# AbeelLab/phasm

Measured on AMD Instinct MI355X. Metric: overlaps_per_sec, higher is better.
Workload: dtype u64

## Files before the change

phasm_amd/csrc/c_api.hip:

```cpp
#include "../../include/phasm_overlap.h"

#include <hip/hip_runtime.h>

#include <dlfcn.h>
#include <execinfo.h>
#include <fcntl.h>
#include <signal.h>
#include <sys/mman.h>
#include <sys/stat.h>
#include <unistd.h>

#include <algorithm>
#include <array>
#include <atomic>
#include <chrono>
#include <cmath>
#include <condition_variable>
#include <cstdio>
#include <cstdlib>
#include <cstring>
#include <deque>
#include <functional>
#include <memory>
#include <mutex>
// ... 65 lines not shown
    uint64_t base, bytes;
    uint32_t kind;
};
std::mutex g_pin_mu;
std::vector<PinNote> g_pins;
uint64_t g_pins_ever = 0;
constexpr size_t PIN_LOG_MAX = 1u << 16;
void pin_note(const void* p, size_t bytes, uint32_t kind) {
    if (!p) return;
    std::lock_guard<std::mutex> lock(g_pin_mu);
    ++g_pins_ever;
    for (PinNote& n : g_pins)
        if (n.base == (uint64_t)(uintptr_t)p && n.bytes == bytes && (n.kind & 0xFFu) == kind) {
            n.kind |= 0x100u;
            return;
        }
    if (g_pins.size() < PIN_LOG_MAX) g_pins.push_back(PinNote{(uint64_t)(uintptr_t)p, (uint64_t)bytes, kind | 0x100u});
}
void pin_drop(const void* p) {
    if (!p) return;
    std::lock_guard<std::mutex> lock(g_pin_mu);
    for (PinNote& n : g_pins)
        if (n.base == (uint64_t)(uintptr_t)p && (n.kind & 0x100u)) n.kind &= ~0x100u;
}

struct HostBuf {
    void* p = nullptr;
    size_t cap = 0;
    void release() {
        if (p) {
            pin_drop(p);
            (void)hipHostFree(p);
        }
        p = nullptr;
        cap = 0;
    }
};

inline int phase_events_env() {
    if (const char* e = getenv("PHASM_PHASE_EVENTS")) {
        const int v = atoi(e);
        return v == 1 ? 1 : v == 2 ? 2 : 0;
    }
    return getenv("PHASM_STREAM_TRACE") ? 1 : -1;
}
enum { EV_START = 0, EV_INDEX, EV_COUNT, EV_FILL, EV_VERIFY, EV_SELECT, EV_EMIT, EV_PROBE0, EV_PROBE1, EV_VER0, EV_VER1, EV_DONE, EV_N };

}

constexpr int PO_MAX_PIECES = 16;

struct RegHeader {
    size_t bytes;
    int registered;
};
constexpr size_t REG_PAGE = 4096;
thread_local bool g_reg_defer = false;
template <class T>
struct RegAlloc {
    using value_type = T;
    RegAlloc() = default;
    template <class U> RegAlloc(const RegAlloc<U>&) {}
    T* allocate(size_t n) {
        const size_t bytes = ((n * sizeof(T) + REG_PAGE - 1) / REG_PAGE) * REG_PAGE;
        void* base = nullptr;
        if (posix_memalign(&base, REG_PAGE, bytes + REG_PAGE) != 0 || !base) throw std::bad_alloc();
        RegHeader* hd = static_cast<RegHeader*>(base);
        hd->bytes = bytes;
        hd->registered = 0;
        char* data = static_cast<char*>(base) + REG_PAGE;
        if (getenv("PHASM_POISON_HOST")) std::memset(data, 0xA5, bytes);
        if (!g_reg_defer) reg_now(data);
        return reinterpret_cast<T*>(data);
    }
    static void reg_now(void* data) {
        RegHeader* hd = reinterpret_cast<RegHeader*>(static_cast<char*>(data) - REG_PAGE);
        if (hd->registered || hd->bytes < (1u << 20) || getenv("PHASM_NO_PIN")) return;
        if (hipHostRegister(data, hd->bytes, hipHostRegisterPortable) == hipSuccess) {
            hd->registered = 1;
            pin_note(data, hd->bytes, 2u);
        } else {
            (void)hipGetLastError();
        }
    }
    template <class U> void construct(U*) noexcept {}
    template <class U, class A0, class... Args> void construct(U* q, A0&& a0, Args&&... args) {
        ::new (static_cast<void*>(q)) U(std::forward<A0>(a0), std::forward<Args>(args)...);
    }
    void deallocate(T* p, size_t) {
        char* base = reinterpret_cast<char*>(p) - REG_PAGE;
        RegHeader* hd = reinterpret_cast<RegHeader*>(base);
        if (hd->registered) {
            pin_drop(p);
            (void)hipHostUnregister(p);
        }
        free(base);
    }
    template <class U> bool operator==(const RegAlloc<U>&) const { return true; }
    template <class U> bool operator!=(const RegAlloc<U>&) const { return false; }
};
using WordStore = std::vector<uint64_t, RegAlloc<uint64_t>>;
inline bool store_is_pinned(const WordStore& w) {
    if (w.capacity() == 0) return false;
    const RegHeader* hd = reinterpret_cast<const RegHeader*>(reinterpret_cast<const char*>(w.data()) - REG_PAGE);
    return hd->registered != 0;
}
constexpr size_t STAGE_MAX = 4u << 20;

struct po_handle {
    int device = 0;
    bool dev_ready = false;
    hipStream_t stream = nullptr;
    hipEvent_t ev_sets[2][EV_N] = {};
    hipEvent_t* ev = ev_sets[0];
    hipEvent_t ev_up0 = nullptr, ev_up1 = nullptr;
    uint64_t* pinned = nullptr;
    uint64_t* pinned_dev = nullptr;
    int n_cu = 256;
    size_t lds_max = 64 * 1024;
    std::string err;

    int bits = 2;
    std::vector<std::string> ids;
    std::vector<uint32_t> len;
    std::vector<uint64_t> cum_len;
    std::vector<uint64_t> woff;
    WordStore words[2];
    bool all_pairs_rc = true;
    bool all_pairs_rcx = true;
    uint64_t base1 = 0;
    uint64_t dev_words = 0;
    uint64_t upload_bytes = 0;
    std::vector<uint32_t> exc_off{0};
    std::vector<uint32_t> exc_pos;
    std::vector<uint8_t> exc_byte;
    std::vector<uint8_t> pair_state;
    uint64_t total_bases = 0;
    bool dirty = true;

    DevBuf d_words, d_woff, d_len, d_tiles, d_read_tile0, d_exc_off, d_exc_pos, d_exc_byte, d_pair_state;
    std::vector<uint32_t> h_read_tile0;
    uint32_t n_tiles = 0;
    uint32_t max_len = 0;
    size_t n_exc_uploaded = 0;
    bool paired = false;

    DevBuf d_table, d_slot_cnt, d_slot_cur, d_slot_start, d_read_slot, d_chain, d_chain_tmp, d_long_list;
    DevBuf d_entry_off;
    DevBuf d_bloom, d_selfrep, d_tile_count, d_tile_off, d_truemask, d_ps_blocks, d_scalars, d_left, d_left_cnt, d_tile_extra;
    DevBuf d_cand_a, d_cand_p, d_cand_b, d_type, d_rowcnt, d_row_off, d_flag, d_pair_key, d_pair_min;
    DevBuf d_vlabel, d_vrank, d_vperm;
    DevBuf d_chain_state;
    DevBuf d_tail_state;
    DevBuf spare_rows;
    DevBuf spare_cands;
    DevBuf spare_edges;
    DevBuf spare_nrank;
    HostBuf spare_host;
    HostBuf scratch_host;
    uint64_t pool_bases = 0;
    std::vector<void*> arena_chunks;
    char* arena_cur = nullptr;
    size_t arena_left = 0;
    int poison = -1;
    hipStream_t copy_stream = nullptr;
    DevBuf chunk_rows[PO_MAX_PIECES + 1];
    bool chunk_compact[PO_MAX_PIECES + 1] = {};
    bool home_on = false;
    HostBuf home_stage;
    size_t home_used = 0;
    uint64_t home_seq = 0;
    uint32_t home_gen = 0;
    uint32_t home_sh_b = 0, home_sh_p = 0;
    uint64_t home_pack_n = ~0ull, home_pack_bases = ~0ull;
    uint32_t home_pack_b = 0, home_pack_p = 0;
    uint64_t home_last_bytes = 0;

    hipStream_t up_stream = nullptr;
    hipEvent_t ev_piece[PO_MAX_PIECES] = {};
    hipStream_t rc_stream = nullptr;
    hipEvent_t ev_rc[PO_MAX_PIECES] = {};
    hipEvent_t ev_meta = nullptr;
    hipEvent_t ev_first = nullptr;
    WordStore first_words;
    uint32_t first_n = 0;
    WordStore lead_words;
    uint32_t lead_n = 0;
    uint32_t st_lead = 2;
    HostBuf meta_host;
    HostBuf stage_host;
    size_t stage_used = 0;
    uint32_t meta_n = 0xFFFFFFFFu;
    int meta_bits = 0;
    uint64_t elig_n = ~0ull, elig_val = 0;
    uint32_t elig_m = 0;
    DevBuf d_first, d_defer;
    uint32_t defer_need = 0;
    struct Pending {
        bool valid = false;
        uint32_t k = 0;
        po_stats S = {};
        bool ver_timed = false;
        bool full_events = true;
        bool pair_events = true;
        bool tail = false;
        bool compact = false;
        int zone = 48;
        uint32_t cap_c = 0;
        hipEvent_t* ev = nullptr;
    } st_pend;
    std::function<po_status()> st_harvest;
    uint64_t st_pred_cand[PO_MAX_PIECES] = {};
    std::vector<uint32_t> st_pred_sig;
    bool st_pred_valid = false;
    bool st_selfclean = false;
    bool st_early_index = false;
    bool st_tail_gave_up = false;
    uint32_t st_defer_cap = 0;
    uint64_t last_host_rows = 0;
    uint64_t upload_gen = 0;
    bool idx_valid = false;
    uint64_t idx_gen = 0;
    uint32_t idx_m = 0, idx_tbits = 0, idx_bits = 0, idx_ww = 0;
    bool idx_wide = false;
    bool sl_is_wide = false;
    uint32_t sl_tbits = 0;
    uint64_t sl_entries = 0;
    const uint64_t* asm_pieces = nullptr;
    uint64_t asm_slot_words = 0;
    uint32_t asm_n = 0, asm_parts = 1;
    DevBuf d_end_a, d_end_b, d_dpcnt;
    int live_results = 0;

    po_stats stats = {};

    bool segments_only = false;
    int ids_paired = -1;
    hipEvent_t ev_lay[EV_LAY_N] = {};
    DevBuf d_lay_len, d_lay_cnt, d_rflag, d_removed, d_ekey, d_ecnt, d_ewin, d_eoff;
    DevBuf d_efirst;
    po_layout_stats lstats = {};

    DevBuf d_red[RB_N];
    po_reduce_stats rstats = {};

    DevBuf d_lay_firstc;
    DevBuf d_tip[TB_N];
    po_tips_stats tstats = {};
    po_diamond_stats dstats = {};
    po_node_order_stats nostats = {};

    DevBuf d_mrg[MB_N];
    po_merge_stats mstats = {};

    DevBuf d_cov[VB_N];
    po_coverage_stats cstats = {};

    DevBuf d_rank[RK_N];
    DevBuf d_cc[KB_N];
    po_components_stats ccstats = {};
    DevBuf d_scc[PB_N];
    po_partition_stats pstats = {};
    DevBuf d_sb[UB_N];
    po_superbubble_stats sbstats = {};
    DevBuf d_bc[HB_N];
    po_bubblechain_stats bcstats = {};
    DevBuf d_ct[CB_N];
    po_contig_stats ctstats = {};
    DevBuf d_ph[FB_N];
    po_phase_stats phstats = {};
};

struct po_result {
    po_handle* h = nullptr;
    DevBuf d_rows;
    uint64_t count = 0;
    size_t elem = sizeof(po_row);
    bool kind_edges = false;
    void* host = nullptr;
    size_t host_cap = 0;
    bool host_malloced = false;
    bool unique_twins = false;
    DevBuf d_rank;
    DevBuf d_nrank;
    bool merged = false;
    bool host_graph = false;
    uint64_t n_merged = 0, n_members = 0;
    DevBuf d_moff, d_member, d_prefix, d_mlen;
    void* ext_dst = nullptr;
    uint64_t ext_cap = 0;
    bool wrote_ext = false;
    bool compact = false;
};

namespace {

po_status fail(po_handle* h, po_status st, const std::string& msg) {
    if (h) h->err = msg;
    return st;
}

#define HIP_TRY(h, expr)                                                                        \
    do {                                                                                        \
        hipError_t e_ = (expr);                                                                 \
        if (e_ != hipSuccess) {                                                                 \
            return fail((h), e_ == hipErrorOutOfMemory ? PO_ERR_NOMEM : PO_ERR_HIP,             \
                        std::string(#expr) + ": " + hipGetErrorString(e_));                     \
        }                                                                                       \
    } while (0)

struct AllocTrace {
    const char* what;
    size_t bytes;
    std::chrono::steady_clock::time_point t0;
    bool on;
    AllocTrace(const char* w, size_t b) : what(w), bytes(b), on(getenv("PHASM_ALLOC_TRACE") != nullptr) {
        if (on) t0 = std::chrono::steady_clock::now();
    }
    ~AllocTrace() {
        if (on)
            std::fprintf(stderr, "[alloc] %-16s %10.3f MB  %8.3f ms\n", what, bytes / 1e6,
                         std::chrono::duration<double, std::milli>(std::chrono::steady_clock::now() - t0).count());
    }
};

struct OverlapArgs {
    uint32_t min_length = 0, shard = 0, nshards = 1;
    bool want_cands = false;
    bool streamed = false, idx_only = false;
    uint32_t r_begin = 0, r_end = 0;
    double ws_scale = 1.0;
    uint32_t build_slice = 0, build_n = 0;
    const void* ext_index = nullptr;
    uint32_t ext_slices = 0, ext_tbits = 0, ext_chunk_slots = 0, ext_chain_off = 0;
    bool dp = false;
    uint32_t dp_E = 0, dp_W = 0;
};

po_status ensure(po_handle* h, DevBuf& b, size_t bytes, double scale = 1.0, bool arena_ok = true, bool streamed = false) {
    if (bytes <= b.cap) return PO_OK;
    AllocTrace tr("hipMalloc", bytes);
    const bool first = b.p == nullptr;
    b.release();
    size_t want = bytes + bytes / 8 + 256;
    if (scale > 1.0) want = (size_t)((double)bytes * scale) + 256;
    if (streamed) want += 8192;
    constexpr size_t ARENA_CHUNK = 64u << 20, ARENA_MAX = 8u << 20;
    if (h && first && arena_ok && want <= ARENA_MAX && !getenv("PHASM_NO_ARENA")) {
        want = (want + 255) & ~size_t(255);
        if (h->arena_left < want) {
            void* c = nullptr;
            if (hipMalloc(&c, ARENA_CHUNK) == hipSuccess) {
                h->arena_chunks.push_back(c);
                h->arena_cur = static_cast<char*>(c);
                h->arena_left = ARENA_CHUNK;
            } else {
                (void)hipGetLastError();
            }
        }
        if (h->arena_left >= want) {
            b.p = h->arena_cur;
            b.cap = want;
            b.arena = true;
            h->arena_cur += want;
            h->arena_left -= want;
            if (h->poison >= 0 && h->stream) (void)hipMemsetAsync(b.p, h->poison, want, h->stream);
            return PO_OK;
        }
    }
    hipError_t e = hipMalloc(&b.p, want);
    if (e != hipSuccess) {
// ... 110 lines not shown
        h->ev_up0 = k.ev_up0;
        h->ev_up1 = k.ev_up1;
        h->ev_meta = k.ev_meta;
        h->ev_first = k.ev_first;
        std::memcpy(h->ev_piece, k.ev_piece, sizeof(k.ev_piece));
        std::memcpy(h->ev_rc, k.ev_rc, sizeof(k.ev_rc));
        std::memcpy(h->ev_lay, k.ev_lay, sizeof(k.ev_lay));
        h->pinned = k.pinned;
        h->pinned_dev = k.pinned_dev;
        return true;
    }
    return false;
}

bool kit_give(po_handle* h) {
    if (getenv("PHASM_NO_KIT_POOL") || !h->stream || !h->copy_stream || !h->up_stream || !h->rc_stream || !h->pinned) return false;
    if (hipStreamSynchronize(h->stream) != hipSuccess || hipStreamSynchronize(h->copy_stream) != hipSuccess ||
        hipStreamSynchronize(h->up_stream) != hipSuccess || hipStreamSynchronize(h->rc_stream) != hipSuccess) {
        (void)hipGetLastError();
        return false;
    }
    DevKit k;
    k.device = h->device;
    k.stream = h->stream;
    k.copy_stream = h->copy_stream;
    k.up_stream = h->up_stream;
    k.rc_stream = h->rc_stream;
    std::memcpy(k.ev_sets, h->ev_sets, sizeof(k.ev_sets));
    k.ev_up0 = h->ev_up0;
    k.ev_up1 = h->ev_up1;
    k.ev_meta = h->ev_meta;
    k.ev_first = h->ev_first;
    std::memcpy(k.ev_piece, h->ev_piece, sizeof(k.ev_piece));
    std::memcpy(k.ev_rc, h->ev_rc, sizeof(k.ev_rc));
    std::memcpy(k.ev_lay, h->ev_lay, sizeof(k.ev_lay));
    k.pinned = h->pinned;
    k.pinned_dev = h->pinned_dev;
    std::lock_guard<std::mutex> lock(g_kit_mu);
    if (g_kits.size() >= KIT_POOL_MAX) return false;
    g_kits.push_back(k);
    return true;
}


unsigned cpu_share() {
    static const unsigned share = [] {
        unsigned n = std::thread::hardware_concurrency();
        n = n ? n : 4u;
        long long q = -1, per = 100000;
        if (FILE* f = std::fopen("/sys/fs/cgroup/cpu.max", "r")) {
            char buf[64] = {0};
            if (std::fscanf(f, "%63s %lld", buf, &per) >= 1 && std::strcmp(buf, "max") != 0) q = atoll(buf);
            std::fclose(f);
        } else if (FILE* g = std::fopen("/sys/fs/cgroup/cpu/cpu.cfs_quota_us", "r")) {
            if (std::fscanf(g, "%lld", &q) != 1) q = -1;
            std::fclose(g);
            if (FILE* g2 = std::fopen("/sys/fs/cgroup/cpu/cpu.cfs_period_us", "r")) {
                if (std::fscanf(g2, "%lld", &per) != 1) per = 100000;
                std::fclose(g2);
            }
        }
        if (q > 0 && per > 0) n = std::min<unsigned>(n, (unsigned)std::max<long long>(1, q / per));
        return n;
    }();
    return share;
}

namespace home {

constexpr uint32_t CHUNK = 4096;

struct Job {
    const void* rec = nullptr;
    uint32_t sh_b = 0, sh_p = 0;
    uint64_t n_rec = 0;
    po_row* out = nullptr;
    uint64_t n_rows = 0;
    const volatile uint32_t* flag = nullptr;
    uint32_t want = 0;
    uint32_t paired = 0, bits = 2;
};

struct Pool {
    std::vector<std::thread> thr;
    std::mutex mu;
    std::condition_variable cv_queue;
    std::condition_variable cv_job;
    std::mutex call_mu;
    std::deque<Job> queue;
    std::atomic<uint64_t> submitted{0}, finished{0};
    std::atomic<int> error{0};
    const uint32_t* len = nullptr;
    uint32_t n_reads = 0;
    std::atomic<uint64_t> sum_l{0}, sum_b{0}, sum_e{0};
    Job cur;
    uint64_t job_seq = 0;
    uint32_t n_chunks = 0;
    std::vector<uint64_t> chunk_off;
    std::atomic<uint32_t> next_count{0}, done_count{0}, next_write{0}, done_write{0};
    std::atomic<int> phase{0};
    std::atomic<int> inside{0};
    std::chrono::steady_clock::time_point t0;
    std::vector<std::array<double, 3>> trace;
    bool tracing = false;
};

Pool* g_pool = nullptr;
std::once_flag g_pool_once;

inline void cpu_pause() {
#if defined(__x86_64__) || defined(__i386__)
    __builtin_ia32_pause();
#endif
}

std::atomic<uint32_t> g_spin_limit{4096};
template <class Pred>
inline void spin_until(Pred pred) {
    const uint32_t limit = g_spin_limit.load(std::memory_order_relaxed);
    for (uint32_t n = 0; !pred(); ++n) {
        if (limit == 0 || n < limit) cpu_pause();
        else std::this_thread::yield();
    }
}

inline po::Cand load_rec(const Job& j, uint64_t i) {
    if (!j.sh_b) return static_cast<const po::Cand*>(j.rec)[i];
    return po::unpack_record(static_cast<const uint64_t*>(j.rec)[i], j.sh_b, j.sh_p);
}

inline uint32_t rows_of_rec(const po::Cand& c, uint32_t paired) {
    if (!paired) return (c.type & 1u) + ((c.type >> 1) & 1u);
    return ((c.type & 1u) ? (c.a == (c.b ^ 1u) ? 1u : 2u) : 0u) + ((c.type & 2u) ? 2u : 0u);
}

inline void put_row(uint64_t*& o, uint32_t a, uint32_t b, uint32_t astart, uint32_t aend, uint32_t bend) {
    __builtin_nontemporal_store((uint64_t)a | ((uint64_t)b << 32), o);
    __builtin_nontemporal_store((uint64_t)astart | ((uint64_t)aend << 32), o + 1);
    __builtin_nontemporal_store((uint64_t)bend << 32, o + 2);
    o += 3;
}

bool expand_records(Pool& P, uint64_t lo, uint64_t hi, po_row* out) {
    uint64_t* o = reinterpret_cast<uint64_t*>(out);
    const Job& job = P.cur;
    const uint32_t* len = P.len;
    const uint32_t paired = job.paired, n_reads = P.n_reads, bits = job.bits;
    auto pb = [bits](uint32_t l) -> uint64_t { return bits == 8u ? l : (l >> 2) + ((l & 3u) != 0u); };
    uint64_t sl = 0, sb = 0, se = 0;
    for (uint64_t i = lo; i < hi; ++i) {
        const po::Cand c = load_rec(job, i);
        if (c.a >= n_reads || c.b >= n_reads) return false;
        const uint32_t la = len[c.a], lb = len[c.b];
        se += 2 * pb((c.type & 1u) ? la - c.p : lb);
        if (c.type & 1u) {
            const uint32_t l = la - c.p;
            const bool twin = paired && c.a != (c.b ^ 1u);
            put_row(o, c.a, c.b, c.p, la, l);
            if (twin) put_row(o, c.b ^ 1u, c.a ^ 1u, lb - l, lb, l);
            const uint64_t k = twin ? 2 : 1;
            sl += k * l;
            sb += k * 2 * pb(l);
        }
        if (c.type & 2u) {
            put_row(o, c.a, c.b, c.p, c.p + lb, lb);
            if (paired) put_row(o, c.a ^ 1u, c.b ^ 1u, la - c.p - lb, la - c.p, lb);
            const uint64_t k = paired ? 2 : 1;
            sl += k * lb;
            sb += k * 2 * pb(lb);
        }
    }
    P.sum_l.fetch_add(sl, std::memory_order_relaxed);
    P.sum_b.fetch_add(sb, std::memory_order_relaxed);
    P.sum_e.fetch_add(se, std::memory_order_relaxed);
    return true;
}

void run_phases(Pool& P, bool lead) {
    const uint32_t nc = P.n_chunks;
    for (;;) {
        const uint32_t c = P.next_count.fetch_add(1, std::memory_order_relaxed);
        if (c >= nc) break;
        const uint64_t lo = (uint64_t)c * CHUNK, hi = std::min<uint64_t>(P.cur.n_rec, lo + CHUNK);
        uint64_t n = 0;
        const uint32_t paired = P.cur.paired;
        for (uint64_t i = lo; i < hi; ++i) n += rows_of_rec(load_rec(P.cur, i), paired);
        P.chunk_off[c + 1] = n;
        P.done_count.fetch_add(1, std::memory_order_release);
    }
    if (lead) {
        spin_until([&] { return P.done_count.load(std::memory_order_acquire) >= nc; });
        P.chunk_off[0] = 0;
        for (uint32_t c = 0; c < nc; ++c) P.chunk_off[c + 1] += P.chunk_off[c];
        if (P.chunk_off[nc] != P.cur.n_rows) P.error.store(1);
        P.phase.store(P.error.load() ? 0 : 2, std::memory_order_release);
    } else {
        spin_until([&] { return P.phase.load(std::memory_order_acquire) != 1; });
    }
    if (P.phase.load(std::memory_order_acquire) != 2) return;
    for (;;) {
        const uint32_t c = P.next_write.fetch_add(1, std::memory_order_relaxed);
        if (c >= nc) break;
        const uint64_t lo = (uint64_t)c * CHUNK, hi = std::min<uint64_t>(P.cur.n_rec, lo + CHUNK);
        if (!expand_records(P, lo, hi, P.cur.out + P.chunk_off[c])) P.error.store(2);
#if defined(__x86_64__)
        __builtin_ia32_sfence();
#endif
        P.done_write.fetch_add(1, std::memory_order_release);
    }
}

void helper(Pool* Pp) {
    Pool& P = *Pp;
    uint64_t seen = 0;
    for (;;) {
        {
            std::unique_lock<std::mutex> lock(P.mu);
            P.cv_job.wait(lock, [&] { return P.job_seq != seen; });
            seen = P.job_seq;
        }
        P.inside.fetch_add(1, std::memory_order_acq_rel);
        if (P.phase.load(std::memory_order_acquire) != 0) run_phases(P, false);
        P.inside.fetch_sub(1, std::memory_order_release);
    }
}

void leader(Pool* Pp) {
    Pool& P = *Pp;
    for (;;) {
        Job j;
        {
            std::unique_lock<std::mutex> lock(P.mu);
            P.cv_queue.wait(lock, [&] { return !P.queue.empty(); });
            j = P.queue.front();
            P.queue.pop_front();
        }
        if (j.flag)
            spin_until([&] { return *j.flag == j.want; });
        std::atomic_thread_fence(std::memory_order_acquire);
        const double t_ready = P.tracing ? std::chrono::duration<double, std::micro>(std::chrono::steady_clock::now() - P.t0).count() : 0.0;
        if (P.error.load() == 0 && j.n_rec) {
            spin_until([&] { return P.inside.load(std::memory_order_acquire) == 0; });
            P.cur = j;
            P.n_chunks = (uint32_t)((j.n_rec + CHUNK - 1) / CHUNK);
            if (P.chunk_off.size() < (size_t)P.n_chunks + 1) P.chunk_off.resize((size_t)P.n_chunks + 1);
            P.next_count.store(0);
            P.done_count.store(0);
            P.next_write.store(0);
            P.done_write.store(0);
            P.phase.store(1, std::memory_order_release);
            {
                std::lock_guard<std::mutex> lock(P.mu);
                ++P.job_seq;
            }
            P.cv_job.notify_all();
            run_phases(P, true);
            if (P.phase.load() == 2)
                spin_until([&] { return P.done_write.load(std::memory_order_acquire) >= P.n_chunks; });
            P.phase.store(0, std::memory_order_release);
            std::atomic_thread_fence(std::memory_order_seq_cst);
        }
        if (P.tracing)
            P.trace.push_back({t_ready, std::chrono::duration<double, std::micro>(std::chrono::steady_clock::now() - P.t0).count(), (double)j.n_rows});
        P.finished.fetch_add(1, std::memory_order_release);
    }
}

Pool* pool() {
    std::call_once(g_pool_once, [] {
        Pool* P = new Pool();
        unsigned n = cpu_share();
        n = std::max(1u, std::min(n * 3 / 4, 12u));
        if (const char* e = getenv("PHASM_HOME_THREADS")) n = (unsigned)std::max(1, std::min(64, atoi(e)));
        try {
            P->thr.emplace_back(leader, P);
            P->thr.back().detach();
            for (unsigned i = 1; i < n; ++i) {
                P->thr.emplace_back(helper, P);
                P->thr.back().detach();
            }
        } catch (const std::system_error&) {
        }
        if (P->thr.empty()) {
            delete P;
            P = nullptr;
        }
        g_pool = P;
    });
    return g_pool;
}

void begin(Pool* P, const uint32_t* len, uint32_t n_reads, bool tracing) {
    if (const char* e = getenv("PHASM_HOME_SPIN")) g_spin_limit.store((uint32_t)std::max(0, atoi(e)));
    else g_spin_limit.store(4096);
    P->len = len;
    P->n_reads = n_reads;
    P->error.store(0);
    P->submitted.store(0);
    P->finished.store(0);
    P->sum_l.store(0);
    P->sum_b.store(0);
    P->sum_e.store(0);
    P->tracing = tracing;
    P->trace.clear();
    P->t0 = std::chrono::steady_clock::now();
}

void submit(Pool* P, const Job& j) {
    {
        std::lock_guard<std::mutex> lock(P->mu);
        P->queue.push_back(j);
    }
    P->submitted.fetch_add(1, std::memory_order_release);
    P->cv_queue.notify_one();
}

void wait_all(Pool* P) {
    spin_until([&] { return P->finished.load(std::memory_order_acquire) >= P->submitted.load(std::memory_order_acquire); });
}

}

po_status init_device(po_handle* h) {
    if (h->dev_ready) {
        HIP_TRY(h, hipSetDevice(h->device));
        return PO_OK;
    }
    AllocTrace tr("init_device", 0);
    const auto ti0 = std::chrono::steady_clock::now();
    auto imark = [&](const char* what) {
        if (tr.on) std::fprintf(stderr, "[init] %s at %.1f ms\n", what, std::chrono::duration<double, std::milli>(std::chrono::steady_clock::now() - ti0).count());
    };
    int n = 0;
    hipError_t e = hipGetDeviceCount(&n);
    imark("runtime up (hipGetDeviceCount)");
    if (e != hipSuccess || n == 0)
        return fail(h, PO_ERR_HIP, "no HIP device available (libphasm_overlap has no CPU fallback)");
    if (h->device < 0 || h->device >= n) return fail(h, PO_ERR_INVALID, "device ordinal out of range");
    HIP_TRY(h, hipSetDevice(h->device));
    hipDeviceProp_t prop;
    HIP_TRY(h, hipGetDeviceProperties(&prop, h->device));
    h->n_cu = prop.multiProcessorCount > 0 ? prop.multiProcessorCount : 256;
    h->lds_max = prop.sharedMemPerBlock;
    if (const char* e = getenv("PHASM_POISON")) h->poison = (int)(strtol(e, nullptr, 0) & 0xFF);
    if (!getenv("PHASM_NO_KIT_POOL") && kit_take(h)) {
        h->ev = h->ev_sets[0];
        std::memset(h->pinned, 0, 1024);
        hipLaunchKernelGGL(po::k_fill_u32, dim3(1), dim3(64), 0, h->stream, reinterpret_cast<uint32_t*>(h->pinned_dev + 63), (uint64_t)1, 0u);
        (void)hipGetLastError();
        h->dev_ready = true;
        return PO_OK;
    }
    imark("device selected, properties read");
    HIP_TRY(h, hipStreamCreateWithFlags(&h->stream, hipStreamNonBlocking));
    imark("first stream made");
    for (int i = 0; i < 2 * EV_N; ++i) HIP_TRY(h, hipEventCreate(&h->ev_sets[i / EV_N][i % EV_N]));
    HIP_TRY(h, hipEventCreate(&h->ev_up0));
    HIP_TRY(h, hipEventCreate(&h->ev_up1));
    imark("first events made");
    HIP_TRY(h, hipHostMalloc(reinterpret_cast<void**>(&h->pinned), 1024, hipHostMallocDefault));
    pin_note(h->pinned, 1024, 1u);
    HIP_TRY(h, hipHostGetDevicePointer(reinterpret_cast<void**>(&h->pinned_dev), h->pinned, 0));
    imark("landing zone made");
    if (const char* e = getenv("PHASM_POISON")) h->poison = (int)(strtol(e, nullptr, 0) & 0xFF);
    HIP_TRY(h, hipStreamCreateWithFlags(&h->copy_stream, hipStreamNonBlocking));
    imark("copy stream made");
    HIP_TRY(h, hipStreamCreateWithFlags(&h->up_stream, hipStreamNonBlocking));
    HIP_TRY(h, hipStreamCreateWithFlags(&h->rc_stream, hipStreamNonBlocking));
    imark("other streams made");
    for (int k = 0; k < PO_MAX_PIECES; ++k) {
        HIP_TRY(h, hipEventCreate(&h->ev_piece[k]));
        HIP_TRY(h, hipEventCreateWithFlags(&h->ev_rc[k], hipEventDisableTiming));
    }
    HIP_TRY(h, hipEventCreateWithFlags(&h->ev_first, hipEventDisableTiming));
    HIP_TRY(h, hipEventCreateWithFlags(&h->ev_meta, hipEventDisableTiming));
    imark("streams and events made");
    hipLaunchKernelGGL(po::k_fill_u32, dim3(1), dim3(64), 0, h->stream, reinterpret_cast<uint32_t*>(h->pinned_dev + 63), (uint64_t)1, 0u);
    (void)hipGetLastError();
    imark("first launch queued (code object loaded)");
    if (!getenv("PHASM_NO_WARM")) {
        void* w = nullptr;
        if (hipMalloc(&w, 256) == hipSuccess) {
            uint32_t* wd = static_cast<uint32_t*>(w);
            (void)hipMemcpyAsync(wd, h->pinned + 62, 8, hipMemcpyHostToDevice, h->up_stream);
            hipLaunchKernelGGL(po::k_fill_u32, dim3(1), dim3(64), 0, h->up_stream, wd + 8, (uint64_t)1, 0u);
            (void)hipMemcpyAsync(wd + 16, h->pinned + 62, 8, hipMemcpyHostToDevice, h->stream);
            hipLaunchKernelGGL(po::k_fill_u32, dim3(1), dim3(64), 0, h->rc_stream, wd + 24, (uint64_t)1, 0u);
            hipLaunchKernelGGL(po::k_fill_u32, dim3(1), dim3(64), 0, h->copy_stream, wd + 32, (uint64_t)1, 0u);
            (void)hipMemcpyAsync(h->pinned + 61, wd + 32, 8, hipMemcpyDeviceToHost, h->copy_stream);
            (void)hipMemcpyAsync(h->pinned + 60, wd + 16, 8, hipMemcpyDeviceToHost, h->stream);
            (void)hipStreamSynchronize(h->up_stream);
            (void)hipStreamSynchronize(h->rc_stream);
            (void)hipStreamSynchronize(h->copy_stream);
            (void)hipStreamSynchronize(h->stream);
            (void)hipFree(w);
        }
        (void)hipGetLastError();
        imark("queues and copy paths warmed");
        static const void* const warm_kernels[] = {
            (const void*)po::k_abs_woff, (const void*)po::k_build_tiles, (const void*)po::k_revcomp_store, (const void*)po::k_scatter_first,
            (const void*)po::k_paired_check, (const void*)po::k_call_init, (const void*)po::k_call_reset, (const void*)po::k_table_insert,
            (const void*)po::k_chain_fill, (const void*)po::k_chain_sort_short<uint32_t>, (const void*)po::k_chain_sort_long<uint32_t>,
            (const void*)po::k_table_finalize, (const void*)po::k_ps_reduce<uint32_t>, (const void*)po::k_ps_spine, (const void*)po::k_ps_down<uint32_t>,
            (const void*)po::k_ps_reduce<uint8_t>, (const void*)po::k_ps_down<uint8_t>, (const void*)po::k_ps_chain<uint32_t>,
            (const void*)po::k_ps_chain<uint8_t>, (const void*)po::k_ps_small,
            (const void*)po::k_scan_probe<2, true, true>, (const void*)po::k_scan_probe<2, true, false>, (const void*)po::k_scan_fixup<2, true>,
            (const void*)po::k_scan_fixup<2, false>, (const void*)po::k_scan_fill<2, true>, (const void*)po::k_scan_fill<2, false>,
            (const void*)po::k_read_label, (const void*)po::k_read_sort, (const void*)po::k_read_invert, (const void*)po::k_defer_split,
            (const void*)po::k_verify_a<2, false, true, true>, (const void*)po::k_verify_a<2, false, true, false>,
            (const void*)po::k_verify_a<2, true, true, false>, (const void*)po::k_select_local, (const void*)po::k_tile_rows<true>,
            (const void*)po::k_tile_rows<false>, (const void*)po::k_tail, (const void*)po::k_tail_cands, (const void*)po::k_select,
            (const void*)po::k_emit, (const void*)po::k_verify_flat, (const void*)po::k_deferred_rowcnt, (const void*)po::k_emit_cands,
            (const void*)po::k_wide_insert<2, 1>, (const void*)po::k_wide_insert<2, 16>, (const void*)po::k_wide_chain_fill<2, 1>,
            (const void*)po::k_wide_chain_fill<2, 16>, (const void*)po::k_wide_finalize<2, 1>, (const void*)po::k_wide_finalize<2, 16>,
            (const void*)po::k_chain_sort_short<uint64_t>, (const void*)po::k_chain_sort_long<uint64_t>,
            (const void*)po::k_wide_scan<2, false, true, 1>, (const void*)po::k_wide_scan<2, true, true, 1>,
            (const void*)po::k_wide_scan<2, false, false, 16>, (const void*)po::k_wide_scan<2, true, false, 16>};
        for (const void* k : warm_kernels) {
            hipFuncAttributes fa;
            (void)hipFuncGetAttributes(&fa, k);
        }
        (void)hipGetLastError();
        imark("kernels looked up");
    }
    h->dev_ready = true;
    return PO_OK;
}

struct BaseLut {
    uint8_t v[256];
    BaseLut() {
        std::memset(v, 0x80, sizeof(v));
        v[(unsigned char)'A'] = 0;
        v[(unsigned char)'C'] = 1;
        v[(unsigned char)'G'] = 2;
        v[(unsigned char)'T'] = 3;
    }
};
const BaseLut g_lut;

bool append_packed(po_handle* h, const unsigned char* s, size_t n, int bits) {
    const size_t per = 64 / bits;
    WordStore& store = h->words[h->woff.size() & 1];
    const size_t old_size = store.size();
    const size_t off = (old_size + 1) & ~size_t(1);
    const size_t nw = (n + per - 1) / per;
    store.resize(off + nw + 1, 0);
    uint64_t* w = store.data() + off;
    if (bits == 2) {
        const uint8_t* lut = g_lut.v;
        uint8_t bad = 0;
        const size_t full = n / 32;
        for (size_t k = 0; k < full; ++k) {
            const unsigned char* q = s + k * 32;
            uint64_t acc = 0;
            for (int j = 0; j < 32; ++j) {
                const uint8_t c = lut[q[j]];
                bad |= c;
                acc |= (uint64_t)(c & 3) << (2 * j);
            }
            w[k] = acc;
        }
        if (full * 32 < n) {
            uint64_t acc = 0;
            for (size_t i = full * 32; i < n; ++i) {
                const uint8_t c = lut[s[i]];
                bad |= c;
                acc |= (uint64_t)(c & 3) << (2 * (i & 31));
            }
            w[full] = acc;
        }
        if (bad & 0x80) {
            size_t cnt = 0;
            for (size_t i = 0; i < n; ++i) cnt += lut[s[i]] >> 7;
            if (cnt > n / 64 + 16) {
                store.resize(old_size);
                return false;
            }
            for (size_t i = 0; i < n; ++i) {
                if (lut[s[i]] & 0x80) {
                    h->exc_pos.push_back((uint32_t)i);
                    h->exc_byte.push_back(s[i]);
                }
            }
        }
        h->exc_off.push_back((uint32_t)h->exc_pos.size());
    } else {
        for (size_t i = 0; i < n; ++i) w[i >> 3] |= (uint64_t)s[i] << ((i & 7) * 8);
    }
    h->woff.push_back(off);
    return true;
}

void materialize(const po_handle* h, size_t r, const WordStore* stores, const uint64_t* woff, std::vector<unsigned char>& out) {
    const uint32_t n = h->len[r];
    out.resize(n);
    const uint64_t* w = stores[r & 1].data() + woff[r];
    for (uint32_t i = 0; i < n; ++i) out[i] = "ACGT"[(w[i >> 5] >> ((i & 31) * 2)) & 3];
    for (uint32_t e = h->exc_off[r]; e < h->exc_off[r + 1]; ++e) out[h->exc_pos[e]] = h->exc_byte[e];
}

void widen_to_bytes(po_handle* h) {
    WordStore old_words[2];
    std::vector<uint64_t> old_off;
    old_words[0].swap(h->words[0]);
    old_words[1].swap(h->words[1]);
    old_off.swap(h->woff);
    std::vector<unsigned char> tmp;
    for (size_t r = 0; r < h->len.size(); ++r) {
        materialize(h, r, old_words, old_off.data(), tmp);
        append_packed(h, tmp.data(), h->len[r], 8);
    }
    h->bits = 8;
    h->all_pairs_rc = false;
    h->all_pairs_rcx = false;
    h->first_n = 0;
    h->first_words.clear();
    h->lead_n = 0;
    h->lead_words.clear();
    h->exc_off.assign(1, 0);
    h->exc_pos.clear();
    h->exc_byte.clear();
    h->pair_state.clear();
}

const unsigned char* comp_table() {
    static unsigned char comp[256];
    static bool init = false;
    if (!init) {
        for (int i = 0; i < 256; ++i) comp[i] = (unsigned char)i;
        const char* from = "ACGTURYKMBVDHSWNacgturykmbvdhswn";
        const char* to = "TGCAAYRMKVBHDSWNtgcaayrmkvbhdswn";
        for (int i = 0; from[i]; ++i) comp[(unsigned char)from[i]] = (unsigned char)to[i];
        init = true;
    }
    return comp;
}

void host_pair_check(po_handle* h, size_t r, const unsigned char* s) {
    const size_t pair = r / 2;
    if (h->pair_state.size() <= pair) h->pair_state.resize(pair + 1, 0);
    const bool has_exc = h->exc_off[r - 1] != h->exc_off[r] || h->exc_off[r] != h->exc_off[r + 1];
    if (!has_exc) return;
    const uint32_t n = h->len[r];
    uint8_t state = 1;
    if (h->len[r - 1] != n) {
        state = 2;
    } else {
        std::vector<unsigned char> prev;
        materialize(h, r - 1, h->words, h->woff.data(), prev);
        const unsigned char* c = comp_table();
        for (uint32_t i = 0; i < n; ++i) {
            const unsigned char x = prev[n - 1 - i], y = s[i];
            if (c[x] != y || c[y] != x) {
                state = 2;
                break;
            }
        }
    }
    h->pair_state[pair] = state;
}

bool packed_is_revcomp(const po_handle* h, size_t r) {
    const uint32_t L = h->len[r];
// ... 257 lines not shown
    HIP_TRY(h, hipStreamSynchronize(h->stream));
    if (try_paired) h->paired = (uint32_t)h->pinned[0] == 0;
    float ms = 0;
    (void)hipEventElapsedTime(&ms, h->ev_up0, h->ev_up1);
    h->stats.ms_upload = ms;
    h->stats.upload_bytes = h->upload_bytes;
    ++h->upload_gen;
    h->dirty = false;
    return PO_OK;
}

void shard_range(const po_handle* h, uint32_t shard, uint32_t nshards, uint32_t* r_begin, uint32_t* r_end, uint64_t* bases) {
    const uint32_t n = (uint32_t)h->len.size();
    std::vector<uint64_t>& cum = const_cast<po_handle*>(h)->cum_len;
    if (cum.size() != (size_t)n + 1) {
        size_t have = cum.empty() ? 0 : std::min(cum.size() - 1, (size_t)n);
        cum.resize((size_t)n + 1);
        if (have == 0) cum[0] = 0;
        for (size_t r = have; r < n; ++r) cum[r + 1] = cum[r] + h->len[r];
    }
    auto cut = [&](uint32_t s) -> uint32_t {
        if (s == 0) return 0;
        if (s >= nshards) return n;
        const uint64_t target = (uint64_t)((__uint128_t)cum[n] * s / nshards);
        return (uint32_t)(std::lower_bound(cum.begin(), cum.end(), target) - cum.begin());
    };
    *r_begin = cut(shard);
    *r_end = cut(shard + 1);
    if (*r_end < *r_begin) *r_end = *r_begin;
    if (bases) *bases = cum[*r_end] - cum[*r_begin];
}

po_status chain_state(po_handle* h, uint32_t n_tiles, po::ChainState** out, hipStream_t on, bool streamed = false) {
    const size_t need = po::chain_state_bytes(n_tiles);
    if (need > h->d_chain_state.cap) {
        PO_TRY(ensure(h, h->d_chain_state, std::max<size_t>(need * 2, 1u << 16), 1.0, true, streamed));
        HIP_TRY(h, hipMemsetAsync(h->d_chain_state.p, 0, h->d_chain_state.cap, on));
    }
    *out = h->d_chain_state.as<po::ChainState>();
    return PO_OK;
}

template <typename T>
po_status prefix_sum(po_handle* h, const T* in, uint64_t n, uint32_t* out, volatile uint64_t* total_host,
                     const uint64_t* also_src = nullptr, volatile uint64_t* also_host = nullptr, const uint32_t* extra = nullptr,
                     hipStream_t on = nullptr, uint64_t* total_dev_at = nullptr, const OverlapArgs& a = OverlapArgs()) {
    *total_host = 0;
    if (n == 0) return PO_OK;
    const hipStream_t ps = on ? on : h->stream;
    const uint32_t nblocks = cdiv(n, po::PS_TILE);
    uint64_t* total_dev = total_dev_at ? total_dev_at : h->d_scalars.as<uint64_t>();
    uint64_t* total_mapped = h->pinned_dev + (const_cast<uint64_t*>(total_host) - h->pinned);
    uint64_t* also_mapped = also_host ? h->pinned_dev + (const_cast<uint64_t*>(also_host) - h->pinned) : nullptr;
    if (nblocks <= 64 && !getenv("PHASM_PS_CLASSIC")) {

        po::ChainState* cs = nullptr;
        PO_TRY(chain_state(h, nblocks, &cs, ps, a.streamed));
        hipLaunchKernelGGL(po::k_ps_chain<T>, dim3(nblocks), dim3(po::PS_BLOCK), 0, ps, const_cast<T*>(in), extra, n, out, cs,
                           nblocks, total_dev, total_mapped, also_src, also_mapped);
        HIP_TRY(h, hipGetLastError());
        return PO_OK;
    }
    if (extra) {
        hipLaunchKernelGGL(po::k_add_extra, dim3(cdiv(n, 256)), dim3(256), 0, ps, const_cast<uint32_t*>(reinterpret_cast<const uint32_t*>(in)),
                           extra, 0u, (uint32_t)n);
    }
    PO_TRY(ensure_piece(h, h->d_ps_blocks, (size_t)nblocks * 8, a));
    uint64_t* blocks = h->d_ps_blocks.as<uint64_t>();
    hipLaunchKernelGGL(po::k_ps_reduce<T>, dim3(nblocks), dim3(po::PS_BLOCK), 0, ps, in, n, blocks);
    hipLaunchKernelGGL(po::k_ps_spine, dim3(1), dim3(1024), 0, ps, blocks, nblocks, total_dev, total_mapped, also_src, also_mapped);
    hipLaunchKernelGGL(po::k_ps_down<T>, dim3(nblocks), dim3(po::PS_BLOCK), 0, ps, in, n, blocks, out);
    HIP_TRY(h, hipGetLastError());
    return PO_OK;
}

po_status prefix_sum_small(po_handle* h, uint32_t* in, const uint32_t* extra, uint32_t n, uint32_t* out, volatile uint64_t* total_host,
                           const uint64_t* also_src, volatile uint64_t* also_host, hipStream_t on = nullptr, uint64_t* total_dev_at = nullptr) {
    *total_host = 0;
    if (n == 0) return PO_OK;
    const hipStream_t ps = on ? on : h->stream;
    uint64_t* total_dev = total_dev_at ? total_dev_at : h->d_scalars.as<uint64_t>();
    uint64_t* total_mapped = h->pinned_dev + (const_cast<uint64_t*>(total_host) - h->pinned);
    uint64_t* also_mapped = also_host ? h->pinned_dev + (const_cast<uint64_t*>(also_host) - h->pinned) : nullptr;
    hipLaunchKernelGGL(po::k_ps_small, dim3(1), dim3(1024), 0, ps, in, extra, n, out, total_dev, total_mapped,
                       also_src, also_mapped);
    HIP_TRY(h, hipGetLastError());
    return PO_OK;
}

void stage_times(po_stats& S, hipEvent_t* ev, bool ver_timed, bool full, bool pairs = true) {
    if (!full && !pairs) {
        S.ms_index = S.ms_scan_count = S.ms_scan_fill = S.ms_verify = S.ms_select = S.ms_emit = 0.f;
        S.ms_total = S.ms_scan_probe = S.ms_verify_kernel = 0.f;
        return;
    }
    if (!full) {
        S.ms_index = S.ms_scan_count = S.ms_scan_fill = S.ms_verify = S.ms_select = S.ms_emit = 0.f;
        (void)hipEventElapsedTime(&S.ms_total, ev[EV_START], ev[EV_EMIT]);
        (void)hipEventElapsedTime(&S.ms_scan_probe, ev[EV_PROBE0], ev[EV_PROBE1]);
        S.ms_verify_kernel = 0.f;
        if (ver_timed) (void)hipEventElapsedTime(&S.ms_verify_kernel, ev[EV_VER0], ev[EV_VER1]);
        return;
    }
    (void)hipEventElapsedTime(&S.ms_index, ev[EV_START], ev[EV_INDEX]);
    (void)hipEventElapsedTime(&S.ms_scan_count, ev[EV_INDEX], ev[EV_COUNT]);
    (void)hipEventElapsedTime(&S.ms_scan_fill, ev[EV_COUNT], ev[EV_FILL]);
    (void)hipEventElapsedTime(&S.ms_verify, ev[EV_FILL], ev[EV_VERIFY]);
    (void)hipEventElapsedTime(&S.ms_select, ev[EV_VERIFY], ev[EV_SELECT]);
    (void)hipEventElapsedTime(&S.ms_emit, ev[EV_SELECT], ev[EV_EMIT]);
    (void)hipEventElapsedTime(&S.ms_total, ev[EV_START], ev[EV_EMIT]);
    (void)hipEventElapsedTime(&S.ms_scan_probe, ev[EV_PROBE0], ev[EV_PROBE1]);
    S.ms_verify_kernel = 0.f;
    if (ver_timed) (void)hipEventElapsedTime(&S.ms_verify_kernel, ev[EV_VER0], ev[EV_VER1]);
}

uint64_t close_stats(po_handle* h, po_stats& S, int rows_at, int cnt_at, hipEvent_t* ev, bool ver_timed, bool full, bool pairs) {
    const uint64_t n_rows = rows_at < 0 ? 0 : h->pinned[rows_at];
    S.n_rows = n_rows;
    S.n_verified = h->pinned[cnt_at];
    S.sum_overlap_bases = h->pinned[cnt_at + 1];
    S.verify_bytes_algo = h->pinned[cnt_at + 2];
    S.verify_bytes_exec = h->pinned[cnt_at + 3];
    stage_times(S, ev, ver_timed, full, pairs);
    return n_rows;
}

uint64_t finish_piece(po_handle* h, bool* needs_classic) {
    po_handle::Pending& P = h->st_pend;
    *needs_classic = P.tail && h->pinned[P.zone + 7] != 0;
    if (P.cap_c) {
        P.S.n_candidates = h->pinned[P.zone + 8];
        if (P.S.n_candidates > P.cap_c) *needs_classic = true;
    }
    P.valid = false;
    return close_stats(h, P.S, P.tail ? P.zone : 2, P.tail ? P.zone + 1 : 4, P.ev, P.ver_timed, P.full_events, P.pair_events);
}

struct OverlapSwitches {
    const char* index = getenv("PHASM_INDEX");
    const char* wide_window = getenv("PHASM_WIDE_WINDOW");
    const char* table_mult = getenv("PHASM_TABLE_MULT");
    const char* scan_waves = getenv("PHASM_SCAN_WAVES");
    const char* pred_scale = getenv("PHASM_PRED_SCALE");
    const char* verify_order = getenv("PHASM_VERIFY_ORDER");
    const char* verify_staged = getenv("PHASM_VERIFY_STAGED");
    const char* dp_kernel = getenv("PHASM_DP_KERNEL");
    const char* dp_kernel_soft = getenv("PHASM_DP_KERNEL_SOFT");
    const char* dp_sort = getenv("PHASM_DP_SORT");
    const bool no_index_reuse = getenv("PHASM_NO_INDEX_REUSE") != nullptr;
    const bool debug_left = getenv("PHASM_DEBUG_LEFT") != nullptr;
    const bool piece_reset = getenv("PHASM_PIECE_RESET") != nullptr;
    const bool sync_count = getenv("PHASM_SYNC_COUNT") != nullptr;
    const bool tail_classic = getenv("PHASM_TAIL_CLASSIC") != nullptr;
    const bool select_kernel = getenv("PHASM_SELECT_KERNEL") != nullptr;
    const bool compact_sync = getenv("PHASM_COMPACT_SYNC") != nullptr;
    const int phase_events = phase_events_env();
};

struct IndexFlavour {
    bool wide;
    uint32_t ww;
};
IndexFlavour index_flavour(po_handle* h, uint32_t m, bool streamed, uint32_t lead, const OverlapSwitches& sw, bool inexact = false) {
    const uint32_t W = 64 / h->bits;
    bool wide = count_eligible(h, m) > 160000 && m >= 2 * W - 1;
    if (sw.index) {
        if (!strcmp(sw.index, "wide")) wide = m >= 2 * W - 1;
        if (!strcmp(sw.index, "narrow")) wide = false;
    }
    if (inexact) wide = false;
    uint32_t ww = 1;
    if (wide && h->bits == 2) {
        ww = m >= W * 16 + W - 1 ? 16u : m >= W * 4 + W - 1 ? 4u : 1u;
        if (streamed) ww = (ww >= 4 && lead >= LEAD_WORDS) ? 4u : 1u;
        if (sw.wide_window) {
            const uint32_t v = (uint32_t)atoi(sw.wide_window);
            if ((v == 1 || v == 4 || v == 16) && v <= ww) ww = v;
        }
    }
    return {wide, ww};
}

po_status take_row_buffer(po_handle* h, po_result* res, bool rows_late, uint64_t n_rows, uint64_t worst_rows, bool streamed = false) {
    if (rows_late || (h->spare_rows.cap >= n_rows * sizeof(po_row) && h->spare_rows.p)) {
        res->d_rows = h->spare_rows;
        h->spare_rows = DevBuf();
    } else {
        h->spare_rows.release();
    }
    if (rows_late) return PO_OK;
    const size_t exact = n_rows * sizeof(po_row);
    size_t roomy = worst_rows * sizeof(po_row) <= (2ull << 30) ? (size_t)(worst_rows * sizeof(po_row)) : 0;
    if (roomy && streamed) roomy += 4096 * sizeof(po_row);
    return ensure(h, res->d_rows, std::max<size_t>(std::max(exact, roomy), 256), 1.0, false, streamed);
}

template <int BITS>
struct OverlapCall {
    static constexpr uint32_t W = 64 / BITS;
    po_handle* const h;
    const OverlapArgs& a;
    po_result* const res;
    const OverlapSwitches sw;
    const hipStream_t st;
    po_stats& S;

    uint32_t n = 0, m = 1, K = 1;
    uint64_t kmask = 0;
    uint32_t paired = 0, paired_ver = 0, dpE = 0, dpW = 0;
    uint32_t r_begin = 0, r_end = 0, tile_begin = 0, tile_end = 0, ntiles = 0;
    uint64_t n_elig = 0;
    bool wide = false;
    uint32_t ww = 1;
    bool slice_build = false;
    bool ext_idx = false;
    bool own_lists = false;
    uint32_t tbits = 10, nslots = 0, bloom_log2 = 13;
    size_t bloom_bytes = 0, n_entries = 0, chain_elem = 4;
    bool phase_events = true;
    bool pair_events = true;
    bool reuse_index = false, fold_clear = false;
    uint32_t scan_waves = 0, scan_grid = 0;
    bool self_clean = false;
    bool sel_in_verify = false, staged = false, dp_lanes = false, dp_bitvec = false;
    int zone = 64;

    const uint64_t* words = nullptr;
    const uint64_t* woff = nullptr;
    const uint32_t* len = nullptr;
    po::Slot* table = nullptr;
    uint32_t *slot_cnt = nullptr, *slot_cur = nullptr, *slot_start = nullptr, *read_slot = nullptr, *chain = nullptr;
    uint32_t *bloom = nullptr, *selfrep = nullptr, *tile_off_p = nullptr, *n_long = nullptr;
    unsigned long long* scalars = nullptr;
    uint32_t* n_deferred = nullptr;

    po::ScanArgs A = {};
    po::WideArgs WA = {};
    uint32_t cap_c = 0;
    bool async_count = false, pred_order = true;
    po::CandGuard G = {nullptr, 0u};
    uint64_t n_cand64 = 0, worst_rows = 0;
    uint32_t n_cand = 0, n_selfrep_reads = 0;
    bool use_order = false, defer_needed = false;
    bool ver_timed = false;
    bool compact_tail = false, can_tail = false;
    bool rows_late = false;
    bool cands_late = false, cands_ext = false;
    uint64_t cands_cap = 0;
    bool used_tail = false;
    int tail_zone = 48;

    OverlapCall(po_handle* h_, const OverlapArgs& a_, po_result* res_) : h(h_), a(a_), res(res_), st(h_->stream), S(h_->stats) {}

    po_status ws(DevBuf& b, size_t bytes, bool arena_ok = true) { return ensure(h, b, bytes, 1.0, arena_ok, a.streamed); }
    po_status ws_piece(DevBuf& b, size_t bytes) { return ensure_piece(h, b, bytes, a); }
    template <typename T>
    po_status prefix(const T* in, uint64_t count, uint32_t* out, volatile uint64_t* total_host) {
        return prefix_sum<T>(h, in, count, out, total_host, nullptr, nullptr, nullptr, nullptr, nullptr, a);
    }

    po_status plan(bool* done) {
        *done = true;
        n = (uint32_t)h->len.size();
        m = a.min_length ? a.min_length : 1;
        K = m < W ? m : W;
        kmask = K * BITS >= 64 ? ~0ull : ((1ull << (K * BITS)) - 1ull);
        const float keep_upload = S.ms_upload;
        S = po_stats();
        S.ms_upload = keep_upload;
        S.upload_bytes = h->upload_bytes;
        S.bits_per_base = BITS;
        S.kmer = K;
        S.n_reads = n;
        S.total_bases = h->total_bases;
        dpE = a.dp ? a.dp_E : 0u;
        dpW = a.dp && a.dp_E ? a.dp_W : 0u;
        paired = (BITS == 2 && h->paired && dpE == 0) ? (a.streamed ? po::PAIRED_STREAM_ALL : a.nshards > 1 ? 2u : 1u) : 0u;
        paired_ver = a.streamed ? po::paired_stream(a.r_end) : paired;
        if (a.streamed && (!paired || a.want_cands)) return fail(h, PO_ERR_INVALID, "streamed step without strand pairs");
        S.paired = paired ? 1u : 0u;
        S.max_diff = dpE;
        S.band = dpW;
        if (a.dp && dpE && a.want_cands) return fail(h, PO_ERR_INVALID, "the candidate (multi-GPU) form has no inexact mode");
        if (a.dp && dpE && BITS == 2 && !h->exc_pos.empty())
            return fail(h, PO_ERR_INVALID, "po_overlaps_ex with max_diff > 0 needs pure upper-case ACGT reads (or the 8-bit representation)");

        r_end = n;
        S.shard_bases = h->total_bases;
        if (a.streamed) {
            r_begin = a.r_begin;
            r_end = a.r_end;
            S.shard_bases = 0;
            for (uint32_t r = r_begin; r < r_end; ++r) S.shard_bases += h->len[r];
        } else if (a.nshards > 1) {
            shard_range(h, a.shard, a.nshards, &r_begin, &r_end, &S.shard_bases);
        }
        tile_begin = h->h_read_tile0[r_begin];
        tile_end = h->h_read_tile0[r_end];
        ntiles = tile_end - tile_begin;
        S.n_tiles = ntiles;

        n_elig = count_eligible(h, m);
        S.n_eligible = n_elig;
        res->count = 0;
        if (n == 0 || n_elig == 0 || ntiles == 0) return PO_OK;

// ... 102 lines not shown

    template <typename T>
    void sort_chains() {
        hipLaunchKernelGGL(po::k_chain_sort_short<T>, dim3(cdiv(nslots, 256)), dim3(256), 0, st, slot_cnt, slot_start,
                           nslots, h->d_chain.as<T>(), h->d_long_list.as<uint32_t>(), n_long);
        hipLaunchKernelGGL(po::k_chain_sort_long<T>, dim3(64), dim3(256), 0, st, slot_cnt, slot_start,
                           h->d_long_list.as<uint32_t>(), n_long, h->d_chain.as<T>(), h->d_chain_tmp.as<T>());
    }

    po_status build_index(bool* done) {
        *done = true;
        if (pair_events) HIP_TRY(h, hipEventRecord(h->ev[EV_START], st));
        S.index_reused = reuse_index ? 1u : 0u;
        h->idx_valid = false;
        if (fold_clear) {
        } else if (reuse_index || ext_idx) {
            hipLaunchKernelGGL(po::k_call_reset, dim3(cdiv(std::max(n, 16u), 256)), dim3(256), 0, st, selfrep, n, scalars, 8u,
                               (uint32_t*)nullptr, 0u, (uint32_t*)nullptr, 0u);
        } else {
            const uint32_t bloom_words = (uint32_t)(bloom_bytes / 4);
            const uint32_t init_n = std::max(std::max(nslots, n), std::max(bloom_words, 8u));
            hipLaunchKernelGGL(po::k_call_init, dim3(cdiv(init_n, 256)), dim3(256), 0, st, table, nslots, slot_cnt, slot_cur, selfrep, n,
                               bloom, bloom_words, h->d_scalars.as<unsigned long long>());
        }
        if (reuse_index || ext_idx) {
        } else if (!wide) {
            hipLaunchKernelGGL(po::k_table_insert, dim3(cdiv(n, 256)), dim3(256), 0, st, words, woff, len, n, m, kmask, table,
                               tbits, slot_cnt, read_slot, bloom, bloom_log2, (uint32_t)BITS);
            PO_TRY(prefix<uint32_t>(slot_cnt, nslots, slot_start, &h->pinned[0]));
            hipLaunchKernelGGL(po::k_chain_fill, dim3(cdiv(n, 256)), dim3(256), 0, st, read_slot, n, slot_start, slot_cur, chain);
            sort_chains<uint32_t>();
            hipLaunchKernelGGL(po::k_table_finalize, dim3(cdiv(nslots, 256)), dim3(256), 0, st, table, nslots, slot_cnt,
                               slot_start, chain, len);
        } else {
            uint16_t* entry_off = h->d_entry_off.as<uint16_t>();
            auto k_ins = ww == 16 ? po::k_wide_insert<BITS, 16> : ww == 4 ? po::k_wide_insert<BITS, 4> : po::k_wide_insert<BITS, 1>;
            auto k_cfill = ww == 16 ? po::k_wide_chain_fill<BITS, 16> : ww == 4 ? po::k_wide_chain_fill<BITS, 4> : po::k_wide_chain_fill<BITS, 1>;
            auto k_fin = ww == 16 ? po::k_wide_finalize<BITS, 16> : ww == 4 ? po::k_wide_finalize<BITS, 4> : po::k_wide_finalize<BITS, 1>;
            hipLaunchKernelGGL(k_ins, dim3(cdiv(n_entries, 256)), dim3(256), 0, st, words, woff, len, n, m,
                               table, tbits, slot_cnt, read_slot, entry_off, slice_build ? a.build_n : 1u, a.build_slice);
            PO_TRY(prefix<uint32_t>(slot_cnt, nslots, slot_start, &h->pinned[0]));
            if (slice_build) {
                HIP_TRY(h, hipStreamSynchronize(st));
                PO_TRY(ws(h->d_chain, (size_t)h->pinned[0] * chain_elem));
                PO_TRY(ws(h->d_chain_tmp, (size_t)h->pinned[0] * chain_elem));
            }
            uint64_t* chain64 = h->d_chain.as<uint64_t>();
            hipLaunchKernelGGL(k_cfill, dim3(cdiv(n_entries, 256)), dim3(256), 0, st, read_slot, entry_off,
                               (uint64_t)n_entries, slot_start, slot_cur, chain64, len);
            sort_chains<uint64_t>();
            hipLaunchKernelGGL(k_fin, dim3(cdiv(nslots, 256)), dim3(256), 0, st, table, nslots, slot_cnt,
                               slot_start, chain64, len);
        }
        HIP_TRY(h, hipGetLastError());
        if (phase_events) HIP_TRY(h, hipEventRecord(h->ev[EV_INDEX], st));
        if (slice_build) {
            HIP_TRY(h, hipStreamSynchronize(st));
            h->sl_tbits = tbits;
            h->sl_entries = h->pinned[0];
            if (phase_events) (void)hipEventElapsedTime(&S.ms_index, h->ev[EV_START], h->ev[EV_INDEX]);
            return PO_OK;
        }
        h->idx_valid = a.idx_only || !ext_idx;
        h->idx_gen = h->upload_gen;
        h->idx_m = m;
        h->idx_wide = wide;
        h->idx_tbits = tbits;
        h->idx_bits = (uint32_t)BITS;
        h->idx_ww = ww;
        *done = a.idx_only;
        return PO_OK;
    }

    po_status scan_count() {
        A.words = words;
        A.tiles = h->d_tiles.as<po::TileRec>();
        A.tile_begin = tile_begin;
        A.tile_end = tile_end;
        A.m = m;
        A.kmask = kmask;
        A.bloom = bloom;
        A.bloom_log2 = bloom_log2;
        A.table = table;
        A.tbits = tbits;
        A.chain = chain;
        A.len = len;
        A.paired = paired;
        A.selfrep = selfrep;
        A.n_selfrep = reinterpret_cast<uint32_t*>(scalars + 2);
        A.tile_count = h->d_tile_count.as<uint32_t>();
        A.tile_off = tile_off_p;
        A.truemask = h->d_truemask.as<uint32_t>();
#ifdef PO_STAMPS
        PO_TRY(ws(h->d_flag, (size_t)4096 * 64));
        HIP_TRY(h, hipMemsetAsync(h->d_flag.p, 0, (size_t)4096 * 64, st));
        A.dbg = h->d_flag.as<unsigned long long>();
#endif
        WA.words = words;
        WA.tiles = A.tiles;
        WA.tile_begin = tile_begin;
        WA.tile_end = tile_end;
        WA.m = m;
        WA.table = table;
        WA.tbits = tbits;
        WA.chain = h->d_chain.as<uint64_t>();
        WA.n_slices = 1;
        if (ext_idx) {
            WA.table = static_cast<const po::Slot*>(a.ext_index);
            WA.chain = nullptr;
            WA.n_slices = a.ext_slices;
            WA.chunk_slots = a.ext_chunk_slots;
            WA.chain_off_slots = a.ext_chain_off;
        }
        WA.len = len;
        WA.paired = paired;
        WA.tile_count = A.tile_count;
        WA.lane_slot = A.truemask;
        WA.tile_off = A.tile_off;
        if (wide) {
            if (pair_events) HIP_TRY(h, hipEventRecord(h->ev[EV_PROBE0], st));
            auto wscan = a.streamed ? (ww == 4 ? po::k_wide_scan<BITS, false, BITS == 2, 4> : po::k_wide_scan<BITS, false, BITS == 2, 1>)
                         : ww == 16 ? po::k_wide_scan<BITS, false, false, 16> : ww == 4 ? po::k_wide_scan<BITS, false, false, 4> : po::k_wide_scan<BITS, false, false, 1>;
            hipLaunchKernelGGL(wscan, dim3(cdiv(ntiles, 4)), dim3(256), 0, st, WA, po::CandGuard{nullptr, 0u});
            if (pair_events) HIP_TRY(h, hipEventRecord(h->ev[EV_PROBE1], st));
        } else {
            const size_t scan_lds = (size_t)scan_waves * po::SCAN_LDS_PER_WAVE + bloom_bytes;
            if (scan_lds > h->lds_max) return fail(h, PO_ERR_HIP, "device LDS too small for the scan kernel");
            constexpr bool CAN_STREAM = BITS == 2;
            auto probe_full = a.streamed ? po::k_scan_probe<BITS, true, CAN_STREAM> : po::k_scan_probe<BITS, true, false>;
            auto probe_part = a.streamed ? po::k_scan_probe<BITS, false, CAN_STREAM> : po::k_scan_probe<BITS, false, false>;
            HIP_TRY(h, hipFuncSetAttribute(reinterpret_cast<const void*>(probe_full), hipFuncAttributeMaxDynamicSharedMemorySize, (int)scan_lds));
            HIP_TRY(h, hipFuncSetAttribute(reinterpret_cast<const void*>(probe_part), hipFuncAttributeMaxDynamicSharedMemorySize, (int)scan_lds));
            const uint32_t n_scan_waves = scan_grid * scan_waves;
            PO_TRY(ws(h->d_left, (size_t)n_scan_waves * po::LEFT_CAP * sizeof(uint2)));
            PO_TRY(ws(h->d_left_cnt, (size_t)n_scan_waves * 4));
            PO_TRY(ws(h->d_tile_extra, ((size_t)h->n_tiles + 1) * 4));
            if (fold_clear && self_clean && h->st_selfclean) {
            } else if (fold_clear) {
                const uint32_t te0 = self_clean ? 0u : tile_begin, ten = self_clean ? h->n_tiles : ntiles;
                hipLaunchKernelGGL(po::k_call_reset, dim3(cdiv(std::max(std::max(n, 16u), std::max(n_scan_waves, ten)), 256)), dim3(256), 0, st,
                                   selfrep, n, self_clean ? h->d_scalars.as<unsigned long long>() : scalars, self_clean ? 16u : 8u,
                                   h->d_left_cnt.as<uint32_t>(), n_scan_waves, h->d_tile_extra.as<uint32_t>() + te0, ten);
            } else {
                HIP_TRY(h, hipMemsetAsync(h->d_left_cnt.p, 0, (size_t)n_scan_waves * 4, st));
                HIP_TRY(h, hipMemsetAsync(h->d_tile_extra.as<uint32_t>() + tile_begin, 0, (size_t)ntiles * 4, st));
            }
            A.left = h->d_left.as<uint2>();
            A.left_cnt = h->d_left_cnt.as<uint32_t>();
            A.tile_extra = h->d_tile_extra.as<uint32_t>();
            if (pair_events) HIP_TRY(h, hipEventRecord(h->ev[EV_PROBE0], st));
            hipLaunchKernelGGL(K == W ? probe_full : probe_part, dim3(scan_grid), dim3(scan_waves * 64), scan_lds, st, A);
            if (pair_events) HIP_TRY(h, hipEventRecord(h->ev[EV_PROBE1], st));
            auto fixup = a.streamed ? po::k_scan_fixup<BITS, CAN_STREAM> : po::k_scan_fixup<BITS, false>;
            hipLaunchKernelGGL(fixup, dim3(n_scan_waves), dim3(256), 0, st, A, n_scan_waves, self_clean ? 1u : 0u);
            if (sw.debug_left) {
                PO_TRY(ensure_host(h, h->scratch_host, (size_t)n_scan_waves * 4));
                HIP_TRY(h, hipMemcpyAsync(h->scratch_host.p, h->d_left_cnt.p, (size_t)n_scan_waves * 4, hipMemcpyDeviceToHost, st));
                HIP_TRY(h, hipStreamSynchronize(st));
                const uint32_t* lc = static_cast<const uint32_t*>(h->scratch_host.p);
                uint64_t sum = 0;
                uint32_t mx = 0;
                for (uint32_t k = 0; k < n_scan_waves; ++k) sum += lc[k], mx = std::max(mx, lc[k]);
                std::fprintf(stderr, "[left] %u scan waves deferred %llu positions (max %u per wave, cap %d)\n", n_scan_waves,
                             (unsigned long long)sum, mx, (int)po::LEFT_CAP);
            }
        }
        HIP_TRY(h, hipGetLastError());
#ifdef PO_STAMPS
        if (!wide) {
            std::vector<unsigned long long> dbg(4096 * 8);
            HIP_TRY(h, hipMemcpyAsync(dbg.data(), h->d_flag.p, dbg.size() * 8, hipMemcpyDeviceToHost, st));
            HIP_TRY(h, hipStreamSynchronize(st));
            double sum[6] = {0, 0, 0, 0, 0, 0};
            for (size_t w = 0; w < 4096; ++w) for (int k = 0; k < 6; ++k) sum[k] += (double)dbg[w * 8 + k];
            if (sum[5] > 0)
                std::fprintf(stderr, "[stamps] per pass (cycles): wait_rw %.0f  filter %.0f  wait_probe %.0f  consume %.0f  issue %.0f  (passes %.0f)\n",
                             sum[0] / sum[5], sum[1] / sum[5], sum[2] / sum[5], sum[3] / sum[5], sum[4] / sum[5], sum[5]);
        }
#endif
        return PO_OK;
    }

    po_status candidate_count() {
        if (a.streamed && h->st_harvest && h->st_pred_valid && !a.dp && !a.want_cands && !sw.sync_count && !sw.tail_classic) {
            uint64_t pred = h->st_pred_cand[a.shard];
            uint64_t cap = pred + pred / 50 + 256;
            if (sw.pred_scale) cap = pred = (uint64_t)((double)pred * atof(sw.pred_scale));
            const uint64_t worst = cap * 4u;
            bool order = pred >= 400000 && (r_end - r_begin) >= 4096;
            if (sw.verify_order) order = atoi(sw.verify_order) != 0;
            pred_order = order;
            auto fits = [](const DevBuf& b, uint64_t bytes) { return b.p && b.cap >= bytes; };
            async_count = pred > 0 && cap < (16u << 20) && cdiv(cap, po::TAIL_TILE) <= po::TAIL_MAX_TILES &&
                          fits(h->d_cand_a, cap * 4) && fits(h->d_cand_p, cap * 4) && fits(h->d_cand_b, cap * 4) && fits(h->d_type, cap) &&
                          fits(h->d_rowcnt, cap) && fits(h->d_row_off, (cap + 1) * 4) &&
                          fits(h->spare_rows, h->home_on ? cap * sizeof(po::Cand) : worst * sizeof(po_row)) &&
                          (!order || (fits(h->d_vlabel, (uint64_t)(r_end - r_begin) * 4) && fits(h->d_vperm, (uint64_t)(r_end - r_begin) * 4) &&
                                      fits(h->d_vrank, (uint64_t)(r_end - r_begin) * 4))) && h->dev_words < 0xFFFFFFF0ull;
            cap_c = (uint32_t)cap;
        }
        volatile uint64_t* count_slot = async_count ? &h->pinned[zone + 8] : &h->pinned[1];
        volatile uint64_t* also_slot = async_count ? &h->pinned[zone + 9] : &h->pinned[8];
        if (ntiles <= po::PS_SMALL_MAX) {
            PO_TRY(prefix_sum_small(h, A.tile_count + tile_begin, wide ? nullptr : A.tile_extra + tile_begin, ntiles,
                                    tile_off_p + tile_begin, count_slot,
                                    reinterpret_cast<const uint64_t*>(scalars + 2), also_slot, st, reinterpret_cast<uint64_t*>(scalars)));
        } else {
            PO_TRY(prefix_sum<uint32_t>(h, A.tile_count + tile_begin, ntiles, tile_off_p + tile_begin, count_slot,
                                        reinterpret_cast<const uint64_t*>(scalars + 2), also_slot,
                                        wide ? nullptr : A.tile_extra + tile_begin, st, reinterpret_cast<uint64_t*>(scalars), a));
        }
        if (phase_events) HIP_TRY(h, hipEventRecord(h->ev[EV_COUNT], st));
        if (async_count) {
            n_cand64 = cap_c;
            n_selfrep_reads = 0;
            S.n_predicted = 1;
            G.n_dev = scalars;
            G.cap = cap_c;
        } else {
            if (h->st_pend.valid && h->st_harvest) {
                HIP_TRY(h, hipEventSynchronize(h->st_pend.ev[EV_DONE]));
                PO_TRY(h->st_harvest());
            }
            HIP_TRY(h, hipStreamSynchronize(st));
            n_cand64 = h->pinned[1];
            n_selfrep_reads = (uint32_t)h->pinned[8];
        }
        if (own_lists || dpE) n_selfrep_reads |= 1u;
        S.n_candidates = n_cand64;
        if (n_cand64 >= 0xFFFFFF00ull)
            return fail(h, PO_ERR_CAPACITY, "candidate count " + std::to_string(n_cand64) + " exceeds one call's capacity (2^32)");
        n_cand = (uint32_t)n_cand64;
        worst_rows = (uint64_t)n_cand * (paired ? 4u : 2u);
        return PO_OK;
    }

    po_status scan_fill() {
        PO_TRY(ws_piece(h->d_cand_a, (size_t)n_cand * 4));
        PO_TRY(ws_piece(h->d_cand_p, (size_t)n_cand * 4));
        PO_TRY(ws_piece(h->d_cand_b, (size_t)n_cand * 4));
        PO_TRY(ws_piece(h->d_type, (size_t)n_cand));
        PO_TRY(ws_piece(h->d_rowcnt, (size_t)n_cand));
        PO_TRY(ws_piece(h->d_row_off, ((size_t)n_cand + 1) * 4));
        A.cand_a = h->d_cand_a.as<uint32_t>();
        A.cand_p = h->d_cand_p.as<uint32_t>();
        A.cand_b = h->d_cand_b.as<uint32_t>();
        if (wide) {
            WA.cand_a = A.cand_a;
            WA.cand_p = A.cand_p;
            WA.cand_b = A.cand_b;
            auto wfill = a.streamed ? (ww == 4 ? po::k_wide_scan<BITS, true, BITS == 2, 4> : po::k_wide_scan<BITS, true, BITS == 2, 1>)
                         : ww == 16 ? po::k_wide_scan<BITS, true, false, 16> : ww == 4 ? po::k_wide_scan<BITS, true, false, 4> : po::k_wide_scan<BITS, true, false, 1>;
            hipLaunchKernelGGL(wfill, dim3(cdiv(ntiles, 4)), dim3(256), 0, st, WA, G);
        } else {
            auto fill = a.streamed ? po::k_scan_fill<BITS, BITS == 2> : po::k_scan_fill<BITS, false>;
            hipLaunchKernelGGL(fill, dim3(cdiv(ntiles, 4 * po::FILL_TILES)), dim3(256), 0, st, A, G);
        }
        use_order = n_cand >= 400000 && (r_end - r_begin) >= 4096;
        if (sw.verify_order) use_order = atoi(sw.verify_order) != 0;
        if (async_count) use_order = pred_order;
        use_order = use_order && !a.dp;
        defer_needed = a.streamed && r_end < n;
        if (defer_needed && !use_order) {
            hipLaunchKernelGGL(po::k_defer_split, dim3(cdiv(n_cand, 256)), dim3(256), 0, st, A.cand_a, A.cand_p, A.cand_b, n_cand,
                               r_end, h->d_defer.as<po::Cand>(), h->st_defer_cap, h->d_defer.as<uint32_t>() + (size_t)h->st_defer_cap * 4, G);
        }
        HIP_TRY(h, hipGetLastError());
        if (phase_events) HIP_TRY(h, hipEventRecord(h->ev[EV_FILL], st));
        return PO_OK;
    }

    po_status verify_dp() {
        if (2ull * h->max_len + 64ull >= (1ull << 30))
            return fail(h, PO_ERR_CAPACITY, "po_overlaps_ex: reads of 2^29 bases or more are beyond the DP kernel");
        PO_TRY(ws(h->d_end_a, (size_t)n_cand * 4));
        PO_TRY(ws(h->d_end_b, (size_t)n_cand * 4));
        PO_TRY(ws(h->d_dpcnt, 64));
        HIP_TRY(h, hipMemsetAsync(h->d_dpcnt.p, 0, 64, st));
        po::ExtArgs X = {};
        X.words = words;
        X.woff = woff;
        X.len = len;
        X.cand_a = A.cand_a;
        X.cand_p = A.cand_p;
        X.cand_b = A.cand_b;
        X.n_cand = n_cand;
        X.max_diff = dpE;
        X.band = dpW;
        X.paired = paired;
        X.exc_off = h->n_exc_uploaded ? h->d_exc_off.as<uint32_t>() : nullptr;
        X.exc_pos = h->d_exc_pos.as<uint32_t>();
        X.exc_byte = h->d_exc_byte.as<uint8_t>();
        X.type = h->d_type.as<uint8_t>();
        X.end_a = h->d_end_a.as<uint32_t>();
        X.end_b = h->d_end_b.as<uint32_t>();
        X.counters = h->d_dpcnt.as<unsigned long long>();
        S.dp_lanes = dp_bitvec ? 2u : dp_lanes ? 1u : 0u;
        if (pair_events) HIP_TRY(h, hipEventRecord(h->ev[EV_VER0], st));
        if (dp_lanes) {
            const uint32_t* perm = nullptr;
            bool sorted = n_cand >= 4096;
            if (sw.dp_sort) sorted = atoi(sw.dp_sort) != 0;
            if (sorted) {
                const uint32_t max_bins = (uint32_t)((std::min<size_t>(h->lds_max, 160 * 1024) - 1024) / 4);
                const uint32_t max_rows = h->max_len + dpW;
                uint32_t shift = 0;
                while ((max_rows >> shift) + 1 > max_bins) ++shift;
                const uint32_t n_bins = (max_rows >> shift) + 1;
                const size_t sort_lds = ((size_t)n_bins + po::SORT_BLOCK / 64) * 4;
                PO_TRY(ws(h->d_vlabel, (size_t)n_cand * 4));
                PO_TRY(ws(h->d_vrank, (size_t)n_cand * 4));
                PO_TRY(ws(h->d_vperm, (size_t)n_cand * 4));
                hipLaunchKernelGGL(po::k_dp_rows, dim3(cdiv(n_cand, 256)), dim3(256), 0, st, A.cand_a, A.cand_p, A.cand_b, len, n_cand,
                                   dpW, h->d_vlabel.as<uint32_t>());
                if (sort_lds > 48 * 1024)
                    HIP_TRY(h, hipFuncSetAttribute(reinterpret_cast<const void*>(po::k_read_sort),
                                                   hipFuncAttributeMaxDynamicSharedMemorySize, (int)sort_lds));
                hipLaunchKernelGGL(po::k_read_sort, dim3(1), dim3(po::SORT_BLOCK), sort_lds, st, h->d_vlabel.as<uint32_t>(), n_cand,
                                   shift, n_bins, h->d_vrank.as<uint32_t>());
                hipLaunchKernelGGL(po::k_read_invert, dim3(cdiv(n_cand, 256)), dim3(256), 0, st, h->d_vrank.as<uint32_t>(), n_cand, 0u,
                                   h->d_vperm.as<uint32_t>());
                perm = h->d_vperm.as<uint32_t>();
            }
            auto kern = dp_bitvec ? po::k_extend_bits : dpW <= 4 ? po::k_extend_lanes<4> : dpW <= 8 ? po::k_extend_lanes<8> : po::k_extend_lanes<15>;
            hipLaunchKernelGGL(kern, dim3(cdiv(n_cand, 256)), dim3(256), 0, st, X, perm);
        } else {
            hipLaunchKernelGGL((po::k_extend_dp<BITS>), dim3(cdiv(n_cand, 256 / po::WAVE)), dim3(256), 0, st, X);
        }
        if (pair_events) HIP_TRY(h, hipEventRecord(h->ev[EV_VER1], st));
        HIP_TRY(h, hipMemcpyAsync(h->pinned + 32, h->d_dpcnt.p, 16, hipMemcpyDeviceToHost, st));
        return PO_OK;
    }

    po_status verify_exact() {
        const uint64_t need_words = ((uint64_t)h->max_len + W - 1) / W + 3;
        const uint32_t lds_words_raw = (uint32_t)std::min<uint64_t>(need_words, 8192 - 1100);
        const uint32_t n_a = r_end - r_begin;
        const uint32_t* perm = nullptr;
        if (use_order) {
            const uint32_t max_bins = (uint32_t)((std::min<size_t>(h->lds_max, 160 * 1024) - 1024) / 4);
            uint32_t shift = 0, n_bins;
            while ((n >> shift) + 1 > max_bins) ++shift;
            n_bins = (n >> shift) + 1;
            const size_t sort_lds = ((size_t)n_bins + po::SORT_BLOCK / 64) * 4;
            PO_TRY(ws(h->d_vlabel, (size_t)n_a * 4));
            PO_TRY(ws(h->d_vperm, (size_t)n_a * 4));
            po::DeferOut dfo = {};
            if (defer_needed) {
                dfo.cand_p = A.cand_p;
                dfo.b_limit = r_end;
                dfo.list = h->d_defer.as<uint4>();
                dfo.cap = h->st_defer_cap;
                dfo.counter = h->d_defer.as<uint32_t>() + (size_t)h->st_defer_cap * 4;
            }
            hipLaunchKernelGGL(po::k_read_label, dim3(cdiv((uint64_t)n_a * 16, 256)), dim3(256), 0, st,
                               h->d_read_tile0.as<uint32_t>(), tile_off_p, A.cand_b, r_begin, n_a, paired,
                               h->d_vlabel.as<uint32_t>(), dfo, G);
            if (sort_lds > 48 * 1024)
                HIP_TRY(h, hipFuncSetAttribute(reinterpret_cast<const void*>(po::k_read_sort),
                                               hipFuncAttributeMaxDynamicSharedMemorySize, (int)sort_lds));
            PO_TRY(ws(h->d_vrank, (size_t)n_a * 4));
            hipLaunchKernelGGL(po::k_read_sort, dim3(1), dim3(po::SORT_BLOCK), sort_lds, st, h->d_vlabel.as<uint32_t>(), n_a,
                               shift, n_bins, h->d_vrank.as<uint32_t>());
            hipLaunchKernelGGL(po::k_read_invert, dim3(cdiv(n_a, 256)), dim3(256), 0, st, h->d_vrank.as<uint32_t>(), n_a, r_begin,
                               h->d_vperm.as<uint32_t>());
            perm = h->d_vperm.as<uint32_t>();
        }
        const uint32_t ver_grid = perm ? 8 * ((n_a + 7) / 8) : n_a;
        auto verify = paired == 2u ? (staged ? po::k_verify_a<BITS, true, true> : po::k_verify_a<BITS, true, false>)
                                   : (staged ? po::k_verify_a<BITS, false, true> : po::k_verify_a<BITS, false, false>);
        if (a.streamed) verify = staged ? po::k_verify_a<BITS, false, true, BITS == 2> : po::k_verify_a<BITS, false, false, BITS == 2>;
        const uint32_t lds_words = (lds_words_raw + 1u) & ~1u;
        const size_t ver_lds = (size_t)lds_words * 8 + (size_t)po::VREC_CAP * sizeof(po::VRec) + 16;
        if (ver_lds > 48 * 1024)
            HIP_TRY(h, hipFuncSetAttribute(reinterpret_cast<const void*>(verify), hipFuncAttributeMaxDynamicSharedMemorySize, (int)ver_lds));
        if (pair_events) HIP_TRY(h, hipEventRecord(h->ev[EV_VER0], st));
        hipLaunchKernelGGL(verify, dim3(ver_grid), dim3(po::VER_BLOCK), ver_lds, st,
                           words, woff, len, h->d_read_tile0.as<uint32_t>(), tile_off_p, A.cand_p,
                           A.cand_b, r_begin, lds_words, paired_ver,
                           h->n_exc_uploaded ? h->d_exc_off.as<uint32_t>() : nullptr, h->d_exc_pos.as<uint32_t>(),
                           h->d_exc_byte.as<uint8_t>(), h->d_type.as<uint8_t>(), perm, n_a, G,
                           sel_in_verify ? selfrep : nullptr, sel_in_verify ? n_deferred : nullptr);
        if (pair_events) HIP_TRY(h, hipEventRecord(h->ev[EV_VER1], st));
        return PO_OK;
    }

    po_status select_local() {
        ver_timed = true;
        HIP_TRY(h, hipGetLastError());
#ifdef PO_VSTAMPS
        {
            unsigned long long v[64 * 8], z[64 * 8] = {};
            HIP_TRY(h, hipStreamSynchronize(st));
            HIP_TRY(h, hipMemcpyFromSymbol(v, HIP_SYMBOL(po::g_vstamps), sizeof(v)));
            HIP_TRY(h, hipMemcpyToSymbol(HIP_SYMBOL(po::g_vstamps), z, sizeof(z)));
            double sum[8] = {};
            for (int i = 0; i < 64; ++i) for (int k = 0; k < 8; ++k) sum[k] += (double)v[i * 8 + k];
            if (sum[6] > 0)
                std::fprintf(stderr, "[vstamps] per wave (shader clocks): setup %.0f  wait_b %.0f  lds+cmp %.0f  book+init %.0f  life %.0f | iterations %.1f  group-steps/iteration %.2f  waves %.0f\n",
                             sum[0] / sum[6], sum[1] / sum[6], sum[2] / sum[6], sum[3] / sum[6], sum[4] / sum[6], sum[5] / sum[6], sum[7] / sum[5], sum[6]);
        }
#endif
        if (phase_events) HIP_TRY(h, hipEventRecord(h->ev[EV_VERIFY], st));
        if ((own_lists || dpE) && !sel_in_verify) {
            static_assert(po::SEL_CAP == 512, "k_select_local hashes to 9 bits");
            hipLaunchKernelGGL(po::k_select_local, dim3(cdiv(r_end - r_begin, 256 / po::WAVE)), dim3(256), 0, st,
                               h->d_read_tile0.as<uint32_t>(), tile_off_p, A.cand_p, A.cand_b, h->d_type.as<uint8_t>(),
                               r_begin, r_end - r_begin, selfrep, n_deferred, G);
        }
        const bool gated_ok = !n_selfrep_reads || (own_lists && n_cand < (16u << 20));
        const bool home_tail_ok = h->home_on && !a.want_cands && !dpE && !sw.tail_classic && gated_ok &&
                                  cdiv(n_cand, po::TAIL_TILE) <= po::TAIL_MAX_TILES;
        if (home_tail_ok && !async_count && h->spare_rows.cap < (size_t)n_cand * sizeof(po::Cand))
            PO_TRY(ws(h->spare_rows, (size_t)n_cand * sizeof(po::Cand) + (a.streamed ? 65536 : 0), false));
        compact_tail = home_tail_ok && h->spare_rows.p && h->spare_rows.cap >= (size_t)n_cand * sizeof(po::Cand);
        can_tail = compact_tail ||
                   (!a.want_cands && !dpE && h->spare_rows.p && h->spare_rows.cap >= worst_rows * sizeof(po_row) && gated_ok &&
                    cdiv(n_cand, po::TAIL_TILE) <= (a.streamed || h->home_on ? po::TAIL_MAX_TILES : 4096u) && !sw.tail_classic);
        if (async_count && !can_tail) return fail(h, PO_ERR_HIP, "internal: a piece with a predicted candidate count needs the fused tail");
        return PO_OK;
    }

    po_status fused_tail() {
        const uint32_t n_tt = cdiv(n_cand, po::TAIL_TILE);
        if (((size_t)po::TAIL_MAX_TILES + 4) * 4 > h->d_tail_state.cap) {
            PO_TRY(ws(h->d_tail_state, ((size_t)po::TAIL_MAX_TILES + 4) * 4));
            HIP_TRY(h, hipMemsetAsync(h->d_tail_state.p, 0, h->d_tail_state.cap, st));
        }
        uint32_t* tile_rows = h->d_tail_state.as<uint32_t>();
        uint32_t* tail_done = tile_rows + po::TAIL_MAX_TILES;
        const uint32_t* tgate = n_selfrep_reads ? n_deferred : nullptr;
        hipLaunchKernelGGL(compact_tail ? po::k_tile_rows<true> : po::k_tile_rows<false>, dim3(n_tt), dim3(po::TAIL_BLOCK), 0, st, A.cand_a,
                           A.cand_b, h->d_type.as<uint8_t>(), n_cand, paired, tgate, tile_rows, G);
        if (phase_events) HIP_TRY(h, hipEventRecord(h->ev[EV_SELECT], st));
        rows_late = true;
        used_tail = true;
        S.fused_tail = 1;
        res->d_rows = h->spare_rows;
        h->spare_rows = DevBuf();
        tail_zone = async_count ? zone : 48;
        h->pinned[tail_zone] = 0;
        h->pinned[tail_zone + 7] = 0;
        if (compact_tail) {
            res->compact = true;
            hipLaunchKernelGGL(po::k_tail_cands, dim3(n_tt), dim3(po::TAIL_BLOCK), 0, st, A.cand_a, A.cand_p, A.cand_b, h->d_type.as<uint8_t>(),
                               n_cand, res->d_rows.as<po::Cand>(), paired, tgate, tile_rows, n_tt, tail_done,
                               scalars + 3, h->pinned_dev + tail_zone, G, h->home_sh_b, h->home_sh_p);
        } else
        hipLaunchKernelGGL(po::k_tail, dim3(n_tt), dim3(po::TAIL_BLOCK), 0, st, A.cand_a, A.cand_p, A.cand_b, h->d_type.as<uint8_t>(),
                           n_cand, len, res->d_rows.as<po::Row>(), (uint32_t)BITS, paired, tgate, tile_rows, n_tt, tail_done,
                           scalars + 4, h->pinned_dev + tail_zone, G);
        HIP_TRY(h, hipGetLastError());
        return PO_OK;
    }

    po_status classic_tail() {
        po::PairSlot* ptab = nullptr;
        uint32_t pbits = 0;
        const uint32_t* gate = nullptr;
        uint64_t n_rows64 = 0;
        if (n_selfrep_reads) {
            uint32_t n_sus;
            if (own_lists && n_cand < (4u << 20)) {
                n_sus = n_cand;
                gate = n_deferred;
            } else {
                uint32_t* n_suspect = reinterpret_cast<uint32_t*>(scalars + 2) + 1;
                hipLaunchKernelGGL(po::k_count_suspects, dim3(std::min<uint32_t>(cdiv(n_cand, 256), (uint32_t)h->n_cu * 8)), dim3(256), 0,
                                   st, A.cand_b, h->d_type.as<uint8_t>(), n_cand, selfrep, n_suspect);
                HIP_TRY(h, hipMemcpyAsync(h->pinned + 8, scalars + 2, 8, hipMemcpyDeviceToHost, st));
                HIP_TRY(h, hipStreamSynchronize(st));
                n_sus = (uint32_t)(h->pinned[8] >> 32);
            }
            if (n_sus) {
                pbits = 4;
                while ((1ull << pbits) < 2ull * n_sus) ++pbits;
                PO_TRY(ws_piece(h->d_pair_key, ((size_t)1 << pbits) * sizeof(po::PairSlot)));
                hipLaunchKernelGGL(po::k_fill_gated, dim3((uint32_t)h->n_cu * 8), dim3(256), 0, st, h->d_pair_key.as<uint4>(),
                                   (uint64_t)((size_t)1 << pbits) * sizeof(po::PairSlot) / 16, 0xFFFFFFFFu, gate);
                ptab = h->d_pair_key.as<po::PairSlot>();
                hipLaunchKernelGGL(po::k_select_mark, dim3(cdiv(n_cand, 256)), dim3(256), 0, st, A.cand_a, A.cand_p, A.cand_b,
                                   h->d_type.as<uint8_t>(), n_cand, selfrep, ptab, pbits, gate);
            }
        }
        if (a.want_cands) PO_TRY(ws(h->d_flag, (size_t)n_cand));
        hipLaunchKernelGGL(po::k_select, dim3(cdiv(n_cand, 256)), dim3(256), 0, st, A.cand_a, A.cand_p, A.cand_b,
                           h->d_type.as<uint8_t>(), n_cand, selfrep, ptab, pbits, paired, h->d_rowcnt.as<uint8_t>(),
                           a.want_cands ? h->d_flag.as<uint8_t>() : nullptr, gate);
        HIP_TRY(h, hipGetLastError());
        if (!a.want_cands) {
            PO_TRY(prefix<uint8_t>(h->d_rowcnt.as<uint8_t>(), n_cand, h->d_row_off.as<uint32_t>(), &h->pinned[2]));
            if (phase_events) HIP_TRY(h, hipEventRecord(h->ev[EV_SELECT], st));
            rows_late = h->spare_rows.p && h->spare_rows.cap >= worst_rows * sizeof(po_row);
            if (!rows_late) {
                HIP_TRY(h, hipStreamSynchronize(st));
                n_rows64 = h->pinned[2];
                if (n_rows64 >= 0xFFFFFF00ull) return fail(h, PO_ERR_CAPACITY, "row count exceeds one call's capacity (2^32)");
            }
            PO_TRY(take_row_buffer(h, res, rows_late, n_rows64, worst_rows, a.streamed));
            if (dpE)
                hipLaunchKernelGGL(po::k_emit_ex, dim3(std::min<uint32_t>(cdiv(n_cand, 256), (uint32_t)h->n_cu * 16)), dim3(256), 0,
                                   st, A.cand_a, A.cand_p, A.cand_b, h->d_type.as<uint8_t>(), h->d_end_a.as<uint32_t>(),
                                   h->d_end_b.as<uint32_t>(), h->d_row_off.as<uint32_t>(), n_cand, len,
                                   res->d_rows.as<po::Row>(), (uint32_t)BITS, scalars + 4);
            else
            hipLaunchKernelGGL(po::k_emit, dim3(std::min<uint32_t>(cdiv(n_cand, 256), (uint32_t)h->n_cu * 16)), dim3(256), 0,
                               st, A.cand_a, A.cand_p, A.cand_b, h->d_type.as<uint8_t>(), h->d_row_off.as<uint32_t>(),
                               n_cand, len, res->d_rows.as<po::Row>(), (uint32_t)BITS, paired, scalars + 4);
            HIP_TRY(h, hipGetLastError());
            return PO_OK;
        }
        PO_TRY(prefix<uint8_t>(h->d_flag.as<uint8_t>(), n_cand, h->d_row_off.as<uint32_t>(), &h->pinned[3]));
        if (phase_events) HIP_TRY(h, hipEventRecord(h->ev[EV_SELECT], st));
        po::Cand* dst;
        uint64_t dst_cap;
        if (res->ext_dst && res->ext_cap && !sw.compact_sync) {
            dst = static_cast<po::Cand*>(res->ext_dst);
            dst_cap = res->ext_cap;
            cands_late = true;
            cands_ext = true;
        } else if (h->spare_cands.p && h->spare_cands.cap >= (size_t)n_cand * sizeof(po::Cand) && !sw.compact_sync) {
            res->d_rows = h->spare_cands;
            h->spare_cands = DevBuf();
            dst = res->d_rows.as<po::Cand>();
            dst_cap = n_cand;
            cands_late = true;
        } else {
            HIP_TRY(h, hipStreamSynchronize(st));
            const uint64_t n_ver = h->pinned[3];
            if (res->ext_dst && n_ver <= res->ext_cap) {
                dst = static_cast<po::Cand*>(res->ext_dst);
                res->wrote_ext = true;
            } else {
                if (h->spare_cands.p && h->spare_cands.cap >= n_ver * sizeof(po::Cand)) {
                    res->d_rows = h->spare_cands;
                    h->spare_cands = DevBuf();
                }
                PO_TRY(ws(res->d_rows, std::max<size_t>(n_ver * sizeof(po::Cand), 256), false));
                dst = res->d_rows.as<po::Cand>();
            }
            dst_cap = n_ver;
        }
        cands_cap = dst_cap;
        hipLaunchKernelGGL(po::k_compact, dim3(cdiv(n_cand, 256)), dim3(256), 0, st, A.cand_a, A.cand_p, A.cand_b,
                           h->d_type.as<uint8_t>(), h->d_flag.as<uint8_t>(), h->d_row_off.as<uint32_t>(), n_cand, dst,
                           (uint32_t)std::min<uint64_t>(dst_cap, 0xFFFFFFFFull));
        HIP_TRY(h, hipGetLastError());
        res->elem = sizeof(po::Cand);
        return PO_OK;
    }

    po_status tail_fallback() {
        h->spare_rows = res->d_rows;
        res->d_rows = DevBuf();
        res->compact = false;
        rows_late = false;
        used_tail = false;
        S.fused_tail = 0;
        S.tail_fallback = 1;
        return classic_tail();
    }

    po_status no_candidates() {
        if (phase_events) HIP_TRY(h, hipEventRecord(h->ev[EV_FILL], st));
        if (phase_events) HIP_TRY(h, hipEventRecord(h->ev[EV_VERIFY], st));
        if (phase_events) HIP_TRY(h, hipEventRecord(h->ev[EV_SELECT], st));
        return PO_OK;
    }

    po_status finish() {
        if (pair_events) HIP_TRY(h, hipEventRecord(h->ev[EV_EMIT], st));
        if (!used_tail) HIP_TRY(h, hipMemcpyAsync(h->pinned + 4, scalars + 4, 4 * sizeof(uint64_t), hipMemcpyDeviceToHost, st));
        res->unique_twins = !a.want_cands && paired != 0 && !dpE;
        HIP_TRY(h, hipEventRecord(h->ev[EV_DONE], st));
        h->st_selfclean = self_clean && used_tail;
        if (async_count && h->st_pend.valid) {
            HIP_TRY(h, hipEventSynchronize(h->st_pend.ev[EV_DONE]));
            PO_TRY(h->st_harvest());
        }
        if (a.streamed && rows_late && h->st_harvest && !h->st_pend.valid) {
            po_handle::Pending& P = h->st_pend;
            P.tail = used_tail;
            P.compact = res->compact;
            P.zone = tail_zone;
            P.cap_c = async_count ? cap_c : 0u;
            P.valid = true;
            P.k = a.shard;
            P.S = S;
            P.ver_timed = ver_timed;
            P.full_events = phase_events;
            P.pair_events = pair_events;
            P.ev = h->ev;
            res->count = 0;
            return PO_OK;
        }
        HIP_TRY(h, hipStreamSynchronize(st));
        if (async_count) return fail(h, PO_ERR_HIP, "internal: a piece with a predicted count must stay pending");
        if (used_tail && h->pinned[tail_zone + 7]) {
            PO_TRY(tail_fallback());
            HIP_TRY(h, hipEventRecord(h->ev[EV_EMIT], st));
// ... 2129 lines not shown
        reg_thread = std::thread([blocks, &fmark] {
            for (int k = 0; k < 2; ++k)
                if (blocks[k]) RegAlloc<uint64_t>::reg_now(blocks[k]);
            fmark("stores registered");
        });
    } catch (const std::system_error&) {
    }
    struct RegJoin {
        std::thread& t;
        po_handle* h;
        ~RegJoin() {
            if (t.joinable()) t.join();
            else
                for (int k = 0; k < 2; ++k)
                    if (h->words[k].capacity()) RegAlloc<uint64_t>::reg_now(h->words[k].data());
        }
    } reg_join{reg_thread, h};
    const uint8_t* lut = g_lut.v;
    const unsigned char* comp = comp_table();
    std::atomic<size_t> next{0};
    std::atomic<int> bad{0};
    auto pack = [&](const unsigned char* sq, size_t n, uint64_t* w) -> uint8_t {
        uint8_t b = 0;
        const size_t full = n / 32;
        for (size_t k = 0; k < full; ++k) {
            const unsigned char* q = sq + k * 32;
            uint64_t acc = 0;
            for (int j = 0; j < 32; ++j) {
                const uint8_t c = lut[q[j]];
                b |= c;
                acc |= (uint64_t)(c & 3) << (2 * j);
            }
            w[k] = acc;
        }
        if (full * 32 < n) {
            uint64_t acc = 0;
            for (size_t i = full * 32; i < n; ++i) {
                const uint8_t c = lut[sq[i]];
                b |= c;
                acc |= (uint64_t)(c & 3) << (2 * (i & 31));
            }
            w[full] = acc;
        }
        return b;
    };
    auto worker = [&]() {
      try {
        std::string seq, rc;
        for (;;) {
            const size_t lo = next.fetch_add(64);
            if (lo >= recs.size() || bad.load(std::memory_order_relaxed)) return;
            const size_t hi = std::min(recs.size(), lo + 64);
            for (size_t i = lo; i < hi; ++i) {
                const FastaRec& r = recs[i];
                seq.clear();
                seq.reserve(r.seq_len);
                for (const char* p = r.seq_begin; p < r.seq_end;) {
                    const char* nl = static_cast<const char*>(std::memchr(p, '\n', (size_t)(r.seq_end - p)));
                    size_t n = nl ? (size_t)(nl - p) + 1 : (size_t)(r.seq_end - p);
                    const char* q = p;
                    size_t m = n;
                    trim_seq_line(q, m);
                    seq.append(q, m);
                    p += n;
                }
                const size_t n = seq.size();
                if (n != r.seq_len) {
                    bad.store(1);
                    return;
                }
                rc.resize(n);
                for (size_t k = 0; k < n; ++k) rc[k] = (char)comp[(unsigned char)seq[n - 1 - k]];
                const size_t nw = (n + 31) / 32;
                for (int k = 0; k < 2; ++k) {
                    const size_t prev_end = i ? off[2 * (i - 1) + k] + (recs[i - 1].seq_len + 31) / 32 + 1 : old_words[k];
                    if (off[2 * i + k] > prev_end) words[k][off[2 * i + k] - 1] = 0;
                    words[k][off[2 * i + k] + nw] = 0;
                }
                uint8_t b = pack(reinterpret_cast<const unsigned char*>(seq.data()), n, words[0] + off[2 * i]);
                b |= pack(reinterpret_cast<const unsigned char*>(rc.data()), n, words[1] + off[2 * i + 1]);
                if (n != r.seq_len || (b & 0x80)) {
                    bad.store(1);
                    return;
                }
            }
        }
      } catch (...) {
        bad.store(1);
      }
    };
    {
        const unsigned hw = std::max(1u, cpu_share() > 3 ? cpu_share() - 2 : cpu_share());
        const unsigned n_thr = std::max(1u, std::min(hw, 16u));
        std::vector<std::thread> thr;
        try {
            for (unsigned t = 1; t < n_thr; ++t) thr.emplace_back(worker);
        } catch (const std::system_error&) {
        }
        worker();
        for (auto& th : thr) th.join();
    }
    fmark("packed");
    if (bad.load()) {
        h->words[0].resize(old_words[0]);
        h->words[1].resize(old_words[1]);
        return false;
    }
    h->ids.reserve(h->ids.size() + 2 * recs.size());
    for (size_t i = 0; i < recs.size(); ++i) {
        std::string id(recs[i].name, recs[i].name_len);
        id.push_back('+');
        h->ids.push_back(id);
        id.back() = '-';
        h->ids.push_back(std::move(id));
        for (int k = 0; k < 2; ++k) {
            h->len.push_back((uint32_t)recs[i].seq_len);
            h->woff.push_back(off[2 * i + k]);
            h->exc_off.push_back((uint32_t)h->exc_pos.size());
        }
        h->total_bases += 2 * recs[i].seq_len;
    }
    h->dirty = true;
    h->ids_paired = -1;
    if (n_records) *n_records = recs.size();
    fmark("ids and tables appended");
    return true;
}

}

extern "C" {

int po_abi_version(void) { return PO_ABI_VERSION; }

po_status po_create(po_handle** out) {
    if (!out) return PO_ERR_INVALID;
    po_handle* h = new (std::nothrow) po_handle();
    if (!h) return PO_ERR_NOMEM;
    *out = h;
    return PO_OK;
}

void po_destroy(po_handle* h) {
    if (!h) return;
    if (h->dev_ready) {
        (void)hipSetDevice(h->device);
        (void)hipStreamSynchronize(h->stream);
        DevBuf* bufs[] = {&h->d_words, &h->d_woff, &h->d_len, &h->d_tiles, &h->d_read_tile0, &h->d_left, &h->d_left_cnt, &h->d_tile_extra, &h->d_exc_off, &h->d_exc_pos, &h->d_exc_byte, &h->d_pair_state, &h->d_truemask,
                          &h->d_table, &h->d_slot_cnt, &h->d_slot_cur, &h->d_slot_start, &h->d_read_slot, &h->d_chain,
                          &h->d_chain_tmp, &h->d_long_list, &h->d_entry_off, &h->d_bloom, &h->d_selfrep, &h->d_tile_count, &h->d_tile_off,
                          &h->d_ps_blocks, &h->d_scalars, &h->d_cand_a, &h->d_cand_p, &h->d_cand_b, &h->d_type,
                          &h->d_rowcnt, &h->d_row_off, &h->d_flag, &h->d_pair_key, &h->d_pair_min, &h->spare_rows, &h->spare_cands, &h->spare_edges, &h->spare_nrank,
                          &h->d_vlabel, &h->d_vrank, &h->d_vperm, &h->d_end_a, &h->d_end_b, &h->d_dpcnt, &h->d_lay_len, &h->d_lay_cnt, &h->d_rflag, &h->d_removed, &h->d_ekey, &h->d_ecnt,
                          &h->d_ewin, &h->d_eoff, &h->d_chain_state, &h->d_tail_state, &h->d_efirst, &h->d_lay_firstc};
        if (h->copy_stream) (void)hipStreamSynchronize(h->copy_stream);
        if (h->up_stream) (void)hipStreamSynchronize(h->up_stream);
        if (h->rc_stream) (void)hipStreamSynchronize(h->rc_stream);
        for (DevBuf* b : bufs) b->release();
        for (DevBuf& b : h->d_red) b.release();
        for (DevBuf& b : h->d_tip) b.release();
        for (DevBuf& b : h->d_mrg) b.release();
        for (DevBuf& b : h->d_cov) b.release();
        for (DevBuf& b : h->d_rank) b.release();
        for (DevBuf& b : h->d_cc) b.release();
        for (DevBuf& b : h->d_scc) b.release();
        for (DevBuf& b : h->d_sb) b.release();
        for (DevBuf& b : h->d_bc) b.release();
        for (DevBuf& b : h->d_ct) b.release();
        for (DevBuf& b : h->d_ph) b.release();
        const bool pooled = kit_give(h);
        if (!pooled) {
        for (int i = 0; i < 2 * EV_N; ++i) (void)hipEventDestroy(h->ev_sets[i / EV_N][i % EV_N]);
        for (hipEvent_t e : h->ev_lay)
            if (e) (void)hipEventDestroy(e);
        (void)hipEventDestroy(h->ev_up0);
        (void)hipEventDestroy(h->ev_up1);
        if (h->pinned) {
            pin_drop(h->pinned);
            (void)hipHostFree(h->pinned);
        }
        }
        h->spare_host.release();
        h->scratch_host.release();
        h->home_stage.release();
        for (DevBuf& b : h->chunk_rows) b.release();
        h->d_first.release();
        h->d_defer.release();
        h->meta_host.release();
        h->stage_host.release();
        for (void* c : h->arena_chunks) (void)hipFree(c);
        h->arena_chunks.clear();
        if (!pooled) {
        if (h->up_stream) {
            (void)hipStreamSynchronize(h->up_stream);
            (void)hipStreamDestroy(h->up_stream);
        }
        for (hipEvent_t e : h->ev_piece)
            if (e) (void)hipEventDestroy(e);
        for (hipEvent_t e : h->ev_rc)
            if (e) (void)hipEventDestroy(e);
        if (h->ev_meta) (void)hipEventDestroy(h->ev_meta);
        if (h->rc_stream) {
            (void)hipStreamSynchronize(h->rc_stream);
            (void)hipStreamDestroy(h->rc_stream);
        }
        if (h->ev_first) (void)hipEventDestroy(h->ev_first);
        if (h->copy_stream) {
            (void)hipStreamSynchronize(h->copy_stream);
            (void)hipStreamDestroy(h->copy_stream);
        }
        (void)hipStreamDestroy(h->stream);
        }
    }
    h->spare_host.release();
    h->home_stage.release();
    delete h;
}

po_status po_set_device(po_handle* h, int device) {
    if (!h) return PO_ERR_INVALID;
    if (h->dev_ready && device != h->device) return fail(h, PO_ERR_INVALID, "device already initialised");
    h->device = device;
    return PO_OK;
}

po_status po_add_sequence(po_handle* h, const char* id, size_t id_len, const char* seq, size_t seq_len) {
    if (!h || (!id && id_len) || (!seq && seq_len)) return PO_ERR_INVALID;
    if (h->segments_only) return fail(h, PO_ERR_INVALID, "this handle holds GFA segments (no sequences); use a new handle");
    if (seq_len > 0x7FFFFFF0ull) return fail(h, PO_ERR_CAPACITY, "read longer than 2^31 bases");
    if (h->len.size() >= 0xFFFFFFF0ull) return fail(h, PO_ERR_CAPACITY, "too many reads");
    quiesce_store(h);
    try {
        const unsigned char* s = reinterpret_cast<const unsigned char*>(seq);
        if (h->bits != 2 || !append_packed(h, s, seq_len, 2)) {
            if (h->bits == 2) widen_to_bytes(h);
            append_packed(h, s, seq_len, 8);
        }
        h->ids.emplace_back(id ? id : "", id_len);
        h->len.push_back((uint32_t)seq_len);
        h->total_bases += seq_len;
        h->dirty = true;
        h->ids_paired = -1;
        if (h->total_bases >= h->pool_bases && h->total_bases >= (64ull << 20)) result_pool_grow(h);
        if (h->bits == 2 && h->first_n + 1 == h->len.size()) note_first_words(h);
        if (h->bits == 2 && (h->len.size() & 1) == 0) {
            const size_t r = h->len.size() - 1;
            if (!h->exc_pos.empty()) host_pair_check(h, r, s);
            const bool has_exc = h->exc_off[r - 1] != h->exc_off[r] || h->exc_off[r] != h->exc_off[r + 1];
            if (h->all_pairs_rcx) {
                const bool ok = has_exc ? (h->pair_state.size() > r / 2 && h->pair_state[r / 2] == 1) : packed_is_revcomp(h, r);
                h->all_pairs_rcx = ok;
                if (has_exc || !ok) h->all_pairs_rc = false;
            } else {
                h->all_pairs_rc = false;
            }
        }
    } catch (const std::bad_alloc&) {
        return fail(h, PO_ERR_NOMEM, "out of host memory in po_add_sequence");
    }
    return PO_OK;
}

po_status po_add_fasta(po_handle* h, const char* path, int both_strands, uint64_t* n_records) {
    if (!h || !path) return PO_ERR_INVALID;
    if (n_records) *n_records = 0;
    quiesce_store(h);
    if (both_strands && !h->segments_only && !getenv("PHASM_FASTA_SEQUENTIAL")) {
        const int fd = ::open(path, O_RDONLY);
        if (fd < 0) return fail(h, PO_ERR_INVALID, std::string("cannot open ") + path);
        struct stat sb;
        bool done = false;
        if (::fstat(fd, &sb) == 0 && sb.st_size > 0) {
            void* m = ::mmap(nullptr, (size_t)sb.st_size, PROT_READ, MAP_PRIVATE, fd, 0);
            if (m != MAP_FAILED) {
                std::thread warm;
                if ((uint64_t)sb.st_size >= (32ull << 20) && !h->dev_ready && !getenv("PHASM_NO_POOL") && !getenv("PHASM_NO_WARM")) {
                    const uint64_t est_bases = 2ull * (uint64_t)sb.st_size;
                    try {
                        warm = std::thread([h, est_bases] {
                            if (h->total_bases + est_bases >= h->pool_bases) result_pool_grow(h, h->total_bases + est_bases);
                        });
                    } catch (const std::system_error&) {
                    }
                }
                struct Joiner {
                    std::thread& t;
                    ~Joiner() {
                        if (t.joinable()) t.join();
                    }
                } joiner{warm};
                try {
                    const auto tf0 = std::chrono::steady_clock::now();
                    done = add_fasta_parallel(h, static_cast<const char*>(m), (size_t)sb.st_size, n_records);
                    if (getenv("PHASM_FASTA_TRACE")) {
                        const double t_parse = std::chrono::duration<double, std::milli>(std::chrono::steady_clock::now() - tf0).count();
                        if (warm.joinable()) warm.join();
                        std::fprintf(stderr, "[fasta] parsed and packed in %.1f ms; the device and the result pool were ready %.1f ms after the start\n", t_parse,
                                     std::chrono::duration<double, std::milli>(std::chrono::steady_clock::now() - tf0).count());
                    }
                } catch (const std::bad_alloc&) {
                    ::munmap(m, (size_t)sb.st_size);
                    ::close(fd);
                    return fail(h, PO_ERR_NOMEM, "out of host memory in po_add_fasta");
                } catch (const std::system_error&) {
                    done = false;
                }
                ::munmap(m, (size_t)sb.st_size);
// ... 383 lines not shown
    sum.tail_fallback += S.tail_fallback;
    sum.n_predicted += S.n_predicted;
    sum.ms_index += S.ms_index;
    sum.ms_scan_count += S.ms_scan_count;
    sum.ms_scan_fill += S.ms_scan_fill;
    sum.ms_verify += S.ms_verify;
    sum.ms_select += S.ms_select;
    sum.ms_emit += S.ms_emit;
    sum.ms_total += S.ms_total;
    sum.ms_scan_probe += S.ms_scan_probe;
    sum.ms_verify_kernel += S.ms_verify_kernel;
}

po_status run_chunk(po_handle* h, const OverlapArgs& a, uint64_t* nk) {
    const uint32_t k = a.shard;
    po_result part;
    part.h = h;
    if (h->chunk_rows[k].p) {
        h->spare_rows.release();
        h->spare_rows = h->chunk_rows[k];
        h->chunk_rows[k] = DevBuf();
    }
    const po_status st = h->bits == 2 ? run_overlaps<2>(h, a, &part) : run_overlaps<8>(h, a, &part);
    h->chunk_rows[k] = part.d_rows;
    h->chunk_compact[k] = part.compact;
    part.d_rows = DevBuf();
    *nk = part.count;
    return st;
}

bool stream_eligible(const po_handle* h, uint32_t min_length) {
    const uint32_t n = (uint32_t)h->len.size();
    if (!h->dirty || h->bits != 2 || n < 4 || (n % 2) != 0 || !h->all_pairs_rcx) return false;
    if (h->asm_pieces) return false;
    if (getenv("PHASM_FULL_UPLOAD") || getenv("PHASM_NO_MIRROR")) return false;
    bool want = n >= 4096 && h->words[0].size() * 8 >= (16ull << 20);
    if (const char* e = getenv("PHASM_STREAM")) want = atoi(e) != 0;
    if (!want) return false;
    const uint32_t m = min_length ? min_length : 1;
    const uint64_t n_elig = count_eligible(const_cast<po_handle*>(h), m);
    if (n_elig == 0) return false;
    return true;
}

std::vector<uint32_t> stream_bounds(const po_handle* h) {
    const uint32_t n = (uint32_t)h->len.size();
    const uint64_t bytes0 = (uint64_t)h->words[0].size() * 8;
    uint64_t max_pieces = h->chunk_rows[0].p ? 12 : 8;
    const bool big = bytes0 >= (512ull << 20) && h->chunk_rows[0].p;
    if (big) max_pieces = 15;
    if (const char* e = getenv("PHASM_STREAM_MAX_PIECES")) max_pieces = (uint64_t)std::max(2, std::min(PO_MAX_PIECES - 1, atoi(e)));
    const uint32_t n_pieces = (uint32_t)std::min<uint64_t>(max_pieces, std::max<uint64_t>(2, (bytes0 + (8ull << 20)) / (16ull << 20)));
    const double skew = big ? 1.6 : 1.25;
    std::vector<uint32_t> cuts;
    for (uint32_t i = 1; i < n_pieces; ++i) cuts.push_back((uint32_t)(1000.0 * (1.0 - std::pow(1.0 - (double)i / n_pieces, skew))));
    if (const char* e = getenv("PHASM_STREAM_CUTS")) {
        cuts.clear();
        for (const char* q = e; *q;) {
            char* endp = nullptr;
            const long v = strtol(q, &endp, 10);
            if (endp == q) break;
            if (v > 0 && v < 1000 && (cuts.empty() || (uint32_t)v > cuts.back()) && cuts.size() + 1 < (size_t)PO_MAX_PIECES) cuts.push_back((uint32_t)v);
            q = *endp ? endp + 1 : endp;
        }
    }
    std::vector<uint32_t> b{0};
    const uint64_t total = h->words[0].size();
    for (uint32_t c : cuts) {
        const uint64_t target = total * c / 1000;
        uint32_t lo = 0, hi = n / 2;
        while (lo < hi) {
            const uint32_t mid = (lo + hi) / 2;
            if (h->woff[2 * (size_t)mid] >= target) hi = mid; else lo = mid + 1;
        }
        if (2 * lo > b.back() && 2 * lo < n) b.push_back(2 * lo);
    }
    b.push_back(n);
    return b;
}

po_status stream_begin(po_handle* h, const std::vector<uint32_t>& bounds) {
    const uint32_t n = (uint32_t)h->len.size();
    const uint32_t P = (uint32_t)bounds.size() - 1;
    bool generate = false;
    if (!h->up_stream) HIP_TRY(h, hipStreamCreateWithFlags(&h->up_stream, hipStreamNonBlocking));
    for (uint32_t k = 0; k < P; ++k)
        if (!h->ev_piece[k]) HIP_TRY(h, hipEventCreate(&h->ev_piece[k]));
    auto queue_piece = [&](uint32_t k) -> po_status {
        uint64_t* dw = h->d_words.as<uint64_t>();
        const uint64_t wb = bounds[k] < n ? h->woff[bounds[k]] : h->words[0].size();
        const uint64_t we = bounds[k + 1] < n ? h->woff[bounds[k + 1]] : h->words[0].size();
        if (we > wb) {
            HIP_TRY(h, hipMemcpyAsync(dw + wb, h->words[0].data() + wb, (we - wb) * 8, hipMemcpyHostToDevice, h->up_stream));
            h->upload_bytes += (we - wb) * 8;
        }
        HIP_TRY(h, hipEventRecord(h->ev_piece[k], h->up_stream));
        return PO_OK;
    };
    PO_TRY(upload_meta(h, &generate));
    if (!generate) return fail(h, PO_ERR_INVALID, "streamed step on reads that are not (x, reverse complement of x) pairs");
    uint64_t* dw = h->d_words.as<uint64_t>();
    if (h->poison >= 0) {
        HIP_TRY(h, hipEventRecord(h->ev_up1, h->stream));
        HIP_TRY(h, hipStreamWaitEvent(h->up_stream, h->ev_up1, 0));
    }
    HIP_TRY(h, hipEventRecord(h->ev_up0, h->up_stream));
    PO_TRY(queue_piece(0));
    if (P > 1) {
        const uint32_t r0 = h->st_early_index ? 0u : bounds[1];
        if (h->st_lead > 2) {
            note_lead_words(h);
            PO_TRY(ensure(h, h->d_first, (size_t)n * LEAD_WORDS * 8));
            HIP_TRY(h, hipMemcpyAsync(h->d_first.as<uint64_t>() + (size_t)LEAD_WORDS * r0, h->lead_words.data() + (size_t)LEAD_WORDS * r0,
                                      (size_t)(n - r0) * LEAD_WORDS * 8, hipMemcpyHostToDevice, h->stream));
            h->upload_bytes += (size_t)(n - r0) * LEAD_WORDS * 8;
            hipLaunchKernelGGL(po::k_scatter_lead, dim3(cdiv((uint64_t)(n - r0) * LEAD_WORDS, 256)), dim3(256), 0, h->stream, dw,
                               h->d_woff.as<uint64_t>(), h->d_len.as<uint32_t>(), h->d_first.as<uint64_t>(), LEAD_WORDS, r0, n);
        } else {
            note_first_words(h);
            PO_TRY(ensure(h, h->d_first, (size_t)n * 16));
            HIP_TRY(h, hipMemcpyAsync(h->d_first.as<uint64_t>() + 2 * (size_t)r0, h->first_words.data() + 2 * (size_t)r0,
                                      (size_t)(n - r0) * 16, hipMemcpyHostToDevice, h->stream));
            h->upload_bytes += (size_t)(n - r0) * 16;
            hipLaunchKernelGGL(po::k_scatter_first, dim3(cdiv(n - r0, 256)), dim3(256), 0, h->stream, dw, h->d_woff.as<uint64_t>(),
                               h->d_first.as<ulonglong2>(), r0, n);
        }
        HIP_TRY(h, hipGetLastError());
        if (!h->ev_first) HIP_TRY(h, hipEventCreateWithFlags(&h->ev_first, hipEventDisableTiming));
        HIP_TRY(h, hipEventRecord(h->ev_first, h->stream));
        HIP_TRY(h, hipStreamWaitEvent(h->up_stream, h->ev_first, 0));
    }
    for (uint32_t k = 1; k < P; ++k) PO_TRY(queue_piece(k));
    HIP_TRY(h, hipEventRecord(h->ev_up1, h->up_stream));
    if (!h->rc_stream) HIP_TRY(h, hipStreamCreateWithFlags(&h->rc_stream, hipStreamNonBlocking));
    if (!h->ev_meta) HIP_TRY(h, hipEventCreateWithFlags(&h->ev_meta, hipEventDisableTiming));
    HIP_TRY(h, hipEventRecord(h->ev_meta, h->stream));
    HIP_TRY(h, hipStreamWaitEvent(h->rc_stream, h->ev_meta, 0));
    for (uint32_t k = 0; k < P; ++k) {
        if (!h->ev_rc[k]) HIP_TRY(h, hipEventCreateWithFlags(&h->ev_rc[k], hipEventDisableTiming));
        HIP_TRY(h, hipStreamWaitEvent(h->rc_stream, h->ev_piece[k], 0));
        const uint32_t p0 = bounds[k] / 2, p1 = bounds[k + 1] / 2;
        if (p1 > p0)
            hipLaunchKernelGGL(po::k_revcomp_store, dim3(cdiv((uint64_t)(p1 - p0) * 64, 256)), dim3(256), 0, h->rc_stream, dw,
                               h->d_woff.as<uint64_t>(), h->d_len.as<uint32_t>(), p0, p1,
                               h->n_exc_uploaded ? h->d_exc_off.as<uint32_t>() : nullptr, h->d_exc_pos.as<uint32_t>());
        HIP_TRY(h, hipGetLastError());
        HIP_TRY(h, hipEventRecord(h->ev_rc[k], h->rc_stream));
    }
    h->st_defer_cap = std::max<uint32_t>(1u << 16, h->defer_need + h->defer_need / 2);
    if (const char* e = getenv("PHASM_DEFER_CAP")) h->st_defer_cap = (uint32_t)std::max(1, atoi(e));
    PO_TRY(ensure(h, h->d_defer, (size_t)h->st_defer_cap * sizeof(po::Cand) + 16));
    if (!getenv("PHASM_DEFER_CAP")) h->st_defer_cap = (uint32_t)std::min<size_t>((h->d_defer.cap - 16) / sizeof(po::Cand), 0xFFFFFF00u);
    HIP_TRY(h, hipMemsetAsync(h->d_defer.as<char>() + (size_t)h->st_defer_cap * sizeof(po::Cand), 0, 16, h->stream));
    h->paired = true;
    ++h->upload_gen;
    h->dirty = false;
    return PO_OK;
}

po_status overlaps_streamed(po_handle* h, uint32_t min_length, HostRows& R, po_stats& sum, bool* overflow) {
    *overflow = false;
    const uint32_t n = (uint32_t)h->len.size();
    const std::vector<uint32_t> bounds = stream_bounds(h);
    const uint32_t P = (uint32_t)bounds.size() - 1;
    const bool trace = getenv("PHASM_STREAM_TRACE") != nullptr;
    const auto t_start = std::chrono::steady_clock::now();
    auto since = [&]() { return std::chrono::duration<double, std::milli>(std::chrono::steady_clock::now() - t_start).count(); };
    std::vector<uint32_t> sig(bounds);
    sig.push_back(min_length);
    sig.push_back((uint32_t)(h->total_bases & 0xFFFFFFFFu));
    h->st_pred_valid = h->st_pred_valid && sig == h->st_pred_sig;
    uint64_t new_pred[PO_MAX_PIECES] = {};
    h->st_selfclean = false;
    h->st_early_index = P > 1 && h->poison < 0 && !getenv("PHASM_NO_INDEX_REUSE") && !getenv("PHASM_LATE_INDEX");
    h->st_lead = index_flavour(h, min_length ? min_length : 1, true, LEAD_WORDS, OverlapSwitches()).ww >= 4 && !getenv("PHASM_STREAM_LEAD2") ? LEAD_WORDS : 2u;
    PO_TRY(stream_begin(h, bounds));
    auto piece_args = [&](uint32_t k) {
        OverlapArgs a{min_length, k, P};
        a.streamed = true;
        a.r_begin = bounds[k];
        a.r_end = bounds[k + 1];
        return a;
    };
    if (trace) std::fprintf(stderr, "[stream] %u pieces queued at %.3f ms\n", P, since());
    if (h->st_early_index) {
        po_result part;
        part.h = h;
        OverlapArgs a = piece_args(0);
        a.idx_only = true;
        const po_status ist = run_overlaps<2>(h, a, &part);
        part.d_rows.release();
        if (ist != PO_OK) {
            (void)hipStreamSynchronize(h->stream);
            (void)hipStreamSynchronize(h->up_stream);
            (void)hipStreamSynchronize(h->rc_stream);
            h->dirty = true;
            return ist;
        }
    }
    uint64_t* dw = h->d_words.as<uint64_t>();
    po_status st = PO_OK;
    auto completed = [&](uint32_t k, const po_stats& S, uint64_t nk) -> po_status {
        add_stats(sum, S);
        new_pred[k] = S.n_candidates;
        const double seen = (double)bounds[k + 1] / (double)n;
        if (h->chunk_compact[k]) PO_TRY(append_home(h, R, h->chunk_rows[k], S.n_verified, nk, k, P, seen * seen));
        else PO_TRY(append_rows(h, R, h->chunk_rows[k], nk, k, P, seen * seen));
        if (trace) {
            float up = 0;
            (void)hipEventElapsedTime(&up, h->ev_up0, h->ev_piece[k]);
            std::fprintf(stderr, "[stream] piece %u reads [%u, %u): landed %.3f ms after the first copy started, rows counted at %.3f ms (device %.3f ms: scan %.3f verify %.3f), %llu rows (%.1f MB) queued for home\n",
                         k, bounds[k], bounds[k + 1], up, since(), S.ms_total, S.ms_scan_count + S.ms_scan_fill, S.ms_verify,
                         (unsigned long long)nk, nk * 24e-6);
        }
        return PO_OK;
    };
    h->st_pend.valid = false;
    bool tail_gave_up = false;
    h->st_harvest = [&]() -> po_status {
        const uint32_t k = h->st_pend.k;
        bool needs_classic = false;
        const uint64_t nk = finish_piece(h, &needs_classic);
        if (needs_classic) {
            tail_gave_up = true;
            return PO_OK;
        }
        return completed(k, h->st_pend.S, nk);
    };
    if (getenv("PHASM_STREAM_SYNC")) h->st_harvest = nullptr;
    for (uint32_t k = 0; k < P && st == PO_OK; ++k) {
        if (hipStreamWaitEvent(h->stream, h->ev_rc[k], 0) != hipSuccess) { st = fail(h, PO_ERR_HIP, "hipStreamWaitEvent"); break; }
        OverlapArgs a = piece_args(k);
        {
            const double mine = (double)bounds[k + 1] * bounds[k + 1] - (double)bounds[k] * bounds[k];
            for (uint32_t j = k + 1; j < P; ++j)
                a.ws_scale = std::max(a.ws_scale, ((double)bounds[j + 1] * bounds[j + 1] - (double)bounds[j] * bounds[j]) / mine * 1.1);
        }
        h->ev = h->ev_sets[k & 1];
        uint64_t nk = 0;
        st = run_chunk(h, a, &nk);
        if (st != PO_OK || tail_gave_up) break;
        if (h->st_pend.valid && h->st_pend.k == k) continue;
        if (h->st_pend.valid) {
            if (hipStreamSynchronize(h->stream) != hipSuccess) { st = fail(h, PO_ERR_HIP, "stream"); break; }
            st = h->st_harvest();
            if (st != PO_OK) break;
        }
        st = completed(k, h->stats, nk);
    }
    if (st == PO_OK && h->st_pend.valid && !tail_gave_up) {
        if (hipStreamSynchronize(h->stream) != hipSuccess) st = fail(h, PO_ERR_HIP, "stream");
        else st = h->st_harvest();
    }
    h->st_harvest = nullptr;
    h->st_pend.valid = false;
    h->ev = h->ev_sets[0];
    if (st == PO_OK && tail_gave_up) {
        (void)hipStreamSynchronize(h->stream);
        (void)hipStreamSynchronize(h->up_stream);
        (void)hipStreamSynchronize(h->rc_stream);
        h->dirty = true;
        h->st_tail_gave_up = true;
        h->st_pred_valid = false;
        *overflow = true;
        return PO_OK;
    }
    if (st != PO_OK) {
        (void)hipStreamSynchronize(h->up_stream);
        (void)hipStreamSynchronize(h->rc_stream);
        h->dirty = true;
        h->st_pred_valid = false;
        return st;
    }
    h->st_pred_sig = sig;
    std::memcpy(h->st_pred_cand, new_pred, sizeof(new_pred));
    h->st_pred_valid = true;
    float ms = 0;
    (void)hipEventSynchronize(h->ev_up1);
    (void)hipEventElapsedTime(&ms, h->ev_up0, h->ev_up1);
    h->stats.ms_upload = ms;
    HIP_TRY(h, hipMemcpyAsync(h->pinned + 40, h->d_defer.as<char>() + (size_t)h->st_defer_cap * sizeof(po::Cand), 8,
                              hipMemcpyDeviceToHost, h->stream));
    HIP_TRY(h, hipStreamSynchronize(h->stream));
    const uint32_t n_def = (uint32_t)h->pinned[40];
    h->defer_need = n_def;
    if (n_def > h->st_defer_cap) {
        *overflow = true;
        return PO_OK;
    }
    if (n_def) {
        hipStream_t s = h->stream;
        po::Cand* list = h->d_defer.as<po::Cand>();
        PO_TRY(ensure(h, h->d_rowcnt, (size_t)n_def));
        PO_TRY(ensure(h, h->d_row_off, ((size_t)n_def + 1) * 4));
        HIP_TRY(h, hipEventRecord(h->ev[EV_START], s));
        hipLaunchKernelGGL(po::k_verify_flat, dim3(cdiv((uint64_t)n_def * 64, 256)), dim3(256), 0, s, dw, h->d_woff.as<uint64_t>(),
                           h->d_len.as<uint32_t>(), list, n_def, h->n_exc_uploaded ? h->d_exc_off.as<uint32_t>() : nullptr,
                           h->d_exc_pos.as<uint32_t>(), h->d_exc_byte.as<uint8_t>());
        hipLaunchKernelGGL(po::k_deferred_rowcnt, dim3(cdiv(n_def, 256)), dim3(256), 0, s, list, n_def, 1u, h->d_rowcnt.as<uint8_t>());
        HIP_TRY(h, hipGetLastError());
        PO_TRY(prefix_sum<uint8_t>(h, h->d_rowcnt.as<uint8_t>(), n_def, h->d_row_off.as<uint32_t>(), &h->pinned[2]));
        HIP_TRY(h, hipStreamSynchronize(s));
        const uint64_t n_rows = h->pinned[2];
        if (n_rows) {
            PO_TRY(ensure(h, h->chunk_rows[P], n_rows * sizeof(po_row)));
            unsigned long long* scalars = h->d_scalars.as<unsigned long long>();
            HIP_TRY(h, hipMemsetAsync(scalars + 4, 0, 32, s));
            hipLaunchKernelGGL(po::k_emit_cands, dim3(std::min<uint32_t>(cdiv(n_def, 256), (uint32_t)h->n_cu * 16)), dim3(256), 0, s,
                               list, h->d_rowcnt.as<uint8_t>(), h->d_row_off.as<uint32_t>(), n_def, h->d_len.as<uint32_t>(),
                               h->chunk_rows[P].as<po::Row>(), 2u, 1u, scalars + 4);
            HIP_TRY(h, hipGetLastError());
            HIP_TRY(h, hipMemcpyAsync(h->pinned + 4, scalars + 4, 4 * sizeof(uint64_t), hipMemcpyDeviceToHost, s));
            HIP_TRY(h, hipEventRecord(h->ev[EV_EMIT], s));
            HIP_TRY(h, hipStreamSynchronize(s));
            float ms_def = 0;
            (void)hipEventElapsedTime(&ms_def, h->ev[EV_START], h->ev[EV_EMIT]);
            sum.n_verified += h->pinned[4];
            sum.sum_overlap_bases += h->pinned[5];
            sum.verify_bytes_algo += h->pinned[6];
            sum.verify_bytes_exec += h->pinned[7];
            sum.n_rows += n_rows;
            sum.ms_verify += ms_def;
            sum.ms_total += ms_def;
            PO_TRY(append_rows(h, R, h->chunk_rows[P], n_rows, P, P + 1));
        }
    }
    (void)n;
    if (trace) {
        std::fprintf(stderr, "[stream] deferred list settled at %.3f ms (%u candidates)\n", since(), n_def);
        (void)hipStreamSynchronize(h->copy_stream);
        std::fprintf(stderr, "[stream] last row home at %.3f ms\n", since());
    }
    return PO_OK;
}

}
}

po_status po_overlaps_to_host(po_handle* h, uint32_t min_length, po_result** out) {
    if (!h || !out) return PO_ERR_INVALID;
    *out = nullptr;
    if (h->segments_only) return fail(h, PO_ERR_INVALID, "this handle holds GFA segments without sequences: nothing to overlap");
    uint32_t n_chunks = (h->len.size() >= 8192 && h->total_bases >= (64ull << 20)) ? 4u : 1u;
    if (const char* e = getenv("PHASM_HOST_CHUNKS")) n_chunks = (uint32_t)std::max(1, std::min(4, atoi(e)));
    po_result* r = new (std::nothrow) po_result();
    if (!r) return fail(h, PO_ERR_NOMEM, "out of host memory");
    r->h = h;
    po_status st = PO_OK;
    HostRows R;
    po_stats sum = {};
    bool streamed = false, overflowed = false;
    float ms_upload = 0;
    try {
        st = init_device(h);
        if (st == PO_OK && !h->copy_stream && hipStreamCreateWithFlags(&h->copy_stream, hipStreamNonBlocking) != hipSuccess)
            st = fail(h, PO_ERR_HIP, "cannot create the copy stream");
        if (st == PO_OK && h->spare_host.p) {
            R.hb = h->spare_host;
            h->spare_host = HostBuf();
        }
        if (st == PO_OK) {
            (void)home_begin(h);
            h->home_last_bytes = 0;
        }
        if (st == PO_OK && stream_eligible(h, min_length)) {
            bool overflow = false;
            st = overlaps_streamed(h, min_length, R, sum, &overflow);
            ms_upload = h->stats.ms_upload;
            if (st == PO_OK && !overflow) {
                streamed = true;
            } else if (st == PO_OK) {
                overflowed = true;
                home_wait(h);
                if (h->home_on) {
                    home::g_pool->sum_l.store(0);
                    home::g_pool->sum_b.store(0);
                    home::g_pool->sum_e.store(0);
                }
                if (hipStreamSynchronize(h->copy_stream) != hipSuccess) st = fail(h, PO_ERR_HIP, "copy stream");
                R.total = 0;
                sum = po_stats();
            }
        }
        if (st == PO_OK && !streamed) st = upload(h);
        for (uint32_t k = 0; k < n_chunks && st == PO_OK && !streamed; ++k) {
            uint64_t nk = 0;
            st = run_chunk(h, OverlapArgs{min_length, k, n_chunks}, &nk);
            if (st != PO_OK) break;
            add_stats(sum, h->stats);
            st = h->chunk_compact[k] ? append_home(h, R, h->chunk_rows[k], h->stats.n_verified, nk, k, n_chunks)
                                     : append_rows(h, R, h->chunk_rows[k], nk, k, n_chunks);
        }
    } catch (const std::bad_alloc&) {
        st = fail(h, PO_ERR_NOMEM, "out of host memory in po_overlaps_to_host");
    }
    h->st_harvest = nullptr;
    h->st_pend.valid = false;
    h->ev = h->ev_sets[0];
    if (h->dev_ready) (void)hipStreamSynchronize(h->stream);
    if (h->up_stream) (void)hipStreamSynchronize(h->up_stream);
    if (h->rc_stream) (void)hipStreamSynchronize(h->rc_stream);
    if (h->copy_stream && hipStreamSynchronize(h->copy_stream) != hipSuccess && st == PO_OK) st = fail(h, PO_ERR_HIP, "row copy device->host");
    {
        const int herr = home_end(h, &sum);
        if (herr && st == PO_OK)
            st = fail(h, PO_ERR_HIP, herr == 1 ? "internal: the host's row count of a piece differs from the device's"
                                     : herr == 2 ? "internal: a verified-candidate record names a read the handle does not hold"
                                                 : "the event behind a device->host copy of records failed");
    }
    if (st != PO_OK) {
        R.hb.release();
        delete r;
        return st;
    }
    po_stats& S = h->stats;
    S.n_candidates = sum.n_candidates;
    S.n_verified = sum.n_verified;
    S.n_rows = sum.n_rows;
    S.sum_overlap_bases = sum.sum_overlap_bases;
    S.verify_bytes_algo = sum.verify_bytes_algo;
    S.verify_bytes_exec = sum.verify_bytes_exec;
    S.n_tiles = sum.n_tiles;
    S.shard_bases = sum.shard_bases;
    S.ms_index = sum.ms_index;
    S.ms_scan_count = sum.ms_scan_count;
    S.ms_scan_fill = sum.ms_scan_fill;
    S.ms_verify = sum.ms_verify;
    S.ms_select = sum.ms_select;
    S.ms_emit = sum.ms_emit;
    S.ms_total = sum.ms_total;
    S.ms_scan_probe = sum.ms_scan_probe;
    S.ms_verify_kernel = sum.ms_verify_kernel;
    S.fused_tail = sum.fused_tail;
// ... 997 lines not shown
```

phasm_amd/csrc/kernels.hip.h:

```cpp
#pragma once
#include <hip/hip_runtime.h>
#include <stdint.h>

namespace po {

using u32x4 = __attribute__((ext_vector_type(4))) uint32_t;

constexpr uint32_t NO_SELFREP = 0xFFFFFFFFu;
constexpr uint64_t KEY_EMPTY = ~0ull;
constexpr int WAVE = 64;

#ifndef PO_VER_PAD
#define PO_VER_PAD 0
#endif
#ifndef PO_SCAN_PAD
#define PO_SCAN_PAD 0
#endif
template <int N>
__device__ __forceinline__ void valu_pad(uint32_t& r, uint32_t c) {
#pragma unroll
    for (int i = 0; i < N; ++i) asm volatile("v_xor_b32 %0, %0, %1" : "+v"(r) : "v"(c));
}

struct CandGuard {
// ... 895 lines not shown
        const uint32_t p0 = (rec.word0 + lane) * W;
        if (have_tile && rec.la >= m && p0 <= rec.la - m) {
            hitmask = filter_tile<BITS, FULLK>(s_bloom, A.bloom_log2, w0, w1, kmask);
            const uint32_t nvalid = rec.la - m - p0 + 1;
            if (nvalid < (uint32_t)W) hitmask &= (1u << nvalid) - 1u;
        }
        PO_STAMP(st2);
        asm volatile("s_waitcnt vmcnt(3)" : "+v"(ps0), "+v"(ps1), "+v"(ps2), "+v"(ps3), "+v"(pt0), "+v"(pt1), "+v"(pt2), "+v"(pt3)
                     : : "memory");
        PO_STAMP(st3);
        if (prev_t != 0xFFFFFFFFu) {
            auto settle = [&](uint64_t key, uint32_t home, uint32_t src, bool on, const u32x4& q0, const u32x4& q1,
                              const u32x4& q2, const u32x4& q3) __attribute__((always_inline)) -> uint32_t {
                const uint32_t klo = (uint32_t)key, khi = (uint32_t)(key >> 32);
                auto stops = [&](const u32x4& q) __attribute__((always_inline)) -> bool {
                    return q.w == 0 || (q.x == klo && q.y == khi);
                };
                const bool h0 = stops(q0), h1 = stops(q1), h2 = stops(q2), h3 = stops(q3);
                u32x4 s = q3;
                if (h2) s = q2;
                if (h1) s = q1;
                if (h0) s = q0;
                const bool settled = h0 | h1 | h2 | h3;
                const bool hard = on && (!settled || (s.w != 0 && !(s.w & SLOT_SINGLE)));
                const bool deferred = defer(hard, prev_t, src);
                uint32_t n = 0;
                if (on && !deferred) {
                    if (!settled) {
                        uint32_t j = (home + PROBE_GROUP - 1u) & tmask;
                        while (s.w != 0 && (((uint64_t)s.y << 32) | s.x) != key) {
                            j = (j + 1u) & tmask;
                            s = *reinterpret_cast<const u32x4*>(&table[j]);
                        }
                    }
                    if (s.w != 0) n = count_slot(s, prev_a, prev_la, (prev_word0 + (src >> 8)) * W + (src & 255u));
                    if (n) atomicOr(&tm[src >> 8], 1u << (src & 255u));
                }
                return n;
            };
            uint32_t n = settle(pk, pidx, psrc, pon, ps0, ps1, ps2, ps3);
            if (extra) n += settle(pk2, pidx2, psrc2, pon2, pt0, pt1, pt2, pt3);
            wave_lds_fence();
            truemask[(size_t)prev_t * WAVE + lane] = tm[lane];
            tm[lane] = 0;
            n = __any(n > 1u) ? wave_sum(n) : (uint32_t)__popcll(__ballot(n != 0u));
            if (lane == 0) tile_count[prev_t] = n;
        }
        PO_STAMP(st4);
        if (!have_tile) return false;
        const uint32_t nh = __popc(hitmask);
        const uint32_t incl = wave_incl_scan(nh);
        const uint32_t total = read_last_lane(incl);
        uint32_t rank = incl - nh;
        while (hitmask && rank < 2u * WAVE) {
            const uint32_t sft = __ffs(hitmask) - 1;
            hitmask &= hitmask - 1;
            qs[rank] = (lane << 8) | sft;
            ++rank;
        }
        while (__any(hitmask != 0)) {
            const bool want = hitmask != 0;
            const uint32_t sft = want ? __ffs(hitmask) - 1 : 0;
            const bool ok = defer(want, t, (lane << 8) | sft);
            if (!__any(ok)) break;
            if (ok) hitmask &= hitmask - 1;
        }
        uint32_t ovf_n = 0;
        while (hitmask) {
            const uint32_t sft = __ffs(hitmask) - 1;
            hitmask &= hitmask - 1;
            const uint64_t kmer = funnel(w0, w1, sft * BITS) & kmask;
            uint32_t z = 0, w = 0;
            table_probe(table, tbits, kmer, z, w);
            if (w) {
                const uint32_t nn = count_slot(u32x4{0, 0, z, w}, rec.read, rec.la, p0 + sft);
                if (nn) {
                    atomicOr(&tm[lane], 1u << sft);
                    ovf_n += nn;
                }
            }
        }
        wave_lds_fence();
        auto request = [&](uint32_t src, bool on, uint64_t& key, uint32_t& home, u32x4& q0, u32x4& q1, u32x4& q2,
                           u32x4& q3) __attribute__((always_inline)) {
            const uint32_t sl = src >> 8;
            const uint32_t x0 = __shfl((uint32_t)w0, sl, WAVE), x1 = __shfl((uint32_t)(w0 >> 32), sl, WAVE);
            const uint32_t x2 = __shfl((uint32_t)w1, sl, WAVE), x3 = __shfl((uint32_t)(w1 >> 32), sl, WAVE);
            const uint32_t sh = (src & 255u) * BITS;
            const bool up = sh >= 32u;
            uint32_t lo = __builtin_amdgcn_alignbit(up ? x2 : x1, up ? x1 : x0, sh);
            uint32_t hi = __builtin_amdgcn_alignbit(up ? x3 : x2, up ? x2 : x1, sh);
            if constexpr (!FULLK) {
                lo &= (uint32_t)kmask;
                hi &= (uint32_t)(kmask >> 32);
            }
            const uint64_t kmer = ((uint64_t)hi << 32) | lo;
            uint32_t idx = narrow_home((lo ^ ((hi << 13) | (hi >> 19))) * 0x9E3779B1u, tbits);
            if (kmer == KEY_EMPTY) idx = tmask + 1u;
            if (!on) idx = 0;
            key = kmer;
            home = idx;
            const Slot* g = &table[idx];
            q0 = ld16(g);
            asm volatile("global_load_dwordx4 %0, %1, off offset:16" : "=v"(q1) : "v"(g) : "memory");
            asm volatile("global_load_dwordx4 %0, %1, off offset:32" : "=v"(q2) : "v"(g) : "memory");
            asm volatile("global_load_dwordx4 %0, %1, off offset:48" : "=v"(q3) : "v"(g) : "memory");
        };
        pon = lane < total;
        psrc = pon ? qs[lane] : 0u;
        request(psrc, pon, pk, pidx, ps0, ps1, ps2, ps3);
        extra = total > (uint32_t)WAVE;
        if (extra) {
            pon2 = lane + (uint32_t)WAVE < total;
            psrc2 = pon2 ? qs[WAVE + lane] : 0u;
            request(psrc2, pon2, pk2, pidx2, pt0, pt1, pt2, pt3);
        }
        wave_lds_fence();
        if (__any(ovf_n != 0)) {
            const uint32_t e = wave_sum(ovf_n);
            if (lane == 0) atomicAdd(&A.tile_extra[t], e);
        }
        prev_t = t;
        prev_a = rec.read;
        prev_la = rec.la;
        prev_word0 = rec.word0;
        t = tn;
        rec = rec1;
#ifdef PO_STAMPS
        PO_STAMP(st5);
        acc_s[0] += st1 - st0;
        acc_s[1] += st2 - st1;
        acc_s[2] += st3 - st2;
        acc_s[3] += st4 - st3;
        acc_s[4] += st5 - st4;
        acc_s[5] += 1;
#endif
        return true;
    };
    while (pass(wa, wb) && pass(wb, wa)) {
    }
    asm volatile("s_waitcnt vmcnt(0)" ::: "memory");
    if (lane == 0) A.left_cnt[blockIdx.x * nwaves + wave] = left_n;
#ifdef PO_STAMPS
    if (A.dbg && lane == 0) {
        unsigned long long* o = A.dbg + (size_t)(blockIdx.x * nwaves + wave) * 8;
        for (int k = 0; k < 6; ++k) o[k] = acc_s[k];
    }
#endif
}

template <int BITS, bool STREAM = false>
__global__ void k_scan_fixup(const ScanArgs A, uint32_t n_waves, uint32_t clean) {
    constexpr int W = 64 / BITS;
    const uint32_t wv = blockIdx.x;
    if (wv >= n_waves) return;
    const uint32_t cnt = min(A.left_cnt[wv], LEFT_CAP);
    const uint2* __restrict__ list = A.left + (size_t)wv * LEFT_CAP;
    for (uint32_t k = threadIdx.x; k < cnt; k += blockDim.x) {
        const uint2 e = list[k];
        const uint32_t t = e.x, ln = e.y >> 8, sft = e.y & 255u;
        if (t < A.tile_begin || t >= A.tile_end || ln >= (uint32_t)WAVE || sft >= (uint32_t)W) continue;
        const TileRec rec = A.tiles[t];
        const uint64_t w0 = A.words[rec.wabs + ln], w1 = A.words[rec.wabs + ln + 1];
        const uint64_t kmer = funnel(w0, w1, sft * BITS) & A.kmask;
        uint32_t z = 0, w = 0;
        table_probe(A.table, A.tbits, kmer, z, w);
        if (!w) continue;
        const uint32_t a = rec.read, p = (rec.word0 + ln) * W + sft;
        if (p > 0) {
            if (w & SLOT_SINGLE) {
                if (z == a) note_selfrep(A.selfrep, a, p, A.n_selfrep);
            } else {
                for (uint32_t j = 0; j < w; ++j)
                    if (A.chain[z + j] == a) note_selfrep(A.selfrep, a, p, A.n_selfrep);
            }
        }
        uint32_t n = 0;
        for_each_candidate<STREAM>(A.chain, A.len, A.paired, z, w, a, rec.la - p, [&](uint32_t, uint32_t, uint32_t) { ++n; });
        if (n) {
            atomicOr(&A.truemask[(size_t)t * WAVE + ln], 1u << sft);
            atomicAdd(&A.tile_count[t], n);
        }
    }
    if (clean) {
        __syncthreads();
        if (threadIdx.x == 0) A.left_cnt[wv] = 0;
    }
}

__global__ void k_add_extra(uint32_t* __restrict__ tile_count, const uint32_t* __restrict__ tile_extra, uint32_t t0, uint32_t t1) {
    const uint32_t t = t0 + blockIdx.x * blockDim.x + threadIdx.x;
    if (t < t1 && tile_extra[t]) tile_count[t] += tile_extra[t];
}

#ifndef PO_FILL_TILES
#define PO_FILL_TILES 8
#endif
constexpr int FILL_TILES = PO_FILL_TILES;

template <int BITS, bool STREAM = false>
__global__ __launch_bounds__(256) void k_scan_fill(const ScanArgs A, const CandGuard G) {
    constexpr int W = 64 / BITS;
    __shared__ uint32_t q_src[4 * WAVE];
    __shared__ TileRec q_rec[4 * FILL_TILES];
    if (G.overflow()) return;
    const uint32_t lane = lane_id(), wave = threadIdx.x >> 6;
    uint32_t* qs = q_src + wave * WAVE;
    TileRec* qr = q_rec + wave * FILL_TILES;
    const uint32_t t0 = __builtin_amdgcn_readfirstlane(A.tile_begin + (blockIdx.x * 4 + wave) * FILL_TILES);
    if (t0 >= A.tile_end) return;
    uint32_t hm[FILL_TILES], rk[FILL_TILES];
#pragma unroll
    for (int i = 0; i < FILL_TILES; ++i) hm[i] = t0 + i < A.tile_end ? A.truemask[(size_t)(t0 + i) * WAVE + lane] : 0u;
    if (lane < (uint32_t)FILL_TILES) qr[lane] = A.tiles[min(t0 + lane, A.tile_end - 1)];
    uint32_t out = A.tile_off[t0];
    uint32_t total = 0;
#pragma unroll
    for (int i = 0; i < FILL_TILES; ++i) {
        const uint32_t nh = __popc(hm[i]);
        const uint32_t incl = wave_incl_scan(nh);
        rk[i] = total + incl - nh;
        total += read_last_lane(incl);
    }
    if (total == 0) return;
    for (uint32_t r0 = 0; r0 < total; r0 += WAVE) {
#pragma unroll
        for (int i = 0; i < FILL_TILES; ++i) {
            while (hm[i] && rk[i] < r0 + WAVE) {
                const uint32_t sft = __ffs(hm[i]) - 1;
                hm[i] &= hm[i] - 1;
                qs[rk[i] - r0] = ((uint32_t)i << 16) | (lane << 8) | sft;
                ++rk[i];
            }
        }
        wave_lds_fence();
        const bool has = r0 + lane < total;
        const uint32_t src = has ? qs[lane] : 0u;
        const TileRec rec = qr[src >> 16];
        wave_lds_fence();
        const uint32_t ln = (src >> 8) & 255u, sft = src & 255u;
        uint32_t z = 0, w = 0;
        if (has) {
            const uint64_t w0 = A.words[rec.wabs + ln], w1 = A.words[rec.wabs + ln + 1];
            table_probe(A.table, A.tbits, funnel(w0, w1, sft * BITS) & A.kmask, z, w);
        }
        const uint32_t a = rec.read, la = rec.la;
        const uint32_t p = (rec.word0 + ln) * W + sft;
        uint32_t n = 0;
        if (w) for_each_candidate<STREAM>(A.chain, A.len, A.paired, z, w, a, la - p, [&](uint32_t, uint32_t, uint32_t) { ++n; });
        const uint32_t inc = wave_incl_scan(n);
        uint32_t off = out + inc - n;
        if (n) {
            for_each_candidate<STREAM>(A.chain, A.len, A.paired, z, w, a, la - p, [&](uint32_t b, uint32_t, uint32_t) {
                A.cand_a[off] = a;
                A.cand_p[off] = p;
                A.cand_b[off] = b;
                ++off;
            });
        }
        out += read_last_lane(inc);
    }
}

struct DeferOut {
    const uint32_t* cand_p;
    uint32_t b_limit;
    uint4* list;
    uint32_t cap;
    uint32_t* counter;
};
__global__ __launch_bounds__(256) void k_read_label(const uint32_t* __restrict__ read_tile0, const uint32_t* __restrict__ tile_off,
                                                    const uint32_t* __restrict__ cand_b, uint32_t r_begin, uint32_t n_reads,
                                                    uint32_t paired, uint32_t* __restrict__ label, const DeferOut defer,
                                                    const CandGuard G) {
    const uint32_t t = blockIdx.x * blockDim.x + threadIdx.x;
    const uint32_t i = t >> 4, sub = t & 15u;
    if (i >= n_reads) return;
    if (G.overflow()) {
        if (sub == 0) label[i] = r_begin + i;
        return;
    }
    const uint32_t a = r_begin + i;
    const uint32_t seg0 = tile_off[read_tile0[a]], seg1 = tile_off[read_tile0[a + 1]];
    const bool reversed = (paired & 3u) == 3u;
    auto rank = [&](uint32_t x) { return reversed ? ~x : mirror_rank(x, paired); };
    uint32_t best = rank(a);
    for (uint32_t c = seg0 + sub; c < seg1; c += 16) {
        const uint32_t b = cand_b[c];
        best = max(best, rank(b ^ 1u));
        if (defer.list && b >= defer.b_limit) {
            const uint32_t k = atomicAdd(defer.counter, 1u);
            if (k < defer.cap) defer.list[k] = uint4{a, defer.cand_p[c], b, 0u};
        }
    }
#pragma unroll
    for (int o = 8; o >= 1; o >>= 1) best = max(best, (uint32_t)__shfl_xor((int)best, o, 16));
    if (paired == 2u) best = (__brev(best & 0xFFFFFF00u) << 8) | (best & 0xFFu);
    if (reversed) best = ~best;
    if (sub == 0) label[i] = best;
}

constexpr int SORT_BLOCK = 1024;
__global__ __launch_bounds__(SORT_BLOCK) void k_read_sort(const uint32_t* __restrict__ label, uint32_t n_reads, uint32_t shift,
                                                          uint32_t n_bins, uint32_t* __restrict__ rank) {
    extern __shared__ uint32_t s_bin[];
    uint32_t* s_wave = s_bin + n_bins;
    const uint32_t tid = threadIdx.x;
    for (uint32_t b = tid; b < n_bins; b += SORT_BLOCK) s_bin[b] = 0;
    __syncthreads();
    constexpr uint32_t UN = 16;
    for (uint32_t base = tid; base < n_reads; base += UN * SORT_BLOCK) {
        uint32_t v[UN];
#pragma unroll
        for (uint32_t k = 0; k < UN; ++k) {
            const uint32_t i = base + k * SORT_BLOCK;
            v[k] = i < n_reads ? label[i] : ~0u;
        }
#pragma unroll
        for (uint32_t k = 0; k < UN; ++k)
            if (v[k] != ~0u) atomicAdd(&s_bin[v[k] >> shift], 1u);
    }
    __syncthreads();
    const uint32_t per = (n_bins + SORT_BLOCK - 1) / SORT_BLOCK;
    const uint32_t lo = min(tid * per, n_bins), hi = min(lo + per, n_bins);
    uint32_t sum = 0;
    for (uint32_t b = lo; b < hi; ++b) sum += s_bin[b];
    const uint32_t incl = wave_incl_scan(sum);
    if (lane_id() == WAVE - 1) s_wave[tid >> 6] = incl;
    __syncthreads();
    uint32_t run = incl - sum;
    for (uint32_t w = 0; w < (tid >> 6); ++w) run += s_wave[w];
    for (uint32_t b = lo; b < hi; ++b) {
        const uint32_t v = s_bin[b];
        s_bin[b] = run;
        run += v;
    }
    __syncthreads();
    for (uint32_t base = tid; base < n_reads; base += UN * SORT_BLOCK) {
        uint32_t v[UN];
#pragma unroll
        for (uint32_t k = 0; k < UN; ++k) {
            const uint32_t i = base + k * SORT_BLOCK;
            v[k] = i < n_reads ? label[i] : ~0u;
        }
#pragma unroll
        for (uint32_t k = 0; k < UN; ++k)
            if (v[k] != ~0u) rank[base + k * SORT_BLOCK] = atomicAdd(&s_bin[v[k] >> shift], 1u);
    }
}

__global__ void k_read_invert(const uint32_t* __restrict__ rank, uint32_t n_reads, uint32_t r_begin, uint32_t* __restrict__ perm) {
    const uint32_t i = blockIdx.x * blockDim.x + threadIdx.x;
    if (i < n_reads && rank[i] < n_reads) perm[rank[i]] = r_begin + i;
}

__device__ inline bool exceptions_equal(const uint32_t* __restrict__ exc_off, const uint32_t* __restrict__ exc_pos,
                                        const uint8_t* __restrict__ exc_byte, uint32_t a, uint32_t p, uint32_t b,
                                        uint32_t n) {
    uint32_t ia = exc_off[a];
    const uint32_t ea = exc_off[a + 1];
    uint32_t ib = exc_off[b];
    const uint32_t eb = exc_off[b + 1];
    if (ia == ea && ib == eb) return true;
    {
        uint32_t lo = ia, hi = ea;
        while (lo < hi) {
            const uint32_t mid = (lo + hi) >> 1;
            if (exc_pos[mid] < p) lo = mid + 1; else hi = mid;
        }
        ia = lo;
    }
    for (;;) {
        const bool ha = ia < ea && exc_pos[ia] - p < n;
        const bool hb = ib < eb && exc_pos[ib] < n;
        if (!ha && !hb) return true;
        if (ha != hb) return false;
        if (exc_pos[ia] - p != exc_pos[ib] || exc_byte[ia] != exc_byte[ib]) return false;
        ++ia;
        ++ib;
    }
}

#ifndef PO_VER_GROUP
#define PO_VER_GROUP 16
#endif
constexpr int VER_GROUP = PO_VER_GROUP;
#ifndef PO_VER_BLOCK
#define PO_VER_BLOCK 256
#endif
constexpr int VER_BLOCK = PO_VER_BLOCK;
#ifndef PO_VER_BLOCKS
#define PO_VER_BLOCKS 3
#endif
#ifndef PO_VER_FIRST
#define PO_VER_FIRST PO_VER_BLOCKS
#endif
constexpr int VER_BLOCKS = PO_VER_BLOCKS;

#ifdef PO_VSTAMPS
__device__ unsigned long long g_vstamps[64 * 8];
#define VST(...) __VA_ARGS__
#else
#define VST(...)
#endif

constexpr int VREC_CAP = 512;
constexpr uint32_t SEL_CAP = 512;
__device__ __forceinline__ void select_read_list(uint32_t seg0, uint32_t seg1, const uint32_t* __restrict__ cand_p,
                                                 const uint32_t* __restrict__ cand_b, uint8_t* __restrict__ type,
                                                 uint32_t* __restrict__ selfrep, uint32_t* __restrict__ n_deferred,
                                                 uint32_t* key, uint32_t* mn, uint32_t lane);
struct __attribute__((aligned(16))) VRec {
    uint32_t pk;
    uint32_t b;
    uint32_t nk;
    uint32_t wo;
};

__device__ __forceinline__ uint32_t lds_draw(uint32_t* counter) {
    typedef __attribute__((address_space(3))) uint32_t lds_u32;
    const uint32_t addr = (uint32_t)(uintptr_t)(lds_u32*)counter;
    uint32_t old, one = 1u;
    asm volatile("ds_add_rtn_u32 %0, %1, %2\n\ts_waitcnt lgkmcnt(0)" : "=v"(old) : "v"(addr), "v"(one) : "memory");
    return old;
}

__device__ __forceinline__ uint32_t group_bcast0(uint32_t v, uint32_t gshift) {
    if constexpr (VER_GROUP == 16) {
        (void)gshift;
        return (uint32_t)__builtin_amdgcn_update_dpp(0, (int)v, 0x150, 0xf, 0xf, false);
    } else {
        return (uint32_t)__shfl((int)v, (int)gshift);
    }
}

template <int BITS, bool SCRAMBLED, bool IN_LDS, bool STAGED, bool STREAM = false>
__device__ __forceinline__ void verify_run(const uint64_t* __restrict__ words, const uint64_t* __restrict__ woff,
                                           const uint32_t* __restrict__ len, const uint32_t* __restrict__ cand_p,
                                           const uint32_t* __restrict__ cand_b, uint32_t paired,
                                           const uint32_t* __restrict__ exc_off, const uint32_t* __restrict__ exc_pos,
                                           const uint8_t* __restrict__ exc_byte, uint8_t* __restrict__ type,
                                           const uint32_t* __restrict__ s_a, const uint32_t* __restrict__ ga32,
                                           const VRec* __restrict__ s_rec, uint32_t* s_next, uint32_t a, uint32_t la,
                                           uint32_t seg0, uint32_t seg1
                                           VST(, unsigned long long vt_start, unsigned long long (&vt)[8])) {
    constexpr int W = 64 / BITS;
    (void)W;
    const uint32_t sub = threadIdx.x & (VER_GROUP - 1);
    const uint32_t gshift = (lane_id() / VER_GROUP) * VER_GROUP;
    constexpr uint32_t NGROUPS = VER_BLOCK / VER_GROUP;

    uint32_t c = seg0;
    uint32_t cA = seg0 + threadIdx.x / VER_GROUP, cB = cA + NGROUPS;
    bool have = cA < seg1;
    uint32_t nbits = 0, sh = 0, q = 0, d = 0, keep = 0, nblk_var = 1, cur_p = 0, cur_b = 0;
    uint32_t nd = 0;
    constexpr bool UNIFORM_STEPS = PO_VER_FIRST == PO_VER_BLOCKS;
    const uint32_t* B = reinterpret_cast<const uint32_t*>(words);
    const uint32_t c_last = seg1 - 1;
    uint32_t m0p = 0, m0b = 0, m0l = 0, m1p = 0, m1b = 0;
    uint64_t m0w = 0;
    if constexpr (!STAGED) {
        const uint32_t c0 = min(cA, c_last), c1 = min(cB, c_last);
        m0p = cand_p[c0];
        m0b = cand_b[c0];
        m1p = cand_p[c1];
        m1b = cand_b[c1];
        m0l = len[m0b];
        m0w = woff[m0b];
    }
    auto init = [&]() __attribute__((always_inline)) {
        uint32_t p, b, lb;
        uint64_t wo;
        if constexpr (STAGED) {
            c = cA;
            const VRec r = s_rec[c - seg0];
            p = r.pk;
            b = r.b;
            lb = r.nk;
            wo = r.wo;
            uint32_t drawn = 0;
            if (sub == 0) drawn = lds_draw(s_next);
            cA = group_bcast0(drawn, gshift);
        } else {
            p = m0p;
            b = m0b;
            lb = m0l;
            wo = m0w;
            c = cA;
            cA = cB;
            m0p = m1p;
            m0b = m1b;
            m0l = len[m1b];
            m0w = woff[m1b];
            uint32_t drawn = 0;
            if (sub == 0) drawn = lds_draw(s_next);
            cB = group_bcast0(drawn, gshift);
            const uint32_t c2 = min(cB, c_last);
            m1p = cand_p[c2];
            m1b = cand_b[c2];
// ... 780 lines not shown
}
__device__ __forceinline__ void chain_store(unsigned long long* p, unsigned long long v) {
    __hip_atomic_store(p, v, __ATOMIC_RELAXED, __HIP_MEMORY_SCOPE_AGENT);
}

__device__ __forceinline__ uint32_t chain_take_tile(ChainState* st, uint32_t* s_tile) {
    if (threadIdx.x == 0) *s_tile = atomicAdd(&st->ticket, 1u);
    __syncthreads();
    return *s_tile;
}

__device__ __forceinline__ unsigned long long chain_lookback(ChainState* st, uint32_t tile, unsigned long long aggregate) {
    const uint32_t lane = lane_id();
    if (lane == 0) chain_store(&st->status[tile], (tile == 0 ? CHAIN_PFX : CHAIN_AGG) | aggregate);
    unsigned long long prefix = 0;
    if (tile == 0) return 0;
    int64_t j = (int64_t)tile - 1;
    for (;;) {
        const int64_t idx = j - (int64_t)lane;
        unsigned long long v;
        for (;;) {
            v = idx >= 0 ? chain_load(&st->status[idx]) : CHAIN_PFX;
            if (!__any((v >> 62) == 0)) break;
            __builtin_amdgcn_s_sleep(1);
        }
        const uint64_t pm = __ballot((v >> 62) == 2);
        const uint32_t first = pm ? (uint32_t)__builtin_ctzll(pm) : 64u;
        unsigned long long part = lane <= first ? (v & CHAIN_VAL) : 0ull;
        part = wave_sum64(part);
        prefix += part;
        if (pm) break;
        j -= 64;
    }
    if (lane == 0) chain_store(&st->status[tile], CHAIN_PFX | (prefix + aggregate));
    return prefix;
}

__device__ __forceinline__ bool chain_finish(ChainState* st, uint32_t n_tiles, uint32_t* s_last) {
    __syncthreads();
    if (threadIdx.x == 0) *s_last = atomicAdd(&st->done, 1u) == n_tiles - 1u ? 1u : 0u;
    __syncthreads();
    const bool last = *s_last != 0u;
    if (last) {
        for (uint32_t i = threadIdx.x; i < n_tiles; i += blockDim.x) st->status[i] = 0;
        if (threadIdx.x == 0) {
            st->ticket = 0;
            st->done = 0;
        }
    }
    return last;
}

template <typename T>
__global__ __launch_bounds__(PS_BLOCK) void k_ps_chain(T* __restrict__ in, const uint32_t* __restrict__ extra, uint64_t n,
                                                       uint32_t* __restrict__ out, ChainState* __restrict__ st, uint32_t n_tiles,
                                                       uint64_t* __restrict__ total, uint64_t* __restrict__ total_host,
                                                       const uint64_t* __restrict__ also_src, uint64_t* __restrict__ also_host) {
    static_assert(PS_ITEMS == 16, "vector paths assume 16 items per thread");
    __shared__ uint32_t s_wave[PS_BLOCK / WAVE];
    __shared__ uint32_t s_tile, s_last;
    __shared__ unsigned long long s_prefix;
    const uint32_t tile = chain_take_tile(st, &s_tile);
    const uint64_t base = (uint64_t)tile * PS_TILE + (uint64_t)threadIdx.x * PS_ITEMS;
    const bool full = base + PS_ITEMS <= n;
    uint32_t v[PS_ITEMS];
    if (full && (reinterpret_cast<uintptr_t>(in + base) & 15u) == 0) {
        if constexpr (sizeof(T) == 1) {
            const u32x4 q = *reinterpret_cast<const u32x4*>(in + base);
            const uint32_t w[4] = {q.x, q.y, q.z, q.w};
#pragma unroll
            for (int k = 0; k < PS_ITEMS; ++k) v[k] = (w[k >> 2] >> (8 * (k & 3))) & 0xFFu;
        } else {
#pragma unroll
            for (int g = 0; g < 4; ++g) {
                const u32x4 q = *reinterpret_cast<const u32x4*>(in + base + 4 * g);
                v[4 * g] = q.x;
                v[4 * g + 1] = q.y;
                v[4 * g + 2] = q.z;
                v[4 * g + 3] = q.w;
            }
        }
    } else {
#pragma unroll
        for (int k = 0; k < PS_ITEMS; ++k) {
            const uint64_t i = base + k;
            v[k] = i < n ? (uint32_t)in[i] : 0u;
        }
    }
    if constexpr (sizeof(T) == 4) {
        if (extra) {
#pragma unroll
            for (int k = 0; k < PS_ITEMS; ++k) {
                const uint64_t i = base + k;
                const uint32_t e = i < n ? extra[i] : 0u;
                if (e) {
                    v[k] += e;
                    in[i] = v[k];
                }
            }
        }
    }
    uint32_t acc = 0;
#pragma unroll
    for (int k = 0; k < PS_ITEMS; ++k) acc += v[k];
    const uint32_t incl = wave_incl_scan(acc);
    if (lane_id() == WAVE - 1) s_wave[threadIdx.x >> 6] = incl;
    __syncthreads();
    uint32_t wave_base = 0, block_total = 0;
    for (uint32_t w = 0; w < PS_BLOCK / WAVE; ++w) {
        if (w < (threadIdx.x >> 6)) wave_base += s_wave[w];
        block_total += s_wave[w];
    }
    if (threadIdx.x < WAVE) {
        const unsigned long long pfx = chain_lookback(st, tile, block_total);
        if (threadIdx.x == 0) s_prefix = pfx;
    }
    __syncthreads();
    uint32_t run = (uint32_t)s_prefix + wave_base + incl - acc;
    uint32_t o[PS_ITEMS];
#pragma unroll
    for (int k = 0; k < PS_ITEMS; ++k) {
        o[k] = run;
        run += v[k];
    }
    if (full && (reinterpret_cast<uintptr_t>(out + base) & 15u) == 0) {
#pragma unroll
        for (int g = 0; g < 4; ++g) {
            u32x4 q;
            q.x = o[4 * g];
            q.y = o[4 * g + 1];
            q.z = o[4 * g + 2];
            q.w = o[4 * g + 3];
            *reinterpret_cast<u32x4*>(out + base + 4 * g) = q;
        }
    } else {
#pragma unroll
        for (int k = 0; k < PS_ITEMS; ++k)
            if (base + k < n) out[base + k] = o[k];
    }
    if (base < n && n <= base + PS_ITEMS) {
        const unsigned long long tot = s_prefix + wave_base + incl;
        out[n] = (uint32_t)tot;
        *total = tot;
        *total_host = tot;
        if (also_src) *also_host = *also_src;
    }
    chain_finish(st, n_tiles, &s_last);
}

constexpr int TAIL_BLOCK = 256;
constexpr int TAIL_ITEMS = 2;
constexpr int TAIL_TILE = TAIL_BLOCK * TAIL_ITEMS;
constexpr uint32_t TAIL_MAX_TILES = 1u << 15;

template <bool COMPACT = false>
__global__ __launch_bounds__(TAIL_BLOCK) void k_tile_rows(const uint32_t* __restrict__ cand_a, const uint32_t* __restrict__ cand_b,
                                                          const uint8_t* __restrict__ type, uint32_t n_cand, uint32_t paired,
                                                          const uint32_t* __restrict__ gate, uint32_t* __restrict__ tile_rows,
                                                          const CandGuard G) {
    __shared__ uint32_t s_part[TAIL_BLOCK / WAVE];
    if (gate && *gate != 0u) return;
    if (G.n_dev) {
        if (G.overflow()) return;
        n_cand = (uint32_t)*G.n_dev;
    }
    const uint32_t base = blockIdx.x * TAIL_TILE;
    if (base >= n_cand) return;
    uint32_t n = 0;
#pragma unroll
    for (int r = 0; r < TAIL_ITEMS; ++r) {
        const uint32_t i = base + r * TAIL_BLOCK + threadIdx.x;
        const uint32_t t = i < n_cand ? type[i] : 0u;
        if (COMPACT) n += t != 0u;
        else if (t) n += rows_of(t, cand_a[i], cand_b[i], paired);
    }
    n = wave_sum(n);
    if (lane_id() == 0) s_part[threadIdx.x >> 6] = n;
    __syncthreads();
    if (threadIdx.x == 0) {
        uint32_t s = 0;
        for (int w = 0; w < TAIL_BLOCK / WAVE; ++w) s += s_part[w];
        tile_rows[blockIdx.x] = s;
    }
}

__global__ __launch_bounds__(TAIL_BLOCK) void k_tail(const uint32_t* __restrict__ cand_a, const uint32_t* __restrict__ cand_p,
                                                     const uint32_t* __restrict__ cand_b, const uint8_t* __restrict__ type,
                                                     uint32_t n_cand, const uint32_t* __restrict__ len, Row* __restrict__ rows,
                                                     uint32_t bits, uint32_t paired, const uint32_t* __restrict__ gate,
                                                     const uint32_t* __restrict__ tile_rows, uint32_t n_tiles, uint32_t* __restrict__ done,
                                                     unsigned long long* __restrict__ counters, uint64_t* __restrict__ host_out,
                                                     const CandGuard G) {
    __shared__ uint32_t s_cnt[TAIL_ITEMS][TAIL_BLOCK / WAVE];
    __shared__ uint32_t s_pre[TAIL_BLOCK / WAVE];
    __shared__ uint32_t s_last;
    if ((gate && *gate != 0u) || G.overflow()) {
        if (blockIdx.x == 0 && threadIdx.x == 0) host_out[7] = G.overflow() ? 2 : 1;
        return;
    }
    if (G.n_dev) {
        n_cand = (uint32_t)*G.n_dev;
        n_tiles = (n_cand + TAIL_TILE - 1) / TAIL_TILE;
        if (n_tiles == 0) {
            if (blockIdx.x == 0 && threadIdx.x == 0) {
                for (int k = 0; k < 5; ++k) host_out[k] = 0;
                host_out[7] = 0;
            }
            return;
        }
        if (blockIdx.x >= n_tiles) return;
    }
    const uint32_t tile = blockIdx.x;
    const uint32_t base = tile * TAIL_TILE;
    const uint32_t wave = threadIdx.x >> 6, lane = lane_id();
    uint32_t pre = 0;
    {
        uint32_t k = threadIdx.x;
        for (; k + 3 * TAIL_BLOCK < tile; k += 4 * TAIL_BLOCK)
            pre += tile_rows[k] + tile_rows[k + TAIL_BLOCK] + tile_rows[k + 2 * TAIL_BLOCK] + tile_rows[k + 3 * TAIL_BLOCK];
        for (; k < tile; k += TAIL_BLOCK) pre += tile_rows[k];
    }
    uint32_t t[TAIL_ITEMS], a[TAIL_ITEMS], b[TAIL_ITEMS], cnt[TAIL_ITEMS], excl[TAIL_ITEMS];
    uint32_t pp[TAIL_ITEMS], la[TAIL_ITEMS], lb[TAIL_ITEMS];
#pragma unroll
    for (int r = 0; r < TAIL_ITEMS; ++r) {
        const uint32_t i = base + r * TAIL_BLOCK + threadIdx.x;
        t[r] = i < n_cand ? type[i] : 0u;
    }
#pragma unroll
    for (int r = 0; r < TAIL_ITEMS; ++r) {
        const uint32_t i = base + r * TAIL_BLOCK + threadIdx.x;
        a[r] = b[r] = pp[r] = la[r] = lb[r] = 0;
        if (t[r]) {
            a[r] = cand_a[i];
            b[r] = cand_b[i];
            pp[r] = cand_p[i];
        }
    }
#pragma unroll
    for (int r = 0; r < TAIL_ITEMS; ++r) {
        if (t[r]) {
            la[r] = len[a[r]];
            lb[r] = len[b[r]];
        }
        cnt[r] = t[r] ? rows_of(t[r], a[r], b[r], paired) : 0u;
        const uint32_t inc = wave_incl_scan(cnt[r]);
        excl[r] = inc - cnt[r];
        if (lane == WAVE - 1) s_cnt[r][wave] = inc;
    }
    pre = wave_sum(pre);
    if (lane == 0) s_pre[wave] = pre;
    __syncthreads();
    uint32_t pfx = 0, block_total = 0;
#pragma unroll
    for (int w = 0; w < TAIL_BLOCK / WAVE; ++w) pfx += s_pre[w];
#pragma unroll
    for (int r = 0; r < TAIL_ITEMS; ++r) {
        uint32_t before = block_total;
#pragma unroll
        for (int w = 0; w < TAIL_BLOCK / WAVE; ++w) {
            if ((uint32_t)w < wave) before += s_cnt[r][w];
            block_total += s_cnt[r][w];
        }
        excl[r] += before;
    }
    uint64_t nver = 0, suml = 0, sumb = 0, sume = 0;
#pragma unroll
    for (int r = 0; r < TAIL_ITEMS; ++r) {
        if (!t[r]) continue;
        nver += 1;
        write_rows(rows, pfx + excl[r], t[r], a[r], pp[r], b[r], la[r], lb[r], bits, paired, suml, sumb, sume);
    }
    {
        __shared__ uint64_t s_red[4][TAIL_BLOCK / WAVE];
        nver = wave_sum64(nver);
        suml = wave_sum64(suml);
        sumb = wave_sum64(sumb);
        sume = wave_sum64(sume);
        if (lane == 0) {
            s_red[0][wave] = nver;
            s_red[1][wave] = suml;
            s_red[2][wave] = sumb;
            s_red[3][wave] = sume;
        }
        __syncthreads();
        if (threadIdx.x < 4) {
            uint64_t v = 0;
            for (int w = 0; w < TAIL_BLOCK / WAVE; ++w) v += s_red[threadIdx.x][w];
            unsigned long long old = 0;
            if (v) old = atomicAdd(&counters[threadIdx.x], (unsigned long long)v);
            asm volatile("" :: "v"((uint32_t)old));
        }
    }
    if (tile == n_tiles - 1u && threadIdx.x == 0) host_out[0] = (uint64_t)pfx + block_total;
    __syncthreads();
    if (threadIdx.x == 0) {
        s_last = atomicAdd(done, 1u) == n_tiles - 1u ? 1u : 0u;
        if (s_last) {
            *done = 0;
            for (int k = 0; k < 4; ++k) {
                host_out[1 + k] = __hip_atomic_load(&counters[k], __ATOMIC_RELAXED, __HIP_MEMORY_SCOPE_AGENT);
                counters[k] = 0;
            }
            host_out[7] = 0;
        }
    }
}

__device__ inline uint32_t row_sums(uint32_t t, uint32_t a, uint32_t p, uint32_t b, uint32_t la, uint32_t lb, uint32_t bits,
                                    uint32_t paired, uint64_t& suml, uint64_t& sumb, uint64_t& sume) {
    uint32_t n = 0;
    sume += 2ull * packed_bytes((t & 1u) ? la - p : lb, bits);
    if (t & 1u) {
        const uint32_t l = la - p;
        const uint32_t k = (paired && a != (b ^ 1u)) ? 2u : 1u;
        suml += (uint64_t)k * l;
        sumb += (uint64_t)k * 2ull * packed_bytes(l, bits);
        n += k;
    }
    if (t & 2u) {
        const uint32_t k = paired ? 2u : 1u;
        suml += (uint64_t)k * lb;
        sumb += (uint64_t)k * 2ull * packed_bytes(lb, bits);
        n += k;
    }
    return n;
}

__global__ __launch_bounds__(TAIL_BLOCK) void k_tail_cands(const uint32_t* __restrict__ cand_a, const uint32_t* __restrict__ cand_p,
                                                           const uint32_t* __restrict__ cand_b, const uint8_t* __restrict__ type,
                                                           uint32_t n_cand, Cand* __restrict__ out, uint32_t paired,
                                                           const uint32_t* __restrict__ gate, const uint32_t* __restrict__ tile_recs,
                                                           uint32_t n_tiles, uint32_t* __restrict__ done, unsigned long long* __restrict__ rows_ctr,
                                                           uint64_t* __restrict__ host_out, const CandGuard G, uint32_t sh_b, uint32_t sh_p) {
    __shared__ uint32_t s_cnt[TAIL_ITEMS][TAIL_BLOCK / WAVE];
    __shared__ uint32_t s_pre[TAIL_BLOCK / WAVE];
    __shared__ uint32_t s_rows[TAIL_BLOCK / WAVE];
    __shared__ uint32_t s_last;
    if ((gate && *gate != 0u) || G.overflow()) {
        if (blockIdx.x == 0 && threadIdx.x == 0) host_out[7] = G.overflow() ? 2 : 1;
        return;
    }
    if (G.n_dev) {
        n_cand = (uint32_t)*G.n_dev;
        n_tiles = (n_cand + TAIL_TILE - 1) / TAIL_TILE;
        if (n_tiles == 0) {
            if (blockIdx.x == 0 && threadIdx.x == 0) {
                for (int k = 0; k < 5; ++k) host_out[k] = 0;
                host_out[7] = 0;
            }
            return;
        }
        if (blockIdx.x >= n_tiles) return;
    }
    const uint32_t tile = blockIdx.x;
    const uint32_t base = tile * TAIL_TILE;
    const uint32_t wave = threadIdx.x >> 6, lane = lane_id();
    uint32_t pre = 0;
    {
        uint32_t k = threadIdx.x;
        for (; k + 3 * TAIL_BLOCK < tile; k += 4 * TAIL_BLOCK)
            pre += tile_recs[k] + tile_recs[k + TAIL_BLOCK] + tile_recs[k + 2 * TAIL_BLOCK] + tile_recs[k + 3 * TAIL_BLOCK];
        for (; k < tile; k += TAIL_BLOCK) pre += tile_recs[k];
    }
    uint32_t t[TAIL_ITEMS], a[TAIL_ITEMS], b[TAIL_ITEMS], pp[TAIL_ITEMS], excl[TAIL_ITEMS];
#pragma unroll
    for (int r = 0; r < TAIL_ITEMS; ++r) {
        const uint32_t i = base + r * TAIL_BLOCK + threadIdx.x;
        t[r] = i < n_cand ? type[i] : 0u;
    }
#pragma unroll
    for (int r = 0; r < TAIL_ITEMS; ++r) {
        const uint32_t i = base + r * TAIL_BLOCK + threadIdx.x;
        a[r] = b[r] = pp[r] = 0;
        if (t[r]) {
            a[r] = cand_a[i];
            b[r] = cand_b[i];
            pp[r] = cand_p[i];
        }
    }
    uint32_t nrows = 0;
#pragma unroll
    for (int r = 0; r < TAIL_ITEMS; ++r) {
        const uint32_t cnt = t[r] ? 1u : 0u;
        const uint32_t inc = wave_incl_scan(cnt);
        excl[r] = inc - cnt;
        if (lane == WAVE - 1) s_cnt[r][wave] = inc;
        if (t[r]) nrows += rows_of(t[r], a[r], b[r], paired);
    }
    pre = wave_sum(pre);
    nrows = wave_sum(nrows);
    if (lane == 0) {
        s_pre[wave] = pre;
        s_rows[wave] = nrows;
    }
    __syncthreads();
    uint32_t pfx = 0, block_total = 0;
#pragma unroll
    for (int w = 0; w < TAIL_BLOCK / WAVE; ++w) pfx += s_pre[w];
#pragma unroll
    for (int r = 0; r < TAIL_ITEMS; ++r) {
        uint32_t before = block_total;
#pragma unroll
        for (int w = 0; w < TAIL_BLOCK / WAVE; ++w) {
            if ((uint32_t)w < wave) before += s_cnt[r][w];
            block_total += s_cnt[r][w];
        }
        excl[r] += before;
    }
    if (sh_b) {
        uint64_t* out8 = reinterpret_cast<uint64_t*>(out);
#pragma unroll
        for (int r = 0; r < TAIL_ITEMS; ++r)
            if (t[r]) out8[pfx + excl[r]] = pack_record(a[r], pp[r], b[r], t[r], sh_b, sh_p);
    } else {
#pragma unroll
        for (int r = 0; r < TAIL_ITEMS; ++r)
            if (t[r]) out[pfx + excl[r]] = Cand{a[r], pp[r], b[r], t[r]};
    }
    if (tile == n_tiles - 1u && threadIdx.x == 0) host_out[1] = (uint64_t)pfx + block_total;
    if (threadIdx.x == 0) {
        uint32_t rows = 0;
        for (int w = 0; w < TAIL_BLOCK / WAVE; ++w) rows += s_rows[w];
        unsigned long long old = 0;
        if (rows) old = atomicAdd(rows_ctr, (unsigned long long)rows);
        asm volatile("" :: "v"((uint32_t)old));
        s_last = atomicAdd(done, 1u) == n_tiles - 1u ? 1u : 0u;
        if (s_last) {
            *done = 0;
            host_out[0] = __hip_atomic_load(rows_ctr, __ATOMIC_RELAXED, __HIP_MEMORY_SCOPE_AGENT);
            *rows_ctr = 0;
            host_out[2] = host_out[3] = host_out[4] = 0;
            host_out[7] = 0;
        }
    }
}

}
```

Baseline: 1.515 billion.

## Queue deferred-list settle behind last piece and streamline compact tail kernels

Several changes land together. Per-tile row counts are now computed in k_tile_rows, so the last block of k_tail_cands writes the totals directly and the atomic done/rows counters are gone. The tail tile size becomes a template parameter, the fixup grid shrinks, k_read_sort can write the permutation directly for small inputs, and expand_records gets a fast path for paired type-1 twins. The deferred list is verified and emitted on the stream behind the last piece, using a deferred count read from the previous harvest, which removes a host round trip at the end. The cost is extra buffers, more code paths, and dependence on that count still being valid when the settle runs.

```diff
diff --git a/phasm_amd/csrc/c_api.hip b/phasm_amd/csrc/c_api.hip
--- a/phasm_amd/csrc/c_api.hip
+++ b/phasm_amd/csrc/c_api.hip
@@ -241,6 +241,7 @@
     DevBuf d_vlabel, d_vrank, d_vperm;
     DevBuf d_chain_state;
     DevBuf d_tail_state;
+    static constexpr size_t TAIL_STATE_BYTES = (2 * (size_t)po::TAIL_MAX_TILES + 4) * 4;
     DevBuf spare_rows;
     DevBuf spare_cands;
     DevBuf spare_edges;
@@ -306,6 +307,8 @@
     bool st_early_index = false;
     bool st_tail_gave_up = false;
     uint32_t st_defer_cap = 0;
+    DevBuf d_settle, d_settle_rows;
+    uint32_t st_settle_cap = 0;
     uint64_t last_host_rows = 0;
     uint64_t upload_gen = 0;
     bool idx_valid = false;
@@ -722,6 +725,21 @@
         const po::Cand c = load_rec(job, i);
         if (c.a >= n_reads || c.b >= n_reads) return false;
         const uint32_t la = len[c.a], lb = len[c.b];
+        if (paired && c.type == 1u && c.a != (c.b ^ 1u)) {
+            const uint32_t l = la - c.p;
+            const uint64_t q = pb(l);
+            __builtin_nontemporal_store((uint64_t)c.a | ((uint64_t)c.b << 32), o);
+            __builtin_nontemporal_store((uint64_t)c.p | ((uint64_t)la << 32), o + 1);
+            __builtin_nontemporal_store((uint64_t)l << 32, o + 2);
+            __builtin_nontemporal_store((uint64_t)(c.b ^ 1u) | ((uint64_t)(c.a ^ 1u) << 32), o + 3);
+            __builtin_nontemporal_store((uint64_t)(lb - l) | ((uint64_t)lb << 32), o + 4);
+            __builtin_nontemporal_store((uint64_t)l << 32, o + 5);
+            o += 6;
+            sl += 2ull * l;
+            sb += 4 * q;
+            se += 2 * q;
+            continue;
+        }
         se += 2 * pb((c.type & 1u) ? la - c.p : lb);
         if (c.type & 1u) {
             const uint32_t l = la - c.p;
@@ -978,8 +996,9 @@
             (const void*)po::k_scan_fixup<2, false>, (const void*)po::k_scan_fill<2, true>, (const void*)po::k_scan_fill<2, false>,
             (const void*)po::k_read_label, (const void*)po::k_read_sort, (const void*)po::k_read_invert, (const void*)po::k_defer_split,
             (const void*)po::k_verify_a<2, false, true, true>, (const void*)po::k_verify_a<2, false, true, false>,
-            (const void*)po::k_verify_a<2, true, true, false>, (const void*)po::k_select_local, (const void*)po::k_tile_rows<true>,
-            (const void*)po::k_tile_rows<false>, (const void*)po::k_tail, (const void*)po::k_tail_cands, (const void*)po::k_select,
+            (const void*)po::k_verify_a<2, true, true, false>, (const void*)po::k_select_local,
+            (const void*)po::k_tile_rows<true, po::TAIL_CANDS_ITEMS>, (const void*)po::k_tile_rows<false>, (const void*)po::k_tail,
+            (const void*)po::k_tail_cands<po::TAIL_CANDS_ITEMS>, (const void*)po::k_select,
             (const void*)po::k_emit, (const void*)po::k_verify_flat, (const void*)po::k_deferred_rowcnt, (const void*)po::k_emit_cands,
             (const void*)po::k_wide_insert<2, 1>, (const void*)po::k_wide_insert<2, 16>, (const void*)po::k_wide_chain_fill<2, 1>,
             (const void*)po::k_wide_chain_fill<2, 16>, (const void*)po::k_wide_finalize<2, 1>, (const void*)po::k_wide_finalize<2, 16>,
@@ -1543,6 +1562,8 @@
     const bool piece_reset = getenv("PHASM_PIECE_RESET") != nullptr;
     const bool sync_count = getenv("PHASM_SYNC_COUNT") != nullptr;
     const bool tail_classic = getenv("PHASM_TAIL_CLASSIC") != nullptr;
+    const char* tail_tile = getenv("PHASM_TAIL_TILE");
+    const char* sort_direct = getenv("PHASM_SORT_DIRECT");
     const bool select_kernel = getenv("PHASM_SELECT_KERNEL") != nullptr;
     const bool compact_sync = getenv("PHASM_COMPACT_SYNC") != nullptr;
     const int phase_events = phase_events_env();
@@ -1951,7 +1972,7 @@
             hipLaunchKernelGGL(K == W ? probe_full : probe_part, dim3(scan_grid), dim3(scan_waves * 64), scan_lds, st, A);
             if (pair_events) HIP_TRY(h, hipEventRecord(h->ev[EV_PROBE1], st));
             auto fixup = a.streamed ? po::k_scan_fixup<BITS, CAN_STREAM> : po::k_scan_fixup<BITS, false>;
-            hipLaunchKernelGGL(fixup, dim3(n_scan_waves), dim3(256), 0, st, A, n_scan_waves, self_clean ? 1u : 0u);
+            hipLaunchKernelGGL(fixup, dim3(cdiv(n_scan_waves, 4)), dim3(256), 0, st, A, n_scan_waves, self_clean ? 1u : 0u);
             if (sw.debug_left) {
                 PO_TRY(ensure_host(h, h->scratch_host, (size_t)n_scan_waves * 4));
                 HIP_TRY(h, hipMemcpyAsync(h->scratch_host.p, h->d_left_cnt.p, (size_t)n_scan_waves * 4, hipMemcpyDeviceToHost, st));
@@ -1993,6 +2014,7 @@
             async_count = pred > 0 && cap < (16u << 20) && cdiv(cap, po::TAIL_TILE) <= po::TAIL_MAX_TILES &&
                           fits(h->d_cand_a, cap * 4) && fits(h->d_cand_p, cap * 4) && fits(h->d_cand_b, cap * 4) && fits(h->d_type, cap) &&
                           fits(h->d_rowcnt, cap) && fits(h->d_row_off, (cap + 1) * 4) &&
+                          fits(h->d_tail_state, po_handle::TAIL_STATE_BYTES) &&
                           fits(h->spare_rows, h->home_on ? cap * sizeof(po::Cand) : worst * sizeof(po_row)) &&
                           (!order || (fits(h->d_vlabel, (uint64_t)(r_end - r_begin) * 4) && fits(h->d_vperm, (uint64_t)(r_end - r_begin) * 4) &&
                                       fits(h->d_vrank, (uint64_t)(r_end - r_begin) * 4))) && h->dev_words < 0xFFFFFFF0ull;
@@ -2116,7 +2138,7 @@
                     HIP_TRY(h, hipFuncSetAttribute(reinterpret_cast<const void*>(po::k_read_sort),
                                                    hipFuncAttributeMaxDynamicSharedMemorySize, (int)sort_lds));
                 hipLaunchKernelGGL(po::k_read_sort, dim3(1), dim3(po::SORT_BLOCK), sort_lds, st, h->d_vlabel.as<uint32_t>(), n_cand,
-                                   shift, n_bins, h->d_vrank.as<uint32_t>());
+                                   shift, n_bins, h->d_vrank.as<uint32_t>(), 0u, (uint32_t*)nullptr);
                 hipLaunchKernelGGL(po::k_read_invert, dim3(cdiv(n_cand, 256)), dim3(256), 0, st, h->d_vrank.as<uint32_t>(), n_cand, 0u,
                                    h->d_vperm.as<uint32_t>());
                 perm = h->d_vperm.as<uint32_t>();
@@ -2159,10 +2181,13 @@
                 HIP_TRY(h, hipFuncSetAttribute(reinterpret_cast<const void*>(po::k_read_sort),
                                                hipFuncAttributeMaxDynamicSharedMemorySize, (int)sort_lds));
             PO_TRY(ws(h->d_vrank, (size_t)n_a * 4));
+            bool direct = n_a < po::SORT_DIRECT_MAX;
+            if (sw.sort_direct) direct = atoi(sw.sort_direct) != 0;
             hipLaunchKernelGGL(po::k_read_sort, dim3(1), dim3(po::SORT_BLOCK), sort_lds, st, h->d_vlabel.as<uint32_t>(), n_a,
-                               shift, n_bins, h->d_vrank.as<uint32_t>());
-            hipLaunchKernelGGL(po::k_read_invert, dim3(cdiv(n_a, 256)), dim3(256), 0, st, h->d_vrank.as<uint32_t>(), n_a, r_begin,
-                               h->d_vperm.as<uint32_t>());
+                               shift, n_bins, h->d_vrank.as<uint32_t>(), r_begin, direct ? h->d_vperm.as<uint32_t>() : (uint32_t*)nullptr);
+            if (!direct)
+                hipLaunchKernelGGL(po::k_read_invert, dim3(cdiv(n_a, 256)), dim3(256), 0, st, h->d_vrank.as<uint32_t>(), n_a, r_begin,
+                                   h->d_vperm.as<uint32_t>());
             perm = h->d_vperm.as<uint32_t>();
         }
         const uint32_t ver_grid = perm ? 8 * ((n_a + 7) / 8) : n_a;
@@ -2221,15 +2246,23 @@
     }
 
     po_status fused_tail() {
-        const uint32_t n_tt = cdiv(n_cand, po::TAIL_TILE);
-        if (((size_t)po::TAIL_MAX_TILES + 4) * 4 > h->d_tail_state.cap) {
-            PO_TRY(ws(h->d_tail_state, ((size_t)po::TAIL_MAX_TILES + 4) * 4));
+        int items = compact_tail ? po::TAIL_CANDS_ITEMS : po::TAIL_ITEMS;
+        if (compact_tail && sw.tail_tile) {
+            const int v = atoi(sw.tail_tile);
+            if (v != 512 && v != 1024 && v != 2048) return fail(h, PO_ERR_INVALID, "PHASM_TAIL_TILE is 512, 1024 or 2048");
+            items = v / po::TAIL_BLOCK;
+        }
+        const uint32_t n_tt = cdiv(n_cand, (uint32_t)(po::TAIL_BLOCK * items));
+        if (po_handle::TAIL_STATE_BYTES > h->d_tail_state.cap) {
+            PO_TRY(ws(h->d_tail_state, po_handle::TAIL_STATE_BYTES));
             HIP_TRY(h, hipMemsetAsync(h->d_tail_state.p, 0, h->d_tail_state.cap, st));
         }
         uint32_t* tile_rows = h->d_tail_state.as<uint32_t>();
-        uint32_t* tail_done = tile_rows + po::TAIL_MAX_TILES;
+        uint32_t* tail_done = tile_rows + 2 * (size_t)po::TAIL_MAX_TILES;
         const uint32_t* tgate = n_selfrep_reads ? n_deferred : nullptr;
-        hipLaunchKernelGGL(compact_tail ? po::k_tile_rows<true> : po::k_tile_rows<false>, dim3(n_tt), dim3(po::TAIL_BLOCK), 0, st, A.cand_a,
+        auto tile_kernel = !compact_tail ? po::k_tile_rows<false> : items == 2 ? po::k_tile_rows<true, 2> :
+                           items == 4 ? po::k_tile_rows<true, 4> : po::k_tile_rows<true, 8>;
+        hipLaunchKernelGGL(tile_kernel, dim3(n_tt), dim3(po::TAIL_BLOCK), 0, st, A.cand_a,
                            A.cand_b, h->d_type.as<uint8_t>(), n_cand, paired, tgate, tile_rows, G);
         if (phase_events) HIP_TRY(h, hipEventRecord(h->ev[EV_SELECT], st));
         rows_late = true;
@@ -2239,12 +2272,15 @@
         h->spare_rows = DevBuf();
         tail_zone = async_count ? zone : 48;
         h->pinned[tail_zone] = 0;
+        h->pinned[tail_zone + 5] = ~0ull;
         h->pinned[tail_zone + 7] = 0;
         if (compact_tail) {
             res->compact = true;
-            hipLaunchKernelGGL(po::k_tail_cands, dim3(n_tt), dim3(po::TAIL_BLOCK), 0, st, A.cand_a, A.cand_p, A.cand_b, h->d_type.as<uint8_t>(),
-                               n_cand, res->d_rows.as<po::Cand>(), paired, tgate, tile_rows, n_tt, tail_done,
-                               scalars + 3, h->pinned_dev + tail_zone, G, h->home_sh_b, h->home_sh_p);
+            auto tail_kernel = items == 2 ? po::k_tail_cands<2> : items == 4 ? po::k_tail_cands<4> : po::k_tail_cands<8>;
+            hipLaunchKernelGGL(tail_kernel, dim3(n_tt), dim3(po::TAIL_BLOCK), 0, st, A.cand_a, A.cand_p, A.cand_b, h->d_type.as<uint8_t>(),
+                               n_cand, res->d_rows.as<po::Cand>(), paired, tgate, tile_rows, n_tt,
+                               h->pinned_dev + tail_zone, G, h->home_sh_b, h->home_sh_p,
+                               a.streamed && h->d_defer.p ? h->d_defer.as<uint32_t>() + (size_t)h->st_defer_cap * 4 : (const uint32_t*)nullptr);
         } else
         hipLaunchKernelGGL(po::k_tail, dim3(n_tt), dim3(po::TAIL_BLOCK), 0, st, A.cand_a, A.cand_p, A.cand_b, h->d_type.as<uint8_t>(),
                            n_cand, len, res->d_rows.as<po::Row>(), (uint32_t)BITS, paired, tgate, tile_rows, n_tt, tail_done,
@@ -4680,7 +4716,7 @@
                           &h->d_ps_blocks, &h->d_scalars, &h->d_cand_a, &h->d_cand_p, &h->d_cand_b, &h->d_type,
                           &h->d_rowcnt, &h->d_row_off, &h->d_flag, &h->d_pair_key, &h->d_pair_min, &h->spare_rows, &h->spare_cands, &h->spare_edges, &h->spare_nrank,
                           &h->d_vlabel, &h->d_vrank, &h->d_vperm, &h->d_end_a, &h->d_end_b, &h->d_dpcnt, &h->d_lay_len, &h->d_lay_cnt, &h->d_rflag, &h->d_removed, &h->d_ekey, &h->d_ecnt,
-                          &h->d_ewin, &h->d_eoff, &h->d_chain_state, &h->d_tail_state, &h->d_efirst, &h->d_lay_firstc};
+                          &h->d_ewin, &h->d_eoff, &h->d_chain_state, &h->d_tail_state, &h->d_settle, &h->d_settle_rows, &h->d_efirst, &h->d_lay_firstc};
         if (h->copy_stream) (void)hipStreamSynchronize(h->copy_stream);
         if (h->up_stream) (void)hipStreamSynchronize(h->up_stream);
         if (h->rc_stream) (void)hipStreamSynchronize(h->rc_stream);
@@ -5370,6 +5406,9 @@
     PO_TRY(ensure(h, h->d_defer, (size_t)h->st_defer_cap * sizeof(po::Cand) + 16));
     if (!getenv("PHASM_DEFER_CAP")) h->st_defer_cap = (uint32_t)std::min<size_t>((h->d_defer.cap - 16) / sizeof(po::Cand), 0xFFFFFF00u);
     HIP_TRY(h, hipMemsetAsync(h->d_defer.as<char>() + (size_t)h->st_defer_cap * sizeof(po::Cand), 0, 16, h->stream));
+    h->st_settle_cap = std::min<uint32_t>(h->st_defer_cap, 64u * po::PS_TILE);
+    PO_TRY(ensure(h, h->d_settle, (size_t)h->st_settle_cap * 5 + 64));
+    PO_TRY(ensure(h, h->d_settle_rows, (size_t)h->st_settle_cap * 4 * sizeof(po_row)));
     h->paired = true;
     ++h->upload_gen;
     h->dirty = false;
@@ -5435,8 +5474,14 @@
     };
     h->st_pend.valid = false;
     bool tail_gave_up = false;
+    uint64_t def_known = ~0ull;
+    uint32_t def_known_k = ~0u;
     h->st_harvest = [&]() -> po_status {
         const uint32_t k = h->st_pend.k;
+        if (h->st_pend.tail && h->st_pend.compact) {
+            def_known = h->pinned[h->st_pend.zone + 5];
+            def_known_k = k;
+        }
         bool needs_classic = false;
         const uint64_t nk = finish_piece(h, &needs_classic);
         if (needs_classic) {
@@ -5466,8 +5511,40 @@
         }
         st = completed(k, h->stats, nk);
     }
+    bool settle_queued = false;
+    uint64_t def_known_final = 0;
+    hipEvent_t* settle_ev = (trace || phase_events_env() == 1) ? h->ev_sets[P & 1] : nullptr;
+    if (st == PO_OK && !tail_gave_up && P >= 2 && h->st_pend.valid && h->st_pend.k == P - 1 && h->st_pend.tail && h->st_pend.compact &&
+        def_known_k == P - 2 && def_known <= h->st_settle_cap) {
+        const uint32_t n_q = (uint32_t)def_known;
+        def_known_final = def_known;
+        auto queue = [&]() -> po_status {
+            hipStream_t s = h->stream;
+            po::Cand* list = h->d_defer.as<po::Cand>();
+            uint8_t* rowcnt = h->d_settle.as<uint8_t>();
+            uint32_t* row_off = reinterpret_cast<uint32_t*>(h->d_settle.as<char>() + (((size_t)h->st_settle_cap + 15) & ~(size_t)15));
+            unsigned long long* scalars = h->d_scalars.as<unsigned long long>();
+            if (settle_ev) HIP_TRY(h, hipEventRecord(settle_ev[EV_START], s));
+            hipLaunchKernelGGL(po::k_verify_flat, dim3(cdiv((uint64_t)n_q * 64, 256)), dim3(256), 0, s, dw, h->d_woff.as<uint64_t>(),
+                               h->d_len.as<uint32_t>(), list, n_q, h->n_exc_uploaded ? h->d_exc_off.as<uint32_t>() : nullptr,
+                               h->d_exc_pos.as<uint32_t>(), h->d_exc_byte.as<uint8_t>());
+            hipLaunchKernelGGL(po::k_deferred_rowcnt, dim3(cdiv(n_q, 256)), dim3(256), 0, s, list, n_q, 1u, rowcnt);
+            HIP_TRY(h, hipGetLastError());
+            PO_TRY(prefix_sum<uint8_t>(h, rowcnt, n_q, row_off, &h->pinned[41]));
+            HIP_TRY(h, hipMemsetAsync(scalars + 4, 0, 32, s));
+            hipLaunchKernelGGL(po::k_emit_cands, dim3(std::min<uint32_t>(cdiv(n_q, 256), (uint32_t)h->n_cu * 16)), dim3(256), 0, s,
+                               list, rowcnt, row_off, n_q, h->d_len.as<uint32_t>(), h->d_settle_rows.as<po::Row>(), 2u, 1u, scalars + 4);
+            HIP_TRY(h, hipGetLastError());
+            HIP_TRY(h, hipMemcpyAsync(h->pinned + 42, scalars + 4, 4 * sizeof(uint64_t), hipMemcpyDeviceToHost, s));
+            if (settle_ev) HIP_TRY(h, hipEventRecord(settle_ev[EV_EMIT], s));
+            return PO_OK;
+        };
+        if (n_q) st = queue();
+        settle_queued = st == PO_OK;
+    }
     if (st == PO_OK && h->st_pend.valid && !tail_gave_up) {
-        if (hipStreamSynchronize(h->stream) != hipSuccess) st = fail(h, PO_ERR_HIP, "stream");
+        const hipError_t e = settle_queued ? hipEventSynchronize(h->st_pend.ev[EV_DONE]) : hipStreamSynchronize(h->stream);
+        if (e != hipSuccess) st = fail(h, PO_ERR_HIP, "stream");
         else st = h->st_harvest();
     }
     h->st_harvest = nullptr;
@@ -5497,6 +5574,30 @@
     (void)hipEventSynchronize(h->ev_up1);
     (void)hipEventElapsedTime(&ms, h->ev_up0, h->ev_up1);
     h->stats.ms_upload = ms;
+    if (settle_queued) {
+        const uint32_t n_def = (uint32_t)def_known_final;
+        h->defer_need = n_def;
+        if (n_def) HIP_TRY(h, hipStreamSynchronize(h->stream));
+        const uint64_t n_rows = n_def ? h->pinned[41] : 0;
+        if (n_rows) {
+            float ms_def = 0;
+            if (settle_ev) (void)hipEventElapsedTime(&ms_def, settle_ev[EV_START], settle_ev[EV_EMIT]);
+            sum.n_verified += h->pinned[42];
+            sum.sum_overlap_bases += h->pinned[43];
+            sum.verify_bytes_algo += h->pinned[44];
+            sum.verify_bytes_exec += h->pinned[45];
+            sum.n_rows += n_rows;
+            sum.ms_verify += ms_def;
+            sum.ms_total += ms_def;
+            PO_TRY(append_rows(h, R, h->d_settle_rows, n_rows, P, P + 1));
+        }
+        if (trace) {
+            std::fprintf(stderr, "[stream] deferred list settled at %.3f ms (%u candidates, queued behind the last piece)\n", since(), n_def);
+            (void)hipStreamSynchronize(h->copy_stream);
+            std::fprintf(stderr, "[stream] last row home at %.3f ms\n", since());
+        }
+        return PO_OK;
+    }
     HIP_TRY(h, hipMemcpyAsync(h->pinned + 40, h->d_defer.as<char>() + (size_t)h->st_defer_cap * sizeof(po::Cand), 8,
                               hipMemcpyDeviceToHost, h->stream));
     HIP_TRY(h, hipStreamSynchronize(h->stream));
diff --git a/phasm_amd/csrc/kernels.hip.h b/phasm_amd/csrc/kernels.hip.h
--- a/phasm_amd/csrc/kernels.hip.h
+++ b/phasm_amd/csrc/kernels.hip.h
@@ -1071,11 +1071,11 @@
 template <int BITS, bool STREAM = false>
 __global__ void k_scan_fixup(const ScanArgs A, uint32_t n_waves, uint32_t clean) {
     constexpr int W = 64 / BITS;
-    const uint32_t wv = blockIdx.x;
+    const uint32_t wv = blockIdx.x * (blockDim.x >> 6) + (threadIdx.x >> 6);
     if (wv >= n_waves) return;
     const uint32_t cnt = min(A.left_cnt[wv], LEFT_CAP);
     const uint2* __restrict__ list = A.left + (size_t)wv * LEFT_CAP;
-    for (uint32_t k = threadIdx.x; k < cnt; k += blockDim.x) {
+    for (uint32_t k = lane_id(); k < cnt; k += WAVE) {
         const uint2 e = list[k];
         const uint32_t t = e.x, ln = e.y >> 8, sft = e.y & 255u;
         if (t < A.tile_begin || t >= A.tile_end || ln >= (uint32_t)WAVE || sft >= (uint32_t)W) continue;
@@ -1101,10 +1101,7 @@
             atomicAdd(&A.tile_count[t], n);
         }
     }
-    if (clean) {
-        __syncthreads();
-        if (threadIdx.x == 0) A.left_cnt[wv] = 0;
-    }
+    if (clean && lane_id() == 0) A.left_cnt[wv] = 0;
 }
 
 __global__ void k_add_extra(uint32_t* __restrict__ tile_count, const uint32_t* __restrict__ tile_extra, uint32_t t0, uint32_t t1) {
@@ -1220,8 +1217,10 @@
 }
 
 constexpr int SORT_BLOCK = 1024;
+constexpr uint32_t SORT_DIRECT_MAX = 12288;
 __global__ __launch_bounds__(SORT_BLOCK) void k_read_sort(const uint32_t* __restrict__ label, uint32_t n_reads, uint32_t shift,
-                                                          uint32_t n_bins, uint32_t* __restrict__ rank) {
+                                                          uint32_t n_bins, uint32_t* __restrict__ rank, uint32_t r_begin,
+                                                          uint32_t* __restrict__ perm) {
     extern __shared__ uint32_t s_bin[];
     uint32_t* s_wave = s_bin + n_bins;
     const uint32_t tid = threadIdx.x;
@@ -1263,8 +1262,12 @@
             v[k] = i < n_reads ? label[i] : ~0u;
         }
 #pragma unroll
-        for (uint32_t k = 0; k < UN; ++k)
-            if (v[k] != ~0u) rank[base + k * SORT_BLOCK] = atomicAdd(&s_bin[v[k] >> shift], 1u);
+        for (uint32_t k = 0; k < UN; ++k) {
+            if (v[k] == ~0u) continue;
+            const uint32_t pos = atomicAdd(&s_bin[v[k] >> shift], 1u);
+            if (perm) perm[pos] = r_begin + base + k * SORT_BLOCK;
+            else rank[base + k * SORT_BLOCK] = pos;
+        }
     }
 }
 
@@ -2351,35 +2354,51 @@
 constexpr int TAIL_ITEMS = 2;
 constexpr int TAIL_TILE = TAIL_BLOCK * TAIL_ITEMS;
 constexpr uint32_t TAIL_MAX_TILES = 1u << 15;
-
-template <bool COMPACT = false>
+constexpr int TAIL_CANDS_ITEMS = 2;
+
+template <bool COMPACT = false, int ITEMS = TAIL_ITEMS>
 __global__ __launch_bounds__(TAIL_BLOCK) void k_tile_rows(const uint32_t* __restrict__ cand_a, const uint32_t* __restrict__ cand_b,
                                                           const uint8_t* __restrict__ type, uint32_t n_cand, uint32_t paired,
                                                           const uint32_t* __restrict__ gate, uint32_t* __restrict__ tile_rows,
                                                           const CandGuard G) {
-    __shared__ uint32_t s_part[TAIL_BLOCK / WAVE];
+    __shared__ uint32_t s_part[2][TAIL_BLOCK / WAVE];
     if (gate && *gate != 0u) return;
     if (G.n_dev) {
         if (G.overflow()) return;
         n_cand = (uint32_t)*G.n_dev;
     }
-    const uint32_t base = blockIdx.x * TAIL_TILE;
+    const uint32_t base = blockIdx.x * (TAIL_BLOCK * ITEMS);
     if (base >= n_cand) return;
-    uint32_t n = 0;
-#pragma unroll
-    for (int r = 0; r < TAIL_ITEMS; ++r) {
+    uint32_t n = 0, nrec = 0;
+    uint32_t t[ITEMS];
+#pragma unroll
+    for (int r = 0; r < ITEMS; ++r) {
         const uint32_t i = base + r * TAIL_BLOCK + threadIdx.x;
-        const uint32_t t = i < n_cand ? type[i] : 0u;
-        if (COMPACT) n += t != 0u;
-        else if (t) n += rows_of(t, cand_a[i], cand_b[i], paired);
+        t[r] = i < n_cand ? type[i] : 0u;
+    }
+#pragma unroll
+    for (int r = 0; r < ITEMS; ++r) {
+        const uint32_t i = base + r * TAIL_BLOCK + threadIdx.x;
+        nrec += t[r] != 0u;
+        if (COMPACT && !((t[r] & 1u) && paired)) n += rows_of(t[r], 0u, 0u, paired);
+        else if (t[r]) n += rows_of(t[r], cand_a[i], cand_b[i], paired);
     }
     n = wave_sum(n);
-    if (lane_id() == 0) s_part[threadIdx.x >> 6] = n;
+    if (COMPACT) nrec = wave_sum(nrec);
+    if (lane_id() == 0) {
+        s_part[0][threadIdx.x >> 6] = n;
+        s_part[1][threadIdx.x >> 6] = nrec;
+    }
     __syncthreads();
     if (threadIdx.x == 0) {
-        uint32_t s = 0;
-        for (int w = 0; w < TAIL_BLOCK / WAVE; ++w) s += s_part[w];
-        tile_rows[blockIdx.x] = s;
+        uint32_t s = 0, sr = 0;
+        for (int w = 0; w < TAIL_BLOCK / WAVE; ++w) s += s_part[0][w], sr += s_part[1][w];
+        if (COMPACT) {
+            tile_rows[blockIdx.x] = sr;
+            tile_rows[TAIL_MAX_TILES + blockIdx.x] = s;
+        } else {
+            tile_rows[blockIdx.x] = s;
+        }
     }
 }
 
@@ -2526,23 +2545,24 @@
     return n;
 }
 
+template <int ITEMS>
 __global__ __launch_bounds__(TAIL_BLOCK) void k_tail_cands(const uint32_t* __restrict__ cand_a, const uint32_t* __restrict__ cand_p,
                                                            const uint32_t* __restrict__ cand_b, const uint8_t* __restrict__ type,
                                                            uint32_t n_cand, Cand* __restrict__ out, uint32_t paired,
                                                            const uint32_t* __restrict__ gate, const uint32_t* __restrict__ tile_recs,
-                                                           uint32_t n_tiles, uint32_t* __restrict__ done, unsigned long long* __restrict__ rows_ctr,
-                                                           uint64_t* __restrict__ host_out, const CandGuard G, uint32_t sh_b, uint32_t sh_p) {
-    __shared__ uint32_t s_cnt[TAIL_ITEMS][TAIL_BLOCK / WAVE];
+                                                           uint32_t n_tiles, uint64_t* __restrict__ host_out, const CandGuard G,
+                                                           uint32_t sh_b, uint32_t sh_p, const uint32_t* __restrict__ defer_ctr) {
+    constexpr uint32_t TILE = TAIL_BLOCK * ITEMS;
+    __shared__ uint32_t s_cnt[ITEMS][TAIL_BLOCK / WAVE];
     __shared__ uint32_t s_pre[TAIL_BLOCK / WAVE];
     __shared__ uint32_t s_rows[TAIL_BLOCK / WAVE];
-    __shared__ uint32_t s_last;
     if ((gate && *gate != 0u) || G.overflow()) {
         if (blockIdx.x == 0 && threadIdx.x == 0) host_out[7] = G.overflow() ? 2 : 1;
         return;
     }
     if (G.n_dev) {
         n_cand = (uint32_t)*G.n_dev;
-        n_tiles = (n_cand + TAIL_TILE - 1) / TAIL_TILE;
+        n_tiles = (n_cand + TILE - 1) / TILE;
         if (n_tiles == 0) {
             if (blockIdx.x == 0 && threadIdx.x == 0) {
                 for (int k = 0; k < 5; ++k) host_out[k] = 0;
@@ -2553,8 +2573,9 @@
         if (blockIdx.x >= n_tiles) return;
     }
     const uint32_t tile = blockIdx.x;
-    const uint32_t base = tile * TAIL_TILE;
+    const uint32_t base = tile * TILE;
     const uint32_t wave = threadIdx.x >> 6, lane = lane_id();
+    const bool last = tile == n_tiles - 1u;
     uint32_t pre = 0;
     {
         uint32_t k = threadIdx.x;
@@ -2562,14 +2583,19 @@
             pre += tile_recs[k] + tile_recs[k + TAIL_BLOCK] + tile_recs[k + 2 * TAIL_BLOCK] + tile_recs[k + 3 * TAIL_BLOCK];
         for (; k < tile; k += TAIL_BLOCK) pre += tile_recs[k];
     }
-    uint32_t t[TAIL_ITEMS], a[TAIL_ITEMS], b[TAIL_ITEMS], pp[TAIL_ITEMS], excl[TAIL_ITEMS];
-#pragma unroll
-    for (int r = 0; r < TAIL_ITEMS; ++r) {
+    uint32_t nrows = 0;
+    if (last) {
+        const uint32_t* __restrict__ tile_nrows = tile_recs + TAIL_MAX_TILES;
+        for (uint32_t k = threadIdx.x; k < n_tiles; k += TAIL_BLOCK) nrows += tile_nrows[k];
+    }
+    uint32_t t[ITEMS], a[ITEMS], b[ITEMS], pp[ITEMS], excl[ITEMS];
+#pragma unroll
+    for (int r = 0; r < ITEMS; ++r) {
         const uint32_t i = base + r * TAIL_BLOCK + threadIdx.x;
         t[r] = i < n_cand ? type[i] : 0u;
     }
 #pragma unroll
-    for (int r = 0; r < TAIL_ITEMS; ++r) {
+    for (int r = 0; r < ITEMS; ++r) {
         const uint32_t i = base + r * TAIL_BLOCK + threadIdx.x;
         a[r] = b[r] = pp[r] = 0;
         if (t[r]) {
@@ -2578,17 +2604,15 @@
             pp[r] = cand_p[i];
         }
     }
-    uint32_t nrows = 0;
-#pragma unroll
-    for (int r = 0; r < TAIL_ITEMS; ++r) {
+#pragma unroll
+    for (int r = 0; r < ITEMS; ++r) {
         const uint32_t cnt = t[r] ? 1u : 0u;
         const uint32_t inc = wave_incl_scan(cnt);
         excl[r] = inc - cnt;
         if (lane == WAVE - 1) s_cnt[r][wave] = inc;
-        if (t[r]) nrows += rows_of(t[r], a[r], b[r], paired);
     }
     pre = wave_sum(pre);
-    nrows = wave_sum(nrows);
+    if (last) nrows = wave_sum(nrows);
     if (lane == 0) {
         s_pre[wave] = pre;
         s_rows[wave] = nrows;
@@ -2598,7 +2622,7 @@
 #pragma unroll
     for (int w = 0; w < TAIL_BLOCK / WAVE; ++w) pfx += s_pre[w];
 #pragma unroll
-    for (int r = 0; r < TAIL_ITEMS; ++r) {
+    for (int r = 0; r < ITEMS; ++r) {
         uint32_t before = block_total;
 #pragma unroll
         for (int w = 0; w < TAIL_BLOCK / WAVE; ++w) {
@@ -2610,29 +2634,22 @@
     if (sh_b) {
         uint64_t* out8 = reinterpret_cast<uint64_t*>(out);
 #pragma unroll
-        for (int r = 0; r < TAIL_ITEMS; ++r)
+        for (int r = 0; r < ITEMS; ++r)
             if (t[r]) out8[pfx + excl[r]] = pack_record(a[r], pp[r], b[r], t[r], sh_b, sh_p);
     } else {
 #pragma unroll
-        for (int r = 0; r < TAIL_ITEMS; ++r)
+        for (int r = 0; r < ITEMS; ++r)
             if (t[r]) out[pfx + excl[r]] = Cand{a[r], pp[r], b[r], t[r]};
     }
-    if (tile == n_tiles - 1u && threadIdx.x == 0) host_out[1] = (uint64_t)pfx + block_total;
-    if (threadIdx.x == 0) {
+    if (last && threadIdx.x == 0) {
         uint32_t rows = 0;
         for (int w = 0; w < TAIL_BLOCK / WAVE; ++w) rows += s_rows[w];
-        unsigned long long old = 0;
-        if (rows) old = atomicAdd(rows_ctr, (unsigned long long)rows);
-        asm volatile("" :: "v"((uint32_t)old));
-        s_last = atomicAdd(done, 1u) == n_tiles - 1u ? 1u : 0u;
-        if (s_last) {
-            *done = 0;
-            host_out[0] = __hip_atomic_load(rows_ctr, __ATOMIC_RELAXED, __HIP_MEMORY_SCOPE_AGENT);
-            *rows_ctr = 0;
-            host_out[2] = host_out[3] = host_out[4] = 0;
-            host_out[7] = 0;
-        }
-    }
-}
-
-}
+        host_out[0] = rows;
+        host_out[1] = (uint64_t)pfx + block_total;
+        host_out[2] = host_out[3] = host_out[4] = 0;
+        if (defer_ctr) host_out[5] = *defer_ctr;
+        host_out[7] = 0;
+    }
+}
+
+}
```

Measured after the change: 1.571 billion (median of 5 runs). 3.7% higher.
